# BruceCanovas/supersurfel_fusion

Hardware: AMD Instinct MI355X
Metric: frames_per_sec (higher is better)
Workload: dtype f32; 1 GPU; 640x480 synthetic RGB-D orbit (seed 1234), map seeded with 1000000 supersurfels (~993223 live, ~86081 visible), reference rgbd_benchmark parameters, extract+ICP+fuse per frame; width=640, height=480, n_model=993223, n_visible=86081, superpixels=1200, icp_iter_max=10, icp_forced=False, seed_order=seeded, exchange=none, pipeline_depth=2, extract_batch=8

## Files before the change

supersurfel_fusion_amd/binding.py:

```python
import ctypes as C
import os
import numpy as np

ICP_RECORD = 29
MIGRANT_WORDS = 28
_HERE = os.path.dirname(os.path.abspath(__file__))
PRODUCT_LIB = os.path.join(_HERE, "csrc", "libssf_hip.so")


class SsfConfig(C.Structure):
    _fields_ = [
        ("width", C.c_int), ("height", C.c_int),
        ("fx", C.c_float), ("fy", C.c_float), ("cx", C.c_float), ("cy", C.c_float),
        ("cell_size", C.c_int), ("lambda_pos", C.c_float), ("lambda_bound", C.c_float),
        ("lambda_size", C.c_float), ("lambda_disp", C.c_float), ("thresh_disp", C.c_float),
        ("seg_iter", C.c_int), ("seg_use_ransac", C.c_int), ("nb_samples", C.c_int),
        ("filter_iter", C.c_int), ("filter_alpha", C.c_float), ("filter_beta", C.c_float),
        ("filter_threshold", C.c_float), ("range_min", C.c_float), ("range_max", C.c_float),
        ("delta_t", C.c_int), ("conf_thresh", C.c_float), ("nb_supersurfels_max", C.c_int),
        ("icp_iter", C.c_int), ("icp_cov_thresh", C.c_double),
        ("rng_seed", C.c_uint64), ("icp_force_iters", C.c_int), ("device_id", C.c_int),
        ("stream", C.c_void_p), ("rank", C.c_int), ("nranks", C.c_int),
        ("shard_tile", C.c_float), ("depth_prefilter", C.c_int), ("prefilter_sigma_color", C.c_float),
        ("prefilter_sigma_space", C.c_float), ("profile", C.c_int), ("pipeline_depth", C.c_int), ("extract_batch", C.c_int),
# ... 2 lines not shown

class SsfSurfels(C.Structure):
    _fields_ = [("positions", C.c_void_p), ("colors", C.c_void_p), ("stamps", C.c_void_p),
                ("orientations", C.c_void_p), ("shapes", C.c_void_p), ("dims", C.c_void_p),
                ("confidences", C.c_void_p)]


class SsfFrameResult(C.Structure):
    _fields_ = [("pose", C.c_float * 12), ("icp_valid", C.c_int), ("icp_iters", C.c_int),
                ("n_model", C.c_int), ("n_visible", C.c_int), ("n_removed", C.c_int),
                ("n_inserted", C.c_int), ("n_updated", C.c_int), ("stamp", C.c_int),
                ("stage_ms", C.c_float * 3)]

    def as_dict(self):
        return dict(pose=np.array(self.pose[:], np.float32), icp_valid=self.icp_valid,
                    icp_iters=self.icp_iters, n_model=self.n_model, n_visible=self.n_visible,
                    n_removed=self.n_removed, n_inserted=self.n_inserted, n_updated=self.n_updated,
                    stamp=self.stamp, stage_ms=list(self.stage_ms[:]))


ABI_SYMBOLS = [
    "ssf_abi_version", "ssf_backend_name", "ssf_default_config", "ssf_create", "ssf_destroy",
    "ssf_last_error", "ssf_process_frame", "ssf_process_frame_device", "ssf_stage_extract",
    "ssf_debug_set_max_passes", "ssf_debug_set_bin_min_rows", "ssf_stage_set_shard", "ssf_stage_icp_begin",
    "ssf_stage_icp_accumulate", "ssf_stage_icp_update", "ssf_stage_icp_end", "ssf_stage_match",
    "ssf_stage_fuse", "ssf_get_pose", "ssf_set_pose", "ssf_get_counts", "ssf_get_model",
    "ssf_get_frame", "ssf_set_model", "ssf_get_index_map", "ssf_get_boundary_map",
    "ssf_get_inlier_map", "ssf_get_plane_depth", "ssf_get_superpixels", "ssf_get_model_device", "ssf_get_frame_device",
    "ssf_export_model_txt", "ssf_apply_deformation", "ssf_get_kernel_times",
    "ssf_reset_kernel_times", "ssf_set_profile", "ssf_bilateral_filter", "ssf_submit_frame",
    "ssf_process_submitted", "ssf_pending_frames", "ssf_pipeline_capacity", "ssf_can_submit", "ssf_stage_begin_submitted",
    "ssf_stage_icp_accumulate_device", "ssf_stage_icp_fetch", "ssf_stage_match_device", "ssf_stage_fuse_device",
    "ssf_comm_unique_id", "ssf_comm_attach", "ssf_comm_info", "ssf_p2p_export", "ssf_p2p_attach", "ssf_p2p_region", "ssf_p2p_attach_local", "ssf_p2p_configure", "ssf_rehome_begin", "ssf_rehome_end", "ssf_get_global_counts", "ssf_align", "ssf_fern_codes", "ssf_process_sequence", "ssf_debug_recentre", "ssf_debug_recentre_count", "ssf_get_preview_image", "ssf_stage_fuse_begin", "ssf_stage_fuse_end", "ssf_stage_fuse_begin_device", "ssf_stage_fuse_end_device",
    "ssf_sequence_times", "ssf_sequence_marks", "ssf_stream_copy_rate", "ssf_upload_stats", "ssf_pooled_streams", "ssf_waiter_matches", "ssf_waiter_match_repairs", "ssf_tuner_state", "ssf_submit_frame_tables", "ssf_comm_deal_extract",
]

INPUT_FORMAT_SYMBOLS = ["ssf_set_input_format", "ssf_get_input_format"]
COLOR_FORMATS = {"rgb8": (0, 3), "bgr8": (1, 3), "rgba8": (2, 4), "bgra8": (3, 4)}
DEPTH_FORMATS = {"f32": (0, 4), "u16": (1, 2)}
DYNAMIC_MASK_SYMBOLS = ["ssf_process_frame_pixmask", "ssf_submit_frame_pixmask", "ssf_process_sequence_pixmask",
                        "ssf_stage_extract_pixmask", "ssf_get_dynamic_superpixels"]
RENDER_SYMBOLS = ["ssf_render_default_params", "ssf_render_model"]
GRAPH_SYMBOLS = ["ssf_graph_default_params", "ssf_graph_build", "ssf_graph_get_nodes", "ssf_graph_get_binding",
                 "ssf_graph_bind_points", "ssf_graph_apply", "ssf_graph_info"]
GRAPH_SOLVE_SYMBOLS = ["ssf_graph_solve_default_params", "ssf_graph_get_edges", "ssf_graph_solve", "ssf_graph_get_transforms",
                       "ssf_graph_apply_solved"]
KEYFRAME_SYMBOLS = ["ssf_keyframes_default_params", "ssf_keyframes_configure", "ssf_keyframes_set_ferns", "ssf_keyframes_get_ferns",
                    "ssf_keyframes_encode", "ssf_keyframes_query", "ssf_keyframes_add", "ssf_keyframes_consider", "ssf_keyframes_put",
                    "ssf_keyframes_get", "ssf_keyframes_set_pose", "ssf_keyframes_align", "ssf_keyframes_info", "ssf_keyframes_clear"]
KEYFRAMES_MAX_FERNS = 4096
KEYFRAMES_MAX_CANDIDATES = 8
FERN_DTYPE = np.dtype([("x", np.uint16), ("y", np.uint16), ("r", np.uint8), ("g", np.uint8), ("b", np.uint8), ("pad", np.uint8),
                       ("depth_mm", np.uint32)])
QUERY_SYMBOLS = ["ssf_query_default_params", "ssf_query_count", "ssf_query_rows"]
QUERY_REGIONS = {"all": 0, "sphere": 1, "box": 2, "frustum": 3}
NAVGRID_SYMBOLS = ["ssf_navgrid_default_params", "ssf_navgrid_default_pose", "ssf_navgrid_build"]
NAVGRID_OUTPUTS = (("zmin", np.float32, ()), ("zmax", np.float32, ()), ("hits", np.uint32, (2,)), ("state", np.int8, ()),
                   ("dist2", np.int32, ()))
NAVGRID_OUTPUT_NAMES = tuple(nm for nm, _, _ in NAVGRID_OUTPUTS)
MOTION_SYMBOLS = ["ssf_motion_default_params", "ssf_motion_segment", "ssf_motion_mask", "ssf_process_frame_motion", "ssf_get_motion_mask"]
ODOMETRY_SYMBOLS = ["ssf_odometry_default_params", "ssf_odometry_set_reference", "ssf_odometry_linearise", "ssf_odometry_estimate",
                    "ssf_odometry_track", "ssf_process_frame_odometry", "ssf_get_odometry"]
ODOMETRY_REASONS = ("converged", "max_iterations", "too_few_pixels", "degenerate", "motion_gate")
ODO_MAX_LEVELS, ODO_RECORD = 6, 29
MOTION_CLASSES = {"invalid": 0, "static": 1, "seed": 2, "unknown": 3}
MOTION_OUTPUTS = (("mask", np.uint8), ("label", np.int32), ("cls", np.uint8))
MOTION_OUTPUT_NAMES = tuple(nm for nm, _ in MOTION_OUTPUTS)
RENDER_OUTPUTS = (("depth", np.float32, ()), ("index", np.int32, ()), ("rgb8", np.uint8, (3,)), ("color", np.float32, (3,)),
                  ("normal", np.float32, (3,)))
RENDER_OUTPUT_NAMES = tuple(nm for nm, _, _ in RENDER_OUTPUTS)

SURFEL_FIELDS = (("positions", 3, np.float32), ("colors", 3, np.float32), ("stamps", 2, np.int32),
                 ("orientations", 9, np.float32), ("shapes", 6, np.float32),
                 ("dims", 2, np.float32), ("confidences", 1, np.float32))


class SsfError(RuntimeError):
    pass


class SsfRenderParams(C.Structure):
    _fields_ = [("pose", C.c_void_p), ("width", C.c_int), ("height", C.c_int)] + \
               [(nm, C.c_float) for nm in ("fx", "fy", "cx", "cy", "z_min", "z_max", "min_conf", "splat_scale")] + \
               [("visible_only", C.c_int), ("on_device", C.c_int)]


class SsfRenderStats(C.Structure):
    _fields_ = [(nm, C.c_int64) for nm in ("fragments", "pixels_filled", "rows_shown", "list_entries")]

    def as_dict(self):
        return {nm: int(getattr(self, nm)) for nm, _ in self._fields_}


class SsfMotionParams(C.Structure):
    _fields_ = [("pose", C.c_void_p)] + \
               [(nm, C.c_float) for nm in ("min_conf", "splat_scale", "front_abs", "front_quad", "link_abs", "link_rel")] + \
               [("min_seeds", C.c_int), ("unknown_per_seed", C.c_int), ("on_device", C.c_int)]


class SsfMotionStats(C.Structure):
    _fields_ = [(nm, C.c_int64) for nm in ("n_seed", "n_unknown", "n_components", "n_dynamic_components", "pixels_masked")]

    def as_dict(self):
        return {nm: int(getattr(self, nm)) for nm, _ in self._fields_}


# ... 136 lines not shown
        L.ssf_set_model.argtypes = [vp, C.POINTER(SsfSurfels), C.c_int, C.c_int, C.c_int]
        for nm in ("ssf_get_index_map", "ssf_get_boundary_map", "ssf_get_inlier_map",
                   "ssf_get_plane_depth", "ssf_get_superpixels", "ssf_get_preview_image"):
            getattr(L, nm).argtypes = [vp, vp]
        L.ssf_get_model_device.argtypes = [vp, C.POINTER(SsfSurfels), C.POINTER(C.c_int)]
        L.ssf_export_model_txt.argtypes = [vp, C.c_char_p]
        L.ssf_apply_deformation.argtypes = [vp, vp, vp, vp, C.c_int, vp, vp]
        L.ssf_get_kernel_times.argtypes = [vp, vp, vp, vp, C.c_int]
        L.ssf_reset_kernel_times.argtypes = [vp]
        L.ssf_set_profile.argtypes = [vp, C.c_int]
        L.ssf_bilateral_filter.argtypes = [vp, vp, vp, C.c_int]
        L.ssf_submit_frame.argtypes = [vp, vp, vp, C.c_int, vp]
        L.ssf_process_sequence.argtypes = [vp, vp, vp, C.c_int, C.c_int, vp]
        L.ssf_process_submitted.argtypes = [vp, vp, C.POINTER(SsfFrameResult)]
        L.ssf_pending_frames.argtypes = [vp]
        L.ssf_pipeline_capacity.argtypes = [vp]
        L.ssf_can_submit.argtypes = [vp]
        L.ssf_align.argtypes = [vp, C.POINTER(SsfSurfels), C.c_int, vp, vp, C.POINTER(C.c_int), C.POINTER(C.c_int), C.POINTER(C.c_int)]
        L.ssf_fern_codes.argtypes = [vp, vp, vp, C.c_int, C.c_int, vp, vp, vp, C.c_int, vp]
        L.ssf_comm_unique_id.argtypes = [vp]
        L.ssf_comm_attach.argtypes = [vp, vp]
        L.ssf_p2p_export.argtypes = [vp, vp]
        L.ssf_p2p_attach.argtypes = [vp, vp]
        L.ssf_p2p_region.argtypes = [vp, C.POINTER(C.c_void_p), C.POINTER(C.c_size_t)]
        L.ssf_p2p_attach_local.argtypes = [vp, C.POINTER(C.c_void_p)]
        L.ssf_p2p_configure.argtypes = [vp, C.c_int, C.c_double]
        L.ssf_rehome_begin.argtypes = [vp, vp, C.c_int, C.POINTER(C.c_int)]
        L.ssf_rehome_end.argtypes = [vp, vp, C.c_int]
        L.ssf_get_global_counts.argtypes = [vp, vp]
        L.ssf_stage_begin_submitted.argtypes = [vp]
        L.ssf_stage_icp_accumulate_device.argtypes = [vp, vp]
        L.ssf_stage_icp_fetch.argtypes = [vp, vp, vp]
        L.ssf_stage_match_device.argtypes = [vp, vp, vp]
        L.ssf_stage_fuse_device.argtypes = [vp, vp, vp, C.POINTER(SsfFrameResult)]
        L.ssf_stage_fuse_begin.argtypes = [vp, vp, vp, vp]
        L.ssf_stage_fuse_end.argtypes = [vp, vp, C.POINTER(SsfFrameResult)]
        L.ssf_stage_fuse_begin_device.argtypes = [vp, vp, vp, vp]
        L.ssf_stage_fuse_end_device.argtypes = [vp, vp, C.POINTER(SsfFrameResult)]
        self.has_input_format = all(hasattr(L, nm) for nm in INPUT_FORMAT_SYMBOLS)
        if self.has_input_format:
            L.ssf_set_input_format.argtypes = [vp, C.c_int, C.c_int, C.c_double]
            L.ssf_get_input_format.argtypes = [vp, C.POINTER(C.c_int), C.POINTER(C.c_int), C.POINTER(C.c_double)]
        self.has_dynamic_mask = all(hasattr(L, nm) for nm in DYNAMIC_MASK_SYMBOLS)
        if self.has_dynamic_mask:
            L.ssf_process_frame_pixmask.argtypes = [vp, vp, vp, C.c_int, vp, vp, C.POINTER(SsfFrameResult)]
            L.ssf_submit_frame_pixmask.argtypes = [vp, vp, vp, C.c_int, vp]
            L.ssf_process_sequence_pixmask.argtypes = [vp, vp, vp, vp, C.c_int, C.c_int, vp]
            L.ssf_stage_extract_pixmask.argtypes = [vp, vp, vp, C.c_int, vp]
            L.ssf_get_dynamic_superpixels.argtypes = [vp, vp, C.POINTER(C.c_int)]
        self.has_render = all(hasattr(L, nm) for nm in RENDER_SYMBOLS)
        if self.has_render:
            L.ssf_render_default_params.argtypes = [vp, C.POINTER(SsfRenderParams)]
            L.ssf_render_model.argtypes = [vp, C.POINTER(SsfRenderParams), vp, vp, vp, vp, vp, C.POINTER(SsfRenderStats)]
        self.has_query = all(hasattr(L, nm) for nm in QUERY_SYMBOLS)
        if self.has_query:
            L.ssf_query_default_params.argtypes = [vp, C.POINTER(SsfQueryParams)]
            L.ssf_query_count.argtypes = [vp, C.POINTER(SsfQueryParams), C.POINTER(SsfQueryStats)]
            L.ssf_query_rows.argtypes = [vp, C.POINTER(SsfQueryParams), C.POINTER(SsfSurfels), vp, C.c_int, C.POINTER(SsfQueryStats)]
        self.has_navgrid = all(hasattr(L, nm) for nm in NAVGRID_SYMBOLS)
        if self.has_navgrid:
            L.ssf_navgrid_default_params.argtypes = [vp, C.POINTER(SsfNavGridParams)]
            L.ssf_navgrid_default_pose.argtypes = [vp, C.POINTER(SsfNavGridParams), vp]
            L.ssf_navgrid_build.argtypes = [vp, C.POINTER(SsfNavGridParams), C.POINTER(SsfNavGridOut), C.POINTER(SsfNavGridStats)]
        self.has_motion = all(hasattr(L, nm) for nm in MOTION_SYMBOLS)
        if self.has_motion:
            mp, ms = C.POINTER(SsfMotionParams), C.POINTER(SsfMotionStats)
            L.ssf_motion_default_params.argtypes = [vp, mp]
            L.ssf_motion_segment.argtypes = [vp, mp, vp, vp, vp, vp, vp, ms]
            L.ssf_motion_mask.argtypes = [vp, mp, vp, vp, vp, vp, vp, ms]
            L.ssf_process_frame_motion.argtypes = [vp, vp, vp, C.c_int, vp, mp, C.POINTER(SsfFrameResult)]
            L.ssf_get_motion_mask.argtypes = [vp, vp, ms]
        self.has_odometry = all(hasattr(L, nm) for nm in ODOMETRY_SYMBOLS)
        if self.has_odometry:
            op, orr = C.POINTER(SsfOdometryParams), C.POINTER(SsfOdometryResult)
            L.ssf_odometry_default_params.argtypes = [vp, op]
            L.ssf_odometry_set_reference.argtypes = [vp, vp, vp, C.c_int, vp]
            L.ssf_odometry_linearise.argtypes = [vp, op, C.c_int, vp, vp]
            L.ssf_odometry_estimate.argtypes = [vp, op, vp, vp, C.c_int, vp, vp, orr]
            L.ssf_odometry_track.argtypes = [vp, op, vp, vp, C.c_int, vp, orr]
            L.ssf_process_frame_odometry.argtypes = [vp, vp, vp, C.c_int, op, C.POINTER(SsfMotionParams), C.POINTER(SsfFrameResult)]
            L.ssf_get_odometry.argtypes = [vp, vp, vp, orr]
            L.ssf_odometry_get_pyramid.argtypes = [vp, C.c_int, C.c_int, vp, vp, vp, vp, C.POINTER(C.c_int), C.POINTER(C.c_int), vp]
        self.has_graph = all(hasattr(L, nm) for nm in GRAPH_SYMBOLS)
        if self.has_graph:
            ip = C.POINTER(C.c_int)
            L.ssf_graph_default_params.argtypes = [C.POINTER(SsfGraphParams)]
            L.ssf_graph_build.argtypes = [vp, C.POINTER(SsfGraphParams), ip]
            L.ssf_graph_get_nodes.argtypes = [vp, vp, vp, vp, C.c_int]
            L.ssf_graph_get_binding.argtypes = [vp, vp, vp, C.c_int]
            L.ssf_graph_bind_points.argtypes = [vp, vp, vp, C.c_int, vp, vp]
            L.ssf_graph_apply.argtypes = [vp, vp, vp]
            L.ssf_graph_info.argtypes = [vp, ip, ip, ip]
        self.has_graph_solve = all(hasattr(L, nm) for nm in GRAPH_SOLVE_SYMBOLS)
        if self.has_graph_solve:
            L.ssf_graph_solve_default_params.argtypes = [C.POINTER(SsfGraphSolveParams)]
            L.ssf_graph_get_edges.argtypes = [vp, vp, C.c_int]
            L.ssf_graph_solve.argtypes = [vp, C.POINTER(SsfGraphSolveParams), vp, vp, vp, C.c_int, C.POINTER(SsfGraphSolveResult)]
            L.ssf_graph_get_transforms.argtypes = [vp, vp, vp, C.c_int]
            L.ssf_graph_apply_solved.argtypes = [vp]
        self.has_keyframes = all(hasattr(L, nm) for nm in KEYFRAME_SYMBOLS)
        if self.has_keyframes:
            ip, kp, kr = C.POINTER(C.c_int), C.POINTER(SsfKeyframesParams), C.POINTER(SsfKeyframeResult)
            L.ssf_keyframes_default_params.argtypes = [kp]
            L.ssf_keyframes_configure.argtypes = [vp, kp]
            L.ssf_keyframes_set_ferns.argtypes = [vp, vp, C.c_int]
            L.ssf_keyframes_get_ferns.argtypes = [vp, vp, C.c_int]
# ... 375 lines not shown
        self._need_odometry("ssf_odometry_estimate")
        return self._odometry_estimate(self._dev_addr(d_rgb), self._dev_addr(d_depth), 1, init12, params)

    def _odometry_track(self, rgb_ptr, depth_ptr, on_device, params):
        p = self._odometry_params(params)
        prior, res = np.zeros(12, np.float32), SsfOdometryResult()
        self._ck(self.L.lib.ssf_odometry_track(self.h, C.byref(p), rgb_ptr, depth_ptr, int(on_device), _ptr(prior), C.byref(res)),
                 "ssf_odometry_track")
        return (prior if res.valid else None), res.as_dict()

    def odometry_track(self, rgb, depth, params=None):
        self._need_odometry("ssf_odometry_track")
        rgb, depth = self._frame(rgb, depth)
        return self._odometry_track(_ptr(rgb), _ptr(depth), 0, params)

    def odometry_track_device(self, d_rgb, d_depth, params=None):
        self._need_odometry("ssf_odometry_track")
        return self._odometry_track(self._dev_addr(d_rgb), self._dev_addr(d_depth), 1, params)

    def odometry_last(self):
        self._need_odometry("ssf_get_odometry")
        rel, prior, res = np.zeros(12, np.float32), np.zeros(12, np.float32), SsfOdometryResult()
        self._ck(self.L.lib.ssf_get_odometry(self.h, _ptr(rel), _ptr(prior), C.byref(res)), "ssf_get_odometry")
        return dict(rel=rel, prior=prior if res.valid else None, result=res.as_dict())

    def odometry_pyramid(self, which, level):
        self._need_odometry("ssf_odometry_get_pyramid")
        w, h, k = C.c_int(), C.c_int(), np.zeros(4, np.float32)
        self._ck(self.L.lib.ssf_odometry_get_pyramid(self.h, int(which), int(level), None, None, None, None, C.byref(w), C.byref(h), _ptr(k)),
                 "ssf_odometry_get_pyramid")
        out = {nm: np.empty((h.value, w.value), np.float32) for nm in ("I", "D", "gx", "gy")}
        self._ck(self.L.lib.ssf_odometry_get_pyramid(self.h, int(which), int(level), *[_ptr(out[nm]) for nm in ("I", "D", "gx", "gy")],
                                                     None, None, None), "ssf_odometry_get_pyramid")
        out["intrinsics"] = k
        return out

    def _process_frame_odometry(self, rgb_ptr, depth_ptr, on_device, odometry, motion):
        self._need_odometry("ssf_process_frame_odometry")
        if not (odometry is True or isinstance(odometry, dict)):
            raise SsfError("odometry is None, True or a dict of ssf_odometry_params fields, got %r" % (odometry,))
        p = self._odometry_params(None if odometry is True else odometry)
        mp, keep = None, None
        if motion is not None:
            self._need_motion("ssf_process_frame_motion")
            if not (motion is True or isinstance(motion, dict)):
                raise SsfError("motion is None, True or a dict of ssf_motion_params fields, got %r" % (motion,))
            m, keep = self._motion_params(None if motion is True else motion, on_device)
            mp = C.byref(m)
        res = SsfFrameResult()
        self._ck(self.L.lib.ssf_process_frame_odometry(self.h, rgb_ptr, depth_ptr, int(bool(on_device)), C.byref(p), mp, C.byref(res)),
                 "ssf_process_frame_odometry")
        return res

    def _need_query(self, symbol):
        if not self.L.has_query:
            raise SsfError("%s does not export %s: it does not query the model (include/ssf_query.h, HIP product only)"
                           % (self.L.path, symbol))

    def _query_params(self, on_device, min_conf=0.0, t_init=None, t_last=None, visible_only=False, region="all", pose=None,
                      radius=0.0, half=(0.0, 0.0, 0.0), camera=None, z_range=None):
        p = SsfQueryParams()
        self._ck(self.L.lib.ssf_query_default_params(self.h, C.byref(p)), "ssf_query_default_params")
        keep = None
        if pose is not None:
            pose = np.asarray(pose, np.float32)
            if pose.shape == (3, 4):
                pose = np.concatenate([pose[:, :3].ravel(), pose[:, 3]])
            if pose.size != 12:
                raise SsfError("a query pose is 12 floats (R row-major, then t) or 3 x 4 [R | t], got shape %s" % (pose.shape,))
            keep = np.ascontiguousarray(pose.ravel(), np.float32)
            p.pose = keep.ctypes.data
        p.min_conf = float(min_conf)
        if t_init is not None:
            p.t_init_min, p.t_init_max = int(t_init[0]), int(t_init[1])
        if t_last is not None:
            p.t_last_min, p.t_last_max = int(t_last[0]), int(t_last[1])
        if isinstance(region, str) and region not in QUERY_REGIONS:
            raise SsfError("unknown query region %r (known: %s)" % (region, ", ".join(QUERY_REGIONS)))
        p.region = QUERY_REGIONS[region] if isinstance(region, str) else int(region)
        p.radius = float(radius)
        p.half[0], p.half[1], p.half[2] = (float(v) for v in half)
        if camera is not None:
            p.width, p.height = int(camera["width"]), int(camera["height"])
            p.fx, p.fy, p.cx, p.cy = (float(camera[k]) for k in ("fx", "fy", "cx", "cy"))
        if z_range is not None:
            p.z_min, p.z_max = float(z_range[0]), float(z_range[1])
        p.visible_only, p.on_device = int(bool(visible_only)), int(bool(on_device))
        return p, keep

    def _query_rows(self, p, ptrs, index_ptr, capacity):
        st = SsfQueryStats()
        surf = SsfSurfels(*[ptrs.get(name) for name, _, _ in SURFEL_FIELDS])
        rc = self.L.lib.ssf_query_rows(self.h, C.byref(p), C.byref(surf) if any(ptrs.get(name) for name, _, _ in SURFEL_FIELDS) else None,
                                       index_ptr, int(capacity), C.byref(st))
        if rc != 0:
            e = SsfError("ssf_query_rows failed (%d): %s" % (rc, self.L.lib.ssf_last_error(self.h).decode()))
            e.rc, e.stats = rc, st.as_dict()
            raise e
        return st.as_dict()

    def query_default_params(self):
        self._need_query("ssf_query_default_params")
        p = SsfQueryParams()
        self._ck(self.L.lib.ssf_query_default_params(self.h, C.byref(p)), "ssf_query_default_params")
        return {nm: (list(getattr(p, nm)) if nm == "half" else getattr(p, nm)) for nm, _ in p._fields_ if nm != "pose"}

# ... 773 lines not shown
```

supersurfel_fusion_amd/csrc/ssf_device.hpp:

```cpp
#pragma once
#include <hip/hip_runtime.h>
#include <stdint.h>
#include <cstddef>
#include "ssf_math.hpp"
#include "../../include/ssf.h"
#include "../../include/ssf_input.h"
#include "../../include/ssf_dynamic.h"

#ifdef SSF_EXPERIMENTS
#include <stdlib.h>
static inline int ssf_env_int_(const char* name, int dflt) { const char* e = getenv(name); return e ? atoi(e) : dflt; }
#define SSF_ENV_INT(name, dflt) ssf_env_int_("SSF_" name, dflt)
#define SSF_ENV_SET(name) (getenv("SSF_" name) != nullptr)
#define SSF_ENV_STR(name) getenv("SSF_" name)
#define SSF_PROBE(dbg, bits) ((((dbg)) & (bits)) != 0)
#else
#define SSF_PROBE(dbg, bits) (false)
#define SSF_ENV_INT(name, dflt) (dflt)
#define SSF_ENV_SET(name) (false)
#define SSF_ENV_STR(name) ((const char*)nullptr)
#endif

namespace ssf {

// ... 126 lines not shown
void pass_args_table(const SegParams& p, const FrameMaps& m, int kmax, void* host_out);
void launch_update_passes_team(hipStream_t st, const SegParams& p, FrameMaps& m, int nb, int k0, int k1, bool rgbd, const void* d_pas, void* d_ws,
                               unsigned int* abort_flag);
void launch_init_samples(hipStream_t st, const SegParams& p, FrameMaps& m, int nb, int true_buf);
void launch_eval_samples(hipStream_t st, const SegParams& p, FrameMaps& m, int nb);
void launch_init_disp(hipStream_t st, const SegParams& p, FrameMaps& m, int nb, bool ransac);
void launch_plane_filter(hipStream_t st, const SegParams& p, FrameMaps& m, int nb, int true_buf);
void launch_import_frame(hipStream_t st, const SegParams& p, FrameMaps& m, int nb, SurfelSoA frame, const float* wire, unsigned long long* best, uint8_t* matched);
void launch_export_rows(hipStream_t st, const SegParams& p, const FrameMaps& m, int nb, SurfelSoA frame, float* wire);
void launch_render_moments(hipStream_t st, const SegParams& p, const Cam& cam, FrameMaps& m, int nb);
void launch_render_moments_pixmask(hipStream_t st, const SegParams& p, const Cam& cam, FrameMaps& m, int nb, const uint8_t* pixmask,
                                   uint32_t* pixcnt);
void launch_finalize_surfels(hipStream_t st, const SegParams& p, FrameMaps& m, int nb, SurfelSoA frame, float zmin,
                             float zmax, int stamp0, const uint8_t* dynamic_mask, unsigned mask_bits,
                             unsigned long long* best, uint8_t* matched);
void launch_finalize_surfels_pixmask(hipStream_t st, const SegParams& p, FrameMaps& m, int nb, SurfelSoA frame, float zmin, float zmax,
                                     int stamp0, const uint8_t* dynamic_mask, unsigned mask_bits, unsigned long long* best, uint8_t* matched,
                                     const uint32_t* pixcnt, unsigned pixmask_bits);
void launch_bilateral(hipStream_t st, const void* in, int depth_format, double depth_scale, float* out, int W, int H, float sigma_color,
                      float sigma_space);
void launch_bilateral_batch(hipStream_t st, const BatchIn& in, float* out0, size_t slab, int nb, int W, int H, float sigma_color, float sigma_space);
void launch_boundary_map(hipStream_t st, const SegParams& p, const int32_t* label, int32_t* out);
void launch_preview(hipStream_t st, int W, int H, const int32_t* label, const uint32_t* rgba, uint8_t* out );

struct alignas(64) IcpGo { float T[12]; unsigned long long flag; unsigned long long x; };
static_assert(sizeof(IcpGo) == 64, "one line");
#define SSF_ICP_GO_ABORT (1ull << 63)
#define SSF_ICP_GO_MATCH (1ull << 62)
#define SSF_ICP_GO_CHECK_MASK 0x3FFFFFFFu
SSF_HD unsigned int icp_go_word_weight(unsigned int dword) {
    return dword < 12u ? (2u * dword + 1u) * 0x9E3779B1u : (dword == 14u ? 0x85EBCA6Bu : (dword == 15u ? 0xC2B2AE35u : 0u));
}
SSF_HD unsigned int icp_go_abort_check(unsigned int want) { return ((want * 0x9E3779B1u) >> 2) & SSF_ICP_GO_CHECK_MASK; }
#define SSF_ICP_GO_SLOTS 4
struct MatchArgs { float zmin, zmax; long long id_offset; unsigned long long* best; uint8_t* matched; int32_t* cand; };
struct ClassifyArgs { Cam cam; const float* plane_depth; int delta_t; float conf_thresh, zmin, zmax; };
struct ShardArgs { int rank, nranks, migrate; float tile; };
struct AssocTables { const unsigned long long* best; const uint8_t* matched; const int32_t* cand; int S; };
int icp_variant_mode();
void launch_icp(hipStream_t st, const Cam& cam, SurfelSoA model, int n_visible, const uint2* pix2, const float4* fpack,
                Rt T, long long* replicas, unsigned int* ticket,
                long long* sums29, Mailbox* mb, unsigned long long seq, int dbg = -1, IcpGo* go = nullptr,
                unsigned long long go_seq = 0, const struct P2PView* pv = nullptr, int by_tile = 0, const MatchArgs* match = nullptr);
void launch_bin_rows(hipStream_t st, const Cam& cam, SurfelSoA model, int n, Rt T, uint32_t* count, uint32_t* cursor, SurfelSoA out);
size_t bin_buffer_words(const Cam& cam, size_t capacity);
void launch_match(hipStream_t st, const Cam& cam, SurfelSoA model, int n_visible, const uint2* pix2, const float4* fpack,
                  Rt pose, float zmin, float zmax, long long id_offset,
                  unsigned long long* best, uint8_t* matched, int32_t* cand , int S,
                  const int32_t* orig = nullptr );
struct OovStore { SurfelSoA rows; uint8_t* live; int cap; };
#define PART_GROUP 16
#define PART_REPLICAS 8
struct PartitionWs { uint32_t* sup_vis; uint32_t* sup_oov; uint32_t* tot; uint32_t* ticket; uint32_t* other; int words; };
void launch_fuse(hipStream_t st, SurfelSoA model , SurfelSoA frame, Rt pose, int stamp, long long id_offset,
                 int n_visible, const AssocTables& at, int do_update, int capacity, const ShardArgs& sh, Counters* cnt, OovStore oov,
                 int span_upper, const ClassifyArgs& ca, uint8_t* state_vis, uint8_t* state_oov, uint32_t* bc_oov, const PartitionWs& ws,
                 int tail_in_move = 0 );
#ifdef SSF_EXPERIMENTS
void set_pass_stats(int on);
void set_pass_trace(unsigned long long* device_words );
void set_fuse_trace(unsigned long long* device_words );
#endif
struct MoveTotals { int from_tot, nv , head_old, tail_old ; };
void launch_pack_emigrants(hipStream_t st, SurfelSoA model, const AssocTables& at, long long id_offset, int n_visible,
                           const uint8_t* state_vis, int do_update, const ShardArgs& sh, int32_t* table);
void launch_migrate_in(hipStream_t st, SurfelSoA model, const int32_t* table, int S, int capacity, Counters* cnt, const ShardArgs& sh,
                       const ClassifyArgs& ca, Rt pose, int stamp, uint8_t* state_vis, const PartitionWs& ws);
void launch_rehome_split(hipStream_t st, SurfelSoA dense, int n, int n_visible, int rank, int nranks, float tile, uint32_t* bc, int* tot3,
                         SurfelSoA stay, int32_t* table, int table_rows);
void launch_rehome_unpack(hipStream_t st, const int32_t* table, int n, SurfelSoA dst, int base);
void launch_first_frame(hipStream_t st, SurfelSoA model, SurfelSoA frame, Rt pose, int S, int capacity, const ShardArgs& sh, Counters* cnt);
struct NextIcp {
    Cam cam; const uint2* pix2; const float4* fpack;
    Rt T;
    long long* replicas; unsigned int* ticket; long long* sums; Mailbox* mb; unsigned long long seq;
};
void launch_move_rows(hipStream_t st, SurfelSoA vis_src, SurfelSoA vis_dst, OovStore oov, int nv_upper, int span_upper,
                      const uint8_t* state_vis, const uint8_t* state_oov, const uint32_t* bc_oov, const PartitionWs& ws,
                      Counters* cnt , Mailbox* mb, unsigned long long cnt_seq, const NextIcp* next,
                      const struct P2PView* next_pv = nullptr, const MoveTotals* totals = nullptr);
void launch_oov_compact(hipStream_t st, OovStore src, OovStore dst, int span_upper, int new_head, uint32_t* bc_oov, Counters* cnt,
                        int set_span);
struct ModelView { SurfelSoA vis; OovStore oov; int n_visible, nbv, nvs, oov_head, oov_tail, nbo, nslots; };
void launch_align(hipStream_t st, const Cam& cam, const float* spos, const float* slab, const float* snrm, const float* sconf,
                  int n, SurfelSoA frame, const int32_t* label, const float* plane_depth, Rt T, long long* out40);
void launch_fern_codes(hipStream_t st, const uint8_t* rgb, const float* depth, int W, int H, const uint32_t* fpos,
                       const uint8_t* frgb, const float* fdepth, int n, uint8_t* codes);
#define SSF_P2P_MAX_RANKS 8
struct P2PView { unsigned char* peer[SSF_P2P_MAX_RANKS]; int me, nranks, S; unsigned long long seq, timeout_ticks; };
enum { P2P_FLAG_ASSOC = 0, P2P_FLAG_MIGR = 1 };
#define SSF_P2P_HEADER 8192
SSF_HD size_t p2p_slot(int par, int src) { return (size_t)(par * SSF_P2P_MAX_RANKS + src); }
SSF_HD size_t p2p_spad(int S) { return ((size_t)S + 63) & ~(size_t)63; }
SSF_HD size_t p2p_off_icp(int par, int src) { return p2p_slot(par, src) * 320; }
SSF_HD size_t p2p_off_cnt(int par, int src) { return 16 * 320 + p2p_slot(par, src) * 64; }
SSF_HD size_t p2p_off_flag(int kind, int par, int src) { return 16 * 384 + ((size_t)kind * 16 + p2p_slot(par, src)) * 64; }
SSF_HD size_t p2p_off_best(int S, int par, int src) { return SSF_P2P_HEADER + p2p_slot(par, src) * (size_t)S * 8; }
SSF_HD size_t p2p_off_matched(int S, int par, int src) { return SSF_P2P_HEADER + 16 * (size_t)S * 8 + p2p_slot(par, src) * p2p_spad(S); }
SSF_HD size_t p2p_off_migr(int S, int par, int src) {
    return SSF_P2P_HEADER + 16 * (size_t)S * 8 + 16 * p2p_spad(S) + p2p_slot(par, src) * (size_t)S * SSF_MIGRANT_WORDS * 4;
}
SSF_HD size_t p2p_region_bytes(int S) { return p2p_off_migr(S, 1, SSF_P2P_MAX_RANKS - 1) + (size_t)S * SSF_MIGRANT_WORDS * 4; }
void launch_p2p_counts(hipStream_t st, const P2PView& pv, const Counters* cnt, Mailbox* mb, unsigned long long all_seq);
void launch_p2p_assoc(hipStream_t st, const P2PView& pv, unsigned long long* best, uint8_t* matched, Mailbox* mb);
void launch_p2p_migrants(hipStream_t st, const P2PView& pv, int32_t* table, unsigned int* ticket , Mailbox* mb);
void launch_publish_icp(hipStream_t st, const long long* rec29, Mailbox* mb, unsigned long long seq);
void launch_publish_all_counts(hipStream_t st, const int* all5, int nranks, Mailbox* mb, unsigned long long seq);
void launch_publish_counts(hipStream_t st, Counters* cnt, int shrink_by_removed, Mailbox* mb, unsigned long long seq);
void launch_lab_refresh(hipStream_t st, SurfelSoA s, int n);
void launch_pack_orient(hipStream_t st, SurfelSoA s, int n, float* out9);
void launch_deformation(hipStream_t st, SurfelSoA model, int n, int m, const float* npos, const float* nrot,
                        const float* ntrans, float* nodes16, const float* w4, const int32_t* idx4);

struct KernelTimer;
KernelTimer* current_timer();
void set_current_timer(KernelTimer* t);
void timer_begin(KernelTimer* t, const char* name, hipStream_t st);
void timer_end(KernelTimer* t, hipStream_t st);
struct ScopedKernel {
    KernelTimer* t; hipStream_t st;
    ScopedKernel(const char* name, hipStream_t s) : t(current_timer()), st(s) { if (t) timer_begin(t, name, st); }
    ~ScopedKernel() { if (t) timer_end(t, st); }
};

}
```

supersurfel_fusion_amd/csrc/ssf_graph.hip:

```cpp
#include <climits>
#include "ssf_slots.hpp"
#include "ssf_handle.hpp"

namespace ssf {

#define GRAPH_SORT_ITEMS 2048

__global__ __launch_bounds__(256) void k_graph_keys(ModelView mv, float min_conf, int32_t* __restrict__ stamp, uint8_t* __restrict__ elig,
                                                    uint32_t* __restrict__ bc, int* __restrict__ mm) {
    __shared__ int mmw[4][2], ce[4], cl[4];
    const uint32_t s = blockIdx.x * 256u + threadIdx.x;
    SurfelSoA src; size_t row;
    const bool lv = slot_row(mv, s, src, row);
    int t = 0; bool el = false;
    if (lv) {
        t = src.stamps[2 * row];
        el = src.conf[row] > min_conf && finite3(src.pos[3 * row], src.pos[3 * row + 1], src.pos[3 * row + 2]);
    }
    stamp[s] = t; elig[s] = el ? 1 : 0;
    int lo = el ? t : INT_MAX, hi = el ? t : INT_MIN;
#pragma unroll
    for (int o = 32; o > 0; o >>= 1) { lo = min(lo, __shfl_xor(lo, o, 64)); hi = max(hi, __shfl_xor(hi, o, 64)); }
    if (lane() == 0) { mmw[threadIdx.x >> 6][0] = lo; mmw[threadIdx.x >> 6][1] = hi; }
    const int e = block_count256(el, ce), l = block_count256(lv, cl);
// ... 294 lines not shown
    if (!h) return SSF_ERR_INVALID_ARG;
    if (n_nodes) *n_nodes = h->graph.built ? h->graph.m : 0;
    if (n_rows) *n_rows = h->graph.built ? h->graph.rows : 0;
    if (valid) *valid = graph_valid(h) ? 1 : 0;
    return SSF_OK;
}
int ssf_graph_get_nodes(ssf_handle* h, float* positions, int32_t* t_init, int32_t* rows, int capacity) {
    if (!h || (!positions && !t_init && !rows)) return SSF_ERR_INVALID_ARG;
    const GraphWs& g = h->graph;
    if (!g.built) { h->err = "ssf_graph_get_nodes: no graph has been built (ssf_graph_build)"; return SSF_ERR_STATE; }
    if (capacity < g.m) { h->err = "ssf_graph_get_nodes: " + std::to_string(g.m) + " nodes, room for " + std::to_string(capacity); return SSF_ERR_CAPACITY; }
    hipStream_t st = h->stream;
    const size_t m = g.m;
    std::vector<float> rec;
    if (positions) HCK(hipMemcpyAsync(positions, g.npos3, 12 * m, hipMemcpyDeviceToHost, st));
    if (rows) HCK(hipMemcpyAsync(rows, g.nrow, 4 * m, hipMemcpyDeviceToHost, st));
    if (t_init) { rec.resize(4 * m); HCK(hipMemcpyAsync(rec.data(), g.nodes, 16 * m, hipMemcpyDeviceToHost, st)); }
    HCK(hipStreamSynchronize(st));
    if (t_init) for (size_t k = 0; k < m; k++) std::memcpy(&t_init[k], &rec[4 * k + 3], 4);
    return SSF_OK;
}
int ssf_graph_get_binding(ssf_handle* h, float* weights4, int32_t* idx4, int on_device) {
    if (!h || (!weights4 && !idx4)) return SSF_ERR_INVALID_ARG;
    { int rc = graph_usable(h, "ssf_graph_get_binding"); if (rc) return rc; }
    const GraphWs& g = h->graph;
    const hipMemcpyKind kind = on_device ? hipMemcpyDeviceToDevice : hipMemcpyDeviceToHost;
    if (weights4) HCK(hipMemcpyAsync(weights4, g.w4, 16 * (size_t)g.rows, kind, h->stream));
    if (idx4) HCK(hipMemcpyAsync(idx4, g.idx4, 16 * (size_t)g.rows, kind, h->stream));
    HCK(hipStreamSynchronize(h->stream));
    return SSF_OK;
}
int ssf_graph_bind_points(ssf_handle* h, const float* points, const int32_t* t_init, int n, float* weights4, int32_t* idx4) {
    if (!h || !points || !t_init || !weights4 || !idx4 || n < 0) return SSF_ERR_INVALID_ARG;
    { int rc = graph_usable(h, "ssf_graph_bind_points"); if (rc) return rc; }
    if (n == 0) return SSF_OK;
    const GraphWs& g = h->graph;
    float *d_p, *d_w; int32_t *d_t, *d_i;
    DevTemps tmp;
    HCK(tmp.take(&d_p, 12 * (size_t)n)); HCK(tmp.take(&d_t, 4 * (size_t)n)); HCK(tmp.take(&d_w, 16 * (size_t)n)); HCK(tmp.take(&d_i, 16 * (size_t)n));
    hipStream_t st = h->stream;
    HCK(hipMemcpyAsync(d_p, points, 12 * (size_t)n, hipMemcpyHostToDevice, st));
    HCK(hipMemcpyAsync(d_t, t_init, 4 * (size_t)n, hipMemcpyHostToDevice, st));
    { TimerScope ts(h); launch_graph_bind_points(st, d_p, d_t, n, g.nodes, g.m, g.look, d_w, d_i, "graph_bind"); }
    HCK(hipGetLastError());
    HCK(hipMemcpyAsync(weights4, d_w, 16 * (size_t)n, hipMemcpyDeviceToHost, st));
    HCK(hipMemcpyAsync(idx4, d_i, 16 * (size_t)n, hipMemcpyDeviceToHost, st));
    { int rc = sync_collect(h); if (rc) return rc; }
    return SSF_OK;
}
int ssf_graph_apply(ssf_handle* h, const float* nr, const float* nt) {
    if (!h || !nr || !nt) return SSF_ERR_INVALID_ARG;
    { int rc = graph_usable(h, "ssf_graph_apply"); if (rc) return rc; }
    drop_shard_sizes(h);
    h->ahead.valid = false;
    const GraphWs& g = h->graph;
    const size_t m = g.m;
    float *d_nr, *d_nt, *d_nodes;
    DevTemps tmp;
    HCK(tmp.take(&d_nr, 36 * m)); HCK(tmp.take(&d_nt, 12 * m)); HCK(tmp.take(&d_nodes, 64 * m));
    HCK(hipMemcpyAsync(d_nr, nr, 36 * m, hipMemcpyHostToDevice, h->stream));
    HCK(hipMemcpyAsync(d_nt, nt, 12 * m, hipMemcpyHostToDevice, h->stream));
    return deform_dense(h, g.m, g.npos3, d_nr, d_nt, d_nodes, g.w4, g.idx4);
}
}
```

supersurfel_fusion_amd/csrc/ssf_graph_solve.hip:

```cpp
#include "ssf_handle.hpp"

namespace ssf {

struct SolveArgs {
    const float4* nodes; const int4* edges; int m, nc, nbn, nbc;
    const uint32_t *in_off, *in_list, *con_off, *con_list;
    const float *src, *dst; const float4* w4; const int4* idx4;
    double *x, *b, *D, *delta, *r, *z, *q, *y_rot, *y_reg, *y_con;
    double *e_rot, *e_reg, *e_con, *pq, *hist;
    float *rot, *trans;
    double sr, sg, sc, damping;
};

__device__ __forceinline__ double block_tree256(double v, double* s) {
    s[threadIdx.x] = v;
    __syncthreads();
#pragma unroll
    for (int h = 128; h >= 1; h >>= 1) {
        if ((int)threadIdx.x < h) s[threadIdx.x] = s[threadIdx.x] + s[threadIdx.x + h];
        __syncthreads();
    }
    const double out = s[0];
    __syncthreads();
    return out;
// ... 424 lines not shown
                ScopedKernel sk("graph_solve", st);
                for (int k = 0; k < chunk; k++, it++) {
                    const int cur = it & 1;
                    hipLaunchKernelGGL(k_solve_jp, dim3(nbmax), dim3(256), 0, st, a, it == 0 ? 1 : 0, rho[cur], rho[cur ^ 1], pbuf[cur ^ 1], pbuf[cur]);
                    hipLaunchKernelGGL(k_solve_jt<false>, dim3(nbn), dim3(256), 0, st, a, (const double*)pbuf[cur], a.pq);
                    hipLaunchKernelGGL(k_solve_update, dim3(nbn), dim3(256), 0, st, a, (const double*)pbuf[cur], (const double*)rho[cur], rho[cur ^ 1], k);
                }
            }
            HCK(hipGetLastError());
            HCK(hipMemcpyAsync(hp.data(), rho[it & 1], 8 * (size_t)nbn, hipMemcpyDeviceToHost, st));
            HCK(hipMemcpyAsync(hp.data() + nbn, a.hist, 8 * (size_t)chunk, hipMemcpyDeviceToHost, st));
            HCK(hipStreamSynchronize(st));
            for (int k = 0; k < chunk; k++) {
                const double pq = hp[nbn + k];
                if (!(pq > 0.0 && std::isfinite(pq))) { it = it - chunk + k; end = SSF_GRAPH_SOLVE_END_BREAKDOWN; running = false; break; }
            }
            if (!running) break;
            const double rho_now = host_ordered_sum(hp.data(), nbn);
            if (it % p->inner_check == 0 && rho_now <= tol2 * rho0) { end = SSF_GRAPH_SOLVE_END_TOLERANCE; break; }
            if (it >= p->max_inner) { end = SSF_GRAPH_SOLVE_END_MAX_INNER; break; }
        }
        { ScopedKernel sk("graph_solve", st); hipLaunchKernelGGL(k_solve_step, dim3(nbn), dim3(256), 0, st, a); }
        { int rc = energy(En); if (rc) return rc; }
        res.inner[outer] = it; res.inner_end = end; res.outer = outer + 1;
        const bool done = std::fabs(E[0] - En[0]) <= p->outer_tol * E[0];
        std::memcpy(E, En, sizeof(E));
        if (done) break;
    }
    res.e_after = E[0]; res.e_rot = E[1]; res.e_reg = E[2]; res.e_con = E[3];
    { int rc = sync_collect(h); if (rc) return rc; }
    s.solved = true; s.gen = g.gen;
    if (result) *result = res;
    return SSF_OK;
}
static int solved_usable(ssf_handle* h, const char* who) {
    { int rc = graph_usable(h, who); if (rc) return rc; }
    if (!h->solve.solved || h->solve.gen != h->graph.gen) { h->err = std::string(who) + ": no transforms have been solved on this graph (ssf_graph_solve)"; return SSF_ERR_STATE; }
    return SSF_OK;
}
int ssf_graph_get_transforms(ssf_handle* h, float* rotations, float* translations, int capacity) {
    if (!h || (!rotations && !translations)) return SSF_ERR_INVALID_ARG;
    { int rc = solved_usable(h, "ssf_graph_get_transforms"); if (rc) return rc; }
    const size_t m = h->graph.m;
    if (capacity < h->graph.m) { h->err = "ssf_graph_get_transforms: " + std::to_string(m) + " nodes, room for " + std::to_string(capacity); return SSF_ERR_CAPACITY; }
    if (rotations) HCK(hipMemcpyAsync(rotations, h->solve.rot, 36 * m, hipMemcpyDeviceToHost, h->stream));
    if (translations) HCK(hipMemcpyAsync(translations, h->solve.trans, 12 * m, hipMemcpyDeviceToHost, h->stream));
    HCK(hipStreamSynchronize(h->stream));
    return SSF_OK;
}
int ssf_graph_apply_solved(ssf_handle* h) {
    if (!h) return SSF_ERR_INVALID_ARG;
    { int rc = solved_usable(h, "ssf_graph_apply_solved"); if (rc) return rc; }
    drop_shard_sizes(h);
    h->ahead.valid = false;
    const GraphWs& g = h->graph;
    float* d_nodes;
    DevTemps tmp;
    HCK(tmp.take(&d_nodes, 64 * (size_t)g.m));
    return deform_dense(h, g.m, g.npos3, h->solve.rot, h->solve.trans, d_nodes, g.w4, g.idx4);
}
}
```

supersurfel_fusion_amd/csrc/ssf_handle.hpp:

```cpp
#pragma once
#include <algorithm>
#include <climits>
#include <cmath>
#include <cstring>
#include <deque>
#include <initializer_list>
#include <map>
#include <string>
#include <utility>
#include <vector>
#include "ssf_device.hpp"
#include "../../include/ssf_render.h"
#include "../../include/ssf_graph.h"
#include "../../include/ssf_graph_solve.h"
#include "../../include/ssf_keyframes.h"
#include "../../include/ssf_motion.h"
#include "../../include/ssf_odometry.h"
#include "../../include/ssf_navgrid.h"

struct ncclComm; typedef struct ncclComm* ncclComm_t;
struct Uploader;
namespace ssf {
struct KernelTimer {
    struct Rec { const char* name; hipEvent_t e0, e1; };
    std::vector<Rec> open, pool_free;
    std::vector<Rec> pending;
    std::map<std::string, std::pair<double, long long>> acc;
    const char* cur_name = nullptr; hipEvent_t cur_e0 = nullptr, cur_e1 = nullptr;
    double bracket_bias_ms = -1.0;
};
}
using namespace ssf;

struct AheadTuner {
    static const int START = 48, PROBE = 16, ROUNDS = 3, HOLD = 1024, SKIP = 2;
    int forced = -1;
    int mode = 0, frames = 0, left = START, round = 0, since_switch = 0;
    bool probing = false;
    double sum[2] = {0, 0}; int n[2] = {0, 0};
    double last_done_us = -1.0; int last_mode = 0;
    int current() const { return forced >= 0 ? (forced ? 1 : 0) : mode; }
    void sequence_break() { last_done_us = -1.0; }
    void frame_done(double t_us, int iters) {
        if (forced >= 0) return;
        if (last_done_us >= 0.0 && since_switch >= SKIP && probing && iters > 0) { sum[last_mode] += (t_us - last_done_us) / (double)(iters + 4); n[last_mode]++; }
        last_done_us = t_us; last_mode = mode; frames++; since_switch++;
        if (--left > 0) return;
        if (!probing) { probing = true; round = 0; sum[0] = sum[1] = 0; n[0] = n[1] = 0; mode ^= 1; left = PROBE; since_switch = 0; return; }
        if (++round < 2 * ROUNDS) { mode ^= 1; left = PROBE; since_switch = 0; return; }
        probing = false;
        if (n[0] > 0 && n[1] > 0) mode = (sum[1] / n[1] < sum[0] / n[0]) ? 1 : 0;
        left = HOLD; since_switch = 0;
    }
};

struct IcpLoop {
    bool active = false, valid = true, done = true;
    int iter = 0;
    unsigned long long ahead_seq = 0;
    double tf_inc[16], prev_error, JtJ[36];
    M3 R_init; V3 t_init, t_inc_stale;
};

struct ExtractCtx {
    FrameMaps maps;
    SurfelSoA frame;
    unsigned long long* d_best = nullptr; uint8_t* d_matched = nullptr;
    uint8_t* d_rgb_in = nullptr; float* d_depth_in = nullptr; float* d_depth_filt = nullptr; uint8_t* d_mask = nullptr;
    float* d_wire = nullptr;
    char* d_pas = nullptr; char* d_team_ws = nullptr;
    ncclComm_t deal_comm = nullptr;
    bool mine = true; long long deal_batch = 0;
    hipStream_t stream = nullptr; bool own_stream = false; int stream_prio = 0;
    hipEvent_t ev_done = nullptr, ev_consumed = nullptr, ev_t0 = nullptr, ev_t1 = nullptr;
    bool consumed_valid = false, timed = false;
    hipGraph_t graph[SSF_MAX_BATCH + 1] = {}; hipGraphExec_t exec[SSF_MAX_BATCH + 1] = {};
    int count = 0, inflight = 0, stamp0 = 0, nb_launched = 1; bool launched = false, waited = false;
    uint32_t epoch0 = 0;
    BatchIn in = {}; unsigned mask_bits = 0;
    uint8_t* d_pixmask = nullptr; uint32_t* d_pixcnt = nullptr; unsigned pixmask_bits = 0;
    bool from_tables = false;
    hipGraph_t graph_pm[SSF_MAX_BATCH + 1] = {}; hipGraphExec_t exec_pm[SSF_MAX_BATCH + 1] = {};
};
struct ActiveFrame {
    FrameMaps maps; SurfelSoA frame;
    unsigned long long* d_best = nullptr; uint8_t* d_matched = nullptr;
    ExtractCtx* ctx = nullptr; int slot = 0;
    bool pixmask = false;
    bool has_rgba = false;
    bool activated = false;
};

#ifndef SSF_BIN_MIN_ROWS_DEFAULT
#define SSF_BIN_MIN_ROWS_DEFAULT 400000
#endif
struct TileCopy {
    SurfelSoA rows{};
    int32_t* d_idx = nullptr; uint32_t* d_count = nullptr; uint32_t* d_cursor = nullptr;
    bool valid = false; int min_rows = SSF_BIN_MIN_ROWS_DEFAULT;
    int make_if_large(ssf_handle* h);
    void drop() { valid = false; }
};
struct DevBufs {
    std::vector<void**> owned;
    bool grow(std::initializer_list<std::pair<void**, size_t>> want) {
        std::vector<void*> got;
        for (const auto& w : want) {
// ... 85 lines not shown
struct NavGridWs {
    DevBufs bufs;
    float4* rec = nullptr; uint2* rbox = nullptr; size_t slots = 0;
    uint32_t* tcnt = nullptr; uint32_t* cursor = nullptr; size_t tiles = 0;
    uint32_t* list = nullptr; size_t list_cap = 0;
    uint32_t* acc = nullptr; uint16_t* colg = nullptr; int8_t* state = nullptr; size_t cells = 0;
    unsigned long long* stats = nullptr;
    unsigned char* img = nullptr; size_t img_bytes = 0;
};
struct ssf_handle {
    ssf_config cfg;
    int S = 0, gx = 0, gy = 0;
    std::string err;
    hipStream_t stream = nullptr; bool own_stream = false; int stream_prio = 0;
    SegParams seg; Cam cam;
    std::vector<ExtractCtx> ctx; int open_ctx = 0, batch = 1;
    std::deque<std::pair<int, int>> pending;
    ActiveFrame active; ActiveFrame* cc = &active;
    uint32_t extract_ordinal = 0;
    const void* const* seq_rgb = nullptr; const void* const* seq_depth = nullptr; const uint8_t* const* seq_pixmask = nullptr; int seq_next = 0, seq_n = 0, seq_on_device = 0, stamp_bias = 0;
    long long n_waiter_matches = 0;
    int seq_k = 0;
    int seq_batches = 0;
    double us_wait_upload = 0.0;
    Uploader* up = nullptr; bool seq_upload = false;
    int in_color = SSF_COLOR_RGB8, in_depth = SSF_DEPTH_F32_METRES; double in_scale = 1.0;
    ncclComm_t comm = nullptr; int* d_all5 = nullptr;
    int deal = 0; long long deal_batches = 0;
    struct P2P {
        unsigned char* region = nullptr; size_t bytes = 0; bool fine = false;
        bool same_device = false; double timeout_s = 30.0;
        P2PView view{}; bool on = false; std::vector<void*> opened;
        unsigned long long seq_icp = 0, seq_cnt = 0, seq_assoc = 0, seq_migr = 0;
    } p2p;
    unsigned long long all_seq = 0; bool all_pending = false, all_valid = false;
    long long all_cnt[5 * SSF_MAX_RANKS];
    SurfelSoA model[2]; int mcur = 0;
    std::vector<void*> allocs;
    struct Guarded { void* base; size_t bytes, guard; };
    std::vector<Guarded> guarded;
    float* d_bf_in = nullptr; float* d_bf_out = nullptr; float* d_orient9 = nullptr; float* d_frame_orient9 = nullptr;
    long long* d_icp = nullptr;
    uint8_t* d_state = nullptr; int32_t* d_cand = nullptr; Counters* d_cnt = nullptr;
    int32_t* d_migrants = nullptr; PartitionWs fuse_ws{}; bool fuse_first = false, fuse_migrate = false, fusing = false;
    MoveTotals fuse_totals{0, 0, 0, 0}; bool move_totals_on = true;
    OovStore oov[2]; int ocur = 0; int oov_head = 0, oov_tail = 0, oov_live = 0; long long n_recentres = 0;
    uint8_t* d_state_oov = nullptr; uint32_t* d_bc_oov = nullptr;
    uint32_t* d_part = nullptr; uint32_t* d_part_ticket = nullptr; int part_words = 0, part_sup_vis = 0, part_sup_oov = 0, part_set = 0;
    SurfelSoA dense; uint8_t* d_live_scratch = nullptr;
    int32_t* d_scratch_map = nullptr;
    long long* d_icp_replicas = nullptr; unsigned int* d_tickets = nullptr; float* d_srgb_lut = nullptr;
    Mailbox* mb_host = nullptr; Mailbox* mb_dev = nullptr;
    unsigned long long icp_seq = 0, cnt_seq = 0;
    struct { bool valid = false; unsigned long long seq = 0; ExtractCtx* ctx = nullptr; int slot = 0; int stamp = 0; Rt pose; } ahead;
    double wait_launched_us = 0.0; long long n_waiter_match_repairs = 0; long long dbg_stall_before_match_us = 0;
    bool icp_ahead = true; int icp_ahead_mode = 1;
    AheadTuner ahead_tuner;
    IcpGo* go = nullptr; bool icp_chain = true; unsigned long long go_count = 0;
    bool graph_failed = false; hipStream_t capture_stream = nullptr;
    TileCopy bins;
    ClassifyArgs classify{}; ShardArgs shard{};
    bool pass_team = false; ExtractCtx* team_prev = nullptr;
    long long h_icp_local[SSF_ICP_RECORD];
    long long* h_icp = nullptr; Counters* h_cnt = nullptr;
    int n_model = 0, n_visible = 0, stamp = 0, max_passes = 0;
    Rt pose;
    IcpLoop icp;
    long long id_offset = 0, global_n_model = -1, global_n_visible = -1;
    bool have_frame = false;
    int last_icp_valid = 0, last_icp_iters = 0;
    hipEvent_t ev[4] = {nullptr, nullptr, nullptr, nullptr};
    KernelTimer timer;
    std::vector<std::string> timer_names;
    double seq_mark_us[4][64] = {{0}}, seq_launch_us[32] = {0}, seq_launch_host_us[32] = {0}; int seq_launch_n[32] = {0}, seq_launches = 0;
    double seq_t0_us = 0, seq_done_us[64] = {0};
    double host_us[8] = {0, 0, 0, 0, 0, 0, 0, 0};
    RenderWs render;
    GraphWs graph;
    KeyframeWs kf;
    SolveWs solve;
    QueryWs query;
    MotionWs motion;
    OdoWs odo;
    NavGridWs navgrid;
    unsigned long long model_gen = 0;
};

#define HCK(call)                                                                                    \
    do {                                                                                             \
        hipError_t e_ = (call);                                                                      \
        if (e_ != hipSuccess) {                                                                      \
            h->err = std::string(#call) + ": " + hipGetErrorString(e_);                              \
            return SSF_ERR_DEVICE;                                                                   \
        }                                                                                            \
    } while (0)

#pragma GCC visibility push(hidden)
namespace ssf {
struct DevTemps {
    std::vector<void*> p;
    template <typename T> hipError_t take(T** out, size_t bytes) {
        void* q = nullptr;
        const hipError_t e = hipMalloc(&q, bytes ? bytes : 1);
        if (e == hipSuccess) { p.push_back(q); *out = (T*)q; }
        return e;
    }
    ~DevTemps() { for (void* q : p) (void)hipFree(q); }
};
struct TimerScope { ssf_handle* h; explicit TimerScope(ssf_handle* hh); ~TimerScope(); };
void timer_collect(KernelTimer* t);
// ... 38 lines not shown
```

supersurfel_fusion_amd/csrc/ssf_host.hip:

```cpp
#include <atomic>
#include <chrono>
#include <cstdio>
#include <cstdlib>
#include <new>
#include <condition_variable>
#include <mutex>
#include <thread>
#include <type_traits>
#include <unistd.h>
#include "ssf_exchange.hpp"
#include "ssf_solvers.hpp"

using namespace ssf;

namespace ssf {
static thread_local KernelTimer* g_timer = nullptr;
KernelTimer* current_timer() { return g_timer; }
void set_current_timer(KernelTimer* t) { g_timer = t; }
void timer_begin(KernelTimer* t, const char* name, hipStream_t st) {
    KernelTimer::Rec r;
    if (!t->pool_free.empty()) { r = t->pool_free.back(); t->pool_free.pop_back(); }
    else { (void)hipEventCreate(&r.e0); (void)hipEventCreate(&r.e1); }
    r.name = name;
    (void)hipEventRecord(r.e0, st);
// ... 465 lines not shown
    if (h->seq_next < h->seq_n) return SSF_OK;
    ExtractCtx& c = h->ctx[h->open_ctx];
    return (c.count > 0 && !c.launched) ? launch_batch(h, c) : SSF_OK;
}
static int seq_submit(ssf_handle* h) {
    const int i = h->seq_next;
    const uint8_t* pixmask = h->seq_pixmask ? h->seq_pixmask[i] : nullptr;
    if (h->seq_on_device || !h->seq_upload) {
        int rc = submit_extract(h, h->seq_rgb[i], h->seq_depth[i], h->seq_on_device, nullptr, pixmask, h->seq_on_device);
        if (!rc) { h->seq_next++; rc = seq_flush_tail(h); }
        return rc;
    }
    Uploader& u = *h->up;
    const auto t0 = std::chrono::steady_clock::now();
    const double w0 = now_us();
    for (unsigned long long spins = 0; !u.ready(i); spins++) {
        if (u.failed.load()) { h->err = "upload of a host frame failed"; return SSF_ERR_DEVICE; }
        if ((spins & 0xFFFF) == 0xFFFF && std::chrono::duration<double>(std::chrono::steady_clock::now() - t0).count() > 10.0) {
            h->err = "upload of a host frame never finished"; return SSF_ERR_DEVICE;
        }
        std::this_thread::yield();
    }
    h->us_wait_upload += now_us() - w0;
    const int sl = i % u.ring;
    int rc = submit_extract(h, u.d_rgb[sl], u.d_depth[sl], 1, nullptr, pixmask ? u.d_mask[sl] : nullptr, 1);
    if (!rc) { h->seq_next++; rc = seq_flush_tail(h); }
    return rc;
}
static int do_extract(ssf_handle* h, const void* rgb, const void* depth, int on_device, const uint8_t* mask, const uint8_t* pixmask = nullptr) {
    if (!frame_args_ok(h, rgb, depth, on_device)) return SSF_ERR_INVALID_ARG;
    TimerScope ts(h);
    if (!h->pending.empty()) { h->err = "frames are pending in the extract pipeline"; return SSF_ERR_STATE; }
    int rc = retire_active(h);
    if (!rc) rc = submit_extract(h, rgb, depth, on_device, mask, pixmask, on_device);
    return rc ? rc : activate_oldest(h);
}

static inline bool single_shard_alone(const ssf_handle* h) { return h->cfg.nranks == 1 && !h->comm && !h->p2p.on; }
static inline bool exchanges_natively(const ssf_handle* h) { return h->comm || h->p2p.on; }
static inline bool icp_is_one_launch(const ssf_handle* h) { return single_shard_alone(h) || (h->p2p.on && !h->comm); }
static inline long long total_model(const ssf_handle* h) { return (h->cfg.nranks > 1 && h->global_n_model >= 0) ? h->global_n_model : h->n_model; }
static inline long long total_visible(const ssf_handle* h) { return (h->cfg.nranks > 1 && h->global_n_visible >= 0) ? h->global_n_visible : h->n_visible; }
static void icp_start_from(IcpLoop& I, const Rt& pose) {
    I.R_init = m3_transpose(pose.R);
    I.t_init = negate(m3_mulv(I.R_init, pose.t));
    for (int i = 0; i < 16; i++) I.tf_inc[i] = (i % 5 == 0) ? 1.0 : 0.0;
}
static void icp_begin(ssf_handle* h, const float* prior) {
    h->bins.drop();
    if (prior) h->pose = pose_from12(prior);
    IcpLoop& I = h->icp;
    I.ahead_seq = 0;
    if (h->ahead.valid && !prior && h->have_frame && h->active.ctx == h->ahead.ctx && h->active.slot == h->ahead.slot &&
        h->stamp == h->ahead.stamp && std::memcmp(&h->pose, &h->ahead.pose, sizeof(Rt)) == 0) I.ahead_seq = h->ahead.seq;
    h->ahead.valid = false;
    I.active = total_visible(h) > 0 && h->cfg.icp_iter > 0;
    I.valid = true; I.done = !I.active; I.iter = 0;
    icp_start_from(I, h->pose);
    for (int i = 0; i < 36; i++) I.JtJ[i] = 0.0;
    I.prev_error = DBL_MAX;
    I.t_inc_stale = v3(0, 0, 0);
    h->last_icp_valid = 0; h->last_icp_iters = 0;
}
static void inc_to_float(const double* tf, M3& R, V3& t) {
    R = m3(v3((float)tf[0], (float)tf[1], (float)tf[2]), v3((float)tf[4], (float)tf[5], (float)tf[6]),
           v3((float)tf[8], (float)tf[9], (float)tf[10]));
    t = v3((float)tf[3], (float)tf[7], (float)tf[11]);
}
static Rt icp_transform(IcpLoop& I) {
    M3 R_inc; V3 t_inc;
    inc_to_float(I.tf_inc, R_inc, t_inc);
    I.t_inc_stale = t_inc;
    Rt T; T.R = m3_mul(R_inc, I.R_init); T.t = add(m3_mulv(R_inc, I.t_init), t_inc);
    return T;
}
static inline void store_fence() {
#if defined(__x86_64__)
    __builtin_ia32_sfence();
#else
    __atomic_thread_fence(__ATOMIC_SEQ_CST);
#endif
}
static void icp_release_waiting(IcpGo* slot, unsigned long long go_seq, const Rt* T, unsigned long long p2p_seq = 0, bool match = false) {
    volatile IcpGo* s = slot;
    const unsigned long long want = go_seq & 0xFFFFFFFFull;
    if (T) {
        const float v[12] = {T->R.r0.x, T->R.r0.y, T->R.r0.z, T->R.r1.x, T->R.r1.y, T->R.r1.z, T->R.r2.x, T->R.r2.y, T->R.r2.z,
                             T->t.x, T->t.y, T->t.z};
        uint32_t w[12]; memcpy(w, v, sizeof w);
        uint32_t sum = (uint32_t)p2p_seq * icp_go_word_weight(14) + (uint32_t)(p2p_seq >> 32) * icp_go_word_weight(15);
        for (unsigned int i = 0; i < 12; i++) sum += w[i] * icp_go_word_weight(i);
        for (int i = 0; i < 12; i++) s->T[i] = v[i];
        s->x = p2p_seq;
        s->flag = want | ((unsigned long long)((sum >> 2) & SSF_ICP_GO_CHECK_MASK) << 32) | (match ? SSF_ICP_GO_MATCH : 0ull);
    } else s->flag = want | ((unsigned long long)icp_go_abort_check((unsigned int)want) << 32) | SSF_ICP_GO_ABORT;
    store_fence();
}

struct IcpWaiter { bool waiting = false; IcpGo* slot = nullptr; unsigned long long go_seq = 0, seq_rec = 0; };
static int icp_fetch(ssf_handle* h, unsigned long long seq, IcpWaiter* waiter = nullptr) {
    const volatile unsigned long long* rec = h->mb_host->icp_rec;
    auto t0 = std::chrono::steady_clock::now();
    bool drained = false;
    for (unsigned long long spins = 0;; spins++) {
        bool ok = true;
        for (int j = 0; j < 5 && ok; j++) ok = __atomic_load_n(&rec[8 * j + 7], __ATOMIC_ACQUIRE) == seq;
        if (ok) {
            unsigned long long check = seq, w29 = 0;
            for (int p = 0; p < 30; p++) {
// ... 75 lines not shown
        else {
            M3 R_inc; V3 t_inc;
            inc_to_float(I.tf_inc, R_inc, t_inc);
            const M3 R_rel = m3_transpose(R_inc);
            const V3 t_rel = negate(m3_mulv(R_rel, t_inc));
            h->pose.t = add(m3_mulv(h->pose.R, t_rel), h->pose.t);
            h->pose.R = m3_mul(h->pose.R, R_rel);
            float R9[9] = {h->pose.R.r0.x, h->pose.R.r0.y, h->pose.R.r0.z, h->pose.R.r1.x, h->pose.R.r1.y, h->pose.R.r1.z,
                           h->pose.R.r2.x, h->pose.R.r2.y, h->pose.R.r2.z};
            renormalise_rotation<float>(R9);
            h->pose.R = m3(v3(R9[0], R9[1], R9[2]), v3(R9[3], R9[4], R9[5]), v3(R9[6], R9[7], R9[8]));
        }
    }
    *valid = ok ? 1 : 0;
    h->last_icp_valid = *valid;
    I.active = false;
}

namespace ssf {
SurfelSoA soa_rows(const SurfelSoA& s, size_t r) {
    SurfelSoA v = s;
    each_stream([&](auto m, size_t w) { v.*m += w * r; });
    return v;
}
int copy_soa(ssf_handle* h, const SurfelSoA& d, const SurfelSoA& s, size_t n) {
    if (n == 0) return SSF_OK;
    hipError_t copy_of_a_stream = hipSuccess;
    each_stream([&](auto m, size_t w) { if (!copy_of_a_stream) copy_of_a_stream = hipMemcpyAsync(d.*m, s.*m, 4 * w * n, hipMemcpyDeviceToDevice, h->stream); });
    HCK(copy_of_a_stream);
    return SSF_OK;
}
static int oov_home(const ssf_handle* h) { return h->cfg.nb_supersurfels_max + h->S + 256; }
static int oov_recentre(ssf_handle* h) {
    OovStore& src = h->oov[h->ocur]; OovStore& dst = h->oov[h->ocur ^ 1];
    HCK(hipMemsetAsync(dst.live, 0, (size_t)dst.cap, h->stream));
    launch_oov_compact(h->stream, src, dst, h->oov_tail - h->oov_head, oov_home(h), h->d_bc_oov, h->d_cnt, 1);
    HCK(hipGetLastError());
    h->ocur ^= 1;
    h->oov_head = oov_home(h); h->oov_tail = h->oov_head + h->oov_live;
    h->n_recentres++;
    return SSF_OK;
}
int materialise(ssf_handle* h) {
    int rc = copy_soa(h, h->dense, h->model[h->mcur], (size_t)h->n_visible);
    if (rc) return rc;
    if (h->oov_live > 0) {
        OovStore dst; dst.rows = h->dense; dst.live = h->d_live_scratch; dst.cap = h->cfg.nb_supersurfels_max;
        launch_oov_compact(h->stream, h->oov[h->ocur], dst, h->oov_tail - h->oov_head, h->n_visible, h->d_bc_oov, h->d_cnt, 0);
        HCK(hipGetLastError());
    }
    return SSF_OK;
}
int store_from_dense(ssf_handle* h, int n, int n_visible) {
    h->ahead.valid = false;
    h->bins.drop();
    h->model_gen++;
    int rc = copy_soa(h, h->model[h->mcur], h->dense, (size_t)n_visible);
    if (rc) return rc;
    OovStore& o = h->oov[h->ocur];
    const int head = oov_home(h), n_oov = n - n_visible;
    rc = copy_soa(h, soa_rows(o.rows, (size_t)head), soa_rows(h->dense, (size_t)n_visible), (size_t)n_oov);
    if (rc) return rc;
    HCK(hipMemsetAsync(o.live, 0, (size_t)o.cap, h->stream));
    if (n_oov > 0) HCK(hipMemsetAsync(o.live + head, 1, (size_t)n_oov, h->stream));
    Counters c; std::memset(&c, 0, sizeof(c));
    c.n_model = n; c.n_visible = n_visible; c.oov_head = head; c.oov_tail = head + n_oov; c.oov_live = n_oov;
    c.last[0] = n; c.last[1] = n_visible;
    HCK(hipStreamSynchronize(h->stream));
    HCK(hipMemcpy(h->d_cnt, &c, sizeof(c), hipMemcpyHostToDevice));
    h->n_model = n; h->n_visible = n_visible; h->oov_head = c.oov_head; h->oov_tail = c.oov_tail; h->oov_live = n_oov;
    return SSF_OK;
}
void drop_shard_sizes(ssf_handle* h) { h->all_valid = false; h->all_pending = false; }
}

static int do_match(ssf_handle* h, int exchange = 0) {
    const bool any = total_model(h) > 0 && total_visible(h) > 0;
    const int n = any ? h->n_visible : 0;
    launch_match(h->stream, h->cam, icp_rows(h), n, h->cc->maps.pix2, h->cc->maps.fpack, h->pose, h->cfg.range_min,
                 h->cfg.range_max, h->id_offset, h->cc->d_best, h->cc->d_matched, h->d_cand, h->S, h->bins.valid ? h->bins.d_idx : nullptr);
    if (exchange && h->p2p.on) launch_p2p_assoc(h->stream, p2p_view(h, ++h->p2p.seq_assoc), h->cc->d_best, h->cc->d_matched, h->mb_dev);
    HCK(hipGetLastError());
    return SSF_OK;
}

static int fuse_begin(ssf_handle* h, int migrate) {
    const long long nmodel_g = total_model(h), nvis_g = total_visible(h);
    SurfelSoA& M = h->model[h->mcur];
    h->bins.drop();
    h->fuse_first = !(nmodel_g > 0);
    h->fuse_migrate = migrate && h->cfg.nranks > 1 && !h->fuse_first;
    h->classify.plane_depth = h->cc->maps.plane_depth; h->shard.migrate = h->fuse_migrate ? 1 : 0;
    if (nmodel_g > 0) {
        {
            const int span = h->oov_tail - h->oov_head;
            if (h->oov_head < h->n_visible + h->S + 256 || h->oov[h->ocur].cap - h->oov_tail < 2 * h->S + 256 ||
                span > h->oov_live + h->oov_live / 4 + 65536) { int rc2 = oov_recentre(h); if (rc2) return rc2; }
        }
        h->fuse_totals.from_tot = (single_shard_alone(h) && !h->fuse_migrate && h->move_totals_on) ? 1 : 0;
        h->fuse_totals.nv = h->n_visible; h->fuse_totals.head_old = h->oov_head; h->fuse_totals.tail_old = h->oov_tail;
        PartitionWs& ws = h->fuse_ws;
        {
            uint32_t* set = h->d_part + (size_t)h->part_set * h->part_words;
            ws.sup_vis = set; ws.sup_oov = set + h->part_sup_vis; ws.tot = ws.sup_oov + h->part_sup_oov;
            ws.ticket = h->d_part_ticket; ws.other = h->d_part + (size_t)(h->part_set ^ 1) * h->part_words; ws.words = h->part_words;
            h->part_set ^= 1;
        }
        const AssocTables at{h->cc->d_best, h->cc->d_matched, h->d_cand, h->S};
        launch_fuse(h->stream, M, h->cc->frame, h->pose, h->stamp, h->id_offset, h->n_visible, at, nvis_g > 0 ? 1 : 0,
                    h->cfg.nb_supersurfels_max, h->shard, h->d_cnt, h->oov[h->ocur], h->oov_tail - h->oov_head, h->classify,
                    h->d_state, h->d_state_oov, h->d_bc_oov, ws, h->fuse_totals.from_tot);
        if (h->fuse_migrate)
            launch_pack_emigrants(h->stream, M, at, h->id_offset, h->n_visible, h->d_state, nvis_g > 0 ? 1 : 0, h->shard, h->d_migrants);
    }
    HCK(hipGetLastError());
    h->fusing = true;
    h->model_gen++;
    return SSF_OK;
}
static int fuse_end(ssf_handle* h, const int32_t* d_table, ssf_frame_result* out) {
    SurfelSoA& M = h->model[h->mcur];
    const unsigned long long seq = ++h->cnt_seq;
    h->fusing = false;
    if (!h->fuse_first) {
        const PartitionWs& ws = h->fuse_ws;
        if (h->fuse_migrate && d_table)
            launch_migrate_in(h->stream, M, d_table, h->S, h->cfg.nb_supersurfels_max, h->d_cnt, h->shard, h->classify, h->pose, h->stamp,
                              h->d_state, ws);
        NextIcp next{};
        P2PView next_pv{};
        bool have_next = false;
        if (h->icp_ahead && (h->p2p.on || h->ahead_tuner.current() == 1) && icp_is_one_launch(h) && h->cfg.icp_iter > 0 && !h->pending.empty()) {
            ExtractCtx& nc = h->ctx[h->pending.front().first];
            const int nslot = h->pending.front().second;
            const bool multi = h->ctx.size() > 1;
            bool ready = nc.launched && (!multi || nc.waited);
            if (nc.launched && !ready && (h->icp_ahead_mode == 2 || h->p2p.on || hipEventQuery(nc.ev_done) == hipSuccess)) {
                HCK(hipStreamWaitEvent(h->stream, nc.ev_done, 0)); nc.waited = true; ready = true;
            }
            (void)hipGetLastError();
            if (ready) {
                const FrameMaps nm = batch_slot(nc.maps, nslot);
                IcpLoop first;
                icp_start_from(first, h->pose);
                next = NextIcp{h->cam, nm.pix2, nm.fpack, icp_transform(first), h->d_icp_replicas, h->d_tickets + 8, h->d_icp, h->mb_dev, ++h->icp_seq};
                if (h->p2p.on) next_pv = p2p_view(h, ++h->p2p.seq_icp);
                h->ahead.valid = true; h->ahead.seq = next.seq; h->ahead.ctx = &nc; h->ahead.slot = nslot;
                h->ahead.stamp = h->stamp + 1; h->ahead.pose = h->pose;
                have_next = true;
            }
        }
        if (exchanges_natively(h)) { int rg = comm_gather_counts(h); if (rg) return rg; }
        launch_move_rows(h->stream, M, h->model[h->mcur ^ 1], h->oov[h->ocur], h->n_visible + (h->fuse_migrate ? 2 : 1) * h->S, h->oov_tail - h->oov_head,
                         h->d_state, h->d_state_oov, h->d_bc_oov, ws, h->d_cnt, h->mb_dev, seq, have_next ? &next : nullptr,
                         have_next && h->p2p.on ? &next_pv : nullptr, h->fuse_totals.from_tot ? &h->fuse_totals : nullptr);
        h->mcur ^= 1;
    } else {
        launch_first_frame(h->stream, M, h->cc->frame, h->pose, h->S, h->cfg.nb_supersurfels_max, h->shard, h->d_cnt);
        launch_publish_counts(h->stream, h->d_cnt, 0, h->mb_dev, seq);
        if (exchanges_natively(h)) { int rg = comm_gather_counts(h); if (rg) return rg; }
    }
    HCK(hipGetLastError());
    { int rr = retire_active(h); if (rr) return rr; }
    h->stamp_bias = 1;
    while (h->seq_next < h->seq_n && !h->ctx[h->open_ctx].launched) {
        int rs = seq_submit(h);
        if (rs) { h->stamp_bias = 0; return rs; }
    }
    h->stamp_bias = 0;
    int rc = wait_seq(h, &h->mb_host->cnt_seq, seq);
    if (rc) return rc;
    Counters c;
    for (int attempt = 0;; attempt++) {
        unsigned long long check = seq;
        const int* srcw = reinterpret_cast<const int*>(&h->mb_host->cnt);
        int* dstw = reinterpret_cast<int*>(&c);
        for (int i = 0; i < (int)(sizeof(Counters) / sizeof(int)); i++) {
            dstw[i] = __atomic_load_n(&srcw[i], __ATOMIC_RELAXED);
            check += (unsigned long long)(unsigned int)dstw[i];
        }
        if (check == __atomic_load_n(&h->mb_host->cnt_check, __ATOMIC_ACQUIRE)) break;
        if (attempt > 100000) { h->err = "counter mailbox record failed its checksum"; return SSF_ERR_DEVICE; }
    }
    h->n_model = c.n_model; h->n_visible = c.n_visible;
    h->oov_head = c.oov_head; h->oov_tail = c.oov_tail; h->oov_live = c.oov_live;
    if (__atomic_load_n(&h->mb_host->extract_abort, __ATOMIC_ACQUIRE) != 0u) {
        __atomic_store_n(&h->mb_host->extract_abort, 0u, __ATOMIC_RELEASE);
        h->err = "a team launch of the relabelling passes could not get all its workgroups onto the GPU and gave up (the GPU is oversubscribed: "
                 "several processes?); the frames of that batch are invalid";
        return SSF_ERR_DEVICE;
    }
    if (h->p2p.on && __atomic_load_n(&h->mb_host->p2p_timeout, __ATOMIC_ACQUIRE) != 0u) {
        __atomic_store_n(&h->mb_host->p2p_timeout, 0u, __ATOMIC_RELEASE);
        h->err = "a peer's association / migrant tables never arrived (peer-to-peer exchange)"; return SSF_ERR_DEVICE;
    }
    if (out) {
        std::memset(out, 0, sizeof(*out));
        pose_to12(h->pose, out->pose);
        out->icp_valid = h->last_icp_valid; out->icp_iters = h->last_icp_iters;
        out->n_model = h->n_model; out->n_visible = h->n_visible; out->n_removed = c.n_removed;
        out->n_inserted = c.n_inserted; out->n_updated = c.n_updated; out->stamp = h->stamp;
        ExtractCtx* ec = h->active.ctx;
        float ms;
        if (h->cfg.profile != 0 && ec && ec->timed && hipEventElapsedTime(&ms, ec->ev_t0, ec->ev_t1) == hipSuccess)
            out->stage_ms[0] = ms / (float)ec->nb_launched;
    }
    h->stamp++;
    h->global_n_model = -1; h->global_n_visible = -1;
    if (h->cfg.profile == 1) { HCK(hipStreamSynchronize(h->stream)); timer_collect(&h->timer); }
    return SSF_OK;
}

static int do_fuse(ssf_handle* h, ssf_frame_result* out) {
    int rc = fuse_begin(h, 0);
    return rc ? rc : fuse_end(h, nullptr, out);
}

static bool icp_waiter_can_match(const ssf_handle* h) {
    static const bool off = SSF_ENV_SET("NO_MATCH_IN_WAITER");
    return !off && single_shard_alone(h) && h->cfg.profile == 0 && icp_variant_mode() == 0;
}
static int icp_launch_waiting(ssf_handle* h, IcpWaiter& w) {
    w.seq_rec = ++h->icp_seq;
    w.go_seq = ++h->go_count;
    w.slot = h->go + (w.go_seq % SSF_ICP_GO_SLOTS);
    h->wait_launched_us = now_us();
    Rt none; none.R = m3_identity(); none.t = v3(0, 0, 0);
    const P2PView pv = h->p2p.view;
    const MatchArgs ma{h->cfg.range_min, h->cfg.range_max, h->id_offset, h->cc->d_best, h->cc->d_matched, h->d_cand};
    const int rc = icp_issue(h, none, w.seq_rec, nullptr, w.slot, w.go_seq, h->p2p.on ? &pv : nullptr, icp_waiter_can_match(h) ? &ma : nullptr);
    w.waiting = rc == SSF_OK;
    return rc;
}
static void icp_chain_reset(ssf_handle* h) {
    (void)hipStreamSynchronize(h->stream);
    (void)hipMemsetAsync(h->d_icp_replicas, 0, 2 * SSF_ICP_REPLICAS * 32 * sizeof(long long), h->stream);
    (void)hipMemsetAsync(h->d_tickets, 0, 512 * sizeof(unsigned int), h->stream);
    (void)hipStreamSynchronize(h->stream);
    h->icp_chain = false; h->ahead.valid = false;
}
struct TrackFrame { double t_a = 0.0, t_b = 0.0; int kf = -1; bool timing = false, first_it = true; IcpWaiter w; };
int TileCopy::make_if_large(ssf_handle* h) {
    if (!(h->icp.active && min_rows >= 0 && h->n_visible >= min_rows && h->n_visible > 0 && single_shard_alone(h) && bin_buffer_words(h->cam, 1) != 0)) return SSF_OK;
    if (!d_idx) {
        const size_t N = (size_t)h->cfg.nb_supersurfels_max, bw = bin_buffer_words(h->cam, N);
        const bool ok = bw && dalloc(h, &rows.pos, 12 * N) && dalloc(h, &d_idx, 1) && dalloc(h, &d_count, bw) && dalloc(h, &d_cursor, bw);
        if (!ok) { h->err = "allocation of the tile-sorted copy failed"; return SSF_ERR_DEVICE; }
    }
    Rt T0; T0.R = h->icp.R_init; T0.t = h->icp.t_init;
    launch_bin_rows(h->stream, h->cam, h->model[h->mcur], h->n_visible, T0, d_count, d_cursor, rows);
    HCK(hipGetLastError());
    valid = true;
    return SSF_OK;
}
static inline bool icp_chains(const ssf_handle* h) { return h->icp_chain && h->go && icp_is_one_launch(h) && h->cfg.profile != 1; }
static int icp_loop_chained(ssf_handle* h, TrackFrame& f) {
    IcpWaiter& w = f.w;
    int again = h->icp.active ? 1 : 0, rc;
    while (again) {
        unsigned long long seq_rec;
        if (h->icp.ahead_seq) { seq_rec = h->icp.ahead_seq; h->icp.ahead_seq = 0; }
        else {
            const Rt T = icp_transform(h->icp);
            const unsigned long long xseq = h->p2p.on ? ++h->p2p.seq_icp : 0;
            if (w.waiting) { icp_release_waiting(w.slot, w.go_seq, &T, xseq); seq_rec = w.seq_rec; w.waiting = false; }
            else {
                const P2PView pv = p2p_view(h, xseq);
                seq_rec = ++h->icp_seq;
                rc = icp_issue(h, T, seq_rec, nullptr, nullptr, 0, h->p2p.on ? &pv : nullptr);
                if (rc) return rc;
            }
        }
        if (h->icp.iter + 1 < h->cfg.icp_iter || (!f.timing && icp_waiter_can_match(h))) {
            rc = icp_launch_waiting(h, w);
            if (rc) return rc;
        }
        rc = icp_fetch(h, seq_rec, w.waiting ? &w : nullptr);
        if (rc) { if (w.waiting) icp_release_waiting(w.slot, w.go_seq, nullptr); icp_chain_reset(h); return rc; }
        if (f.first_it) { h->host_us[5] += now_us() - f.t_a; f.first_it = false; if (f.kf >= 0 && f.kf < 64) h->seq_mark_us[1][f.kf] = now_us() - h->seq_t0_us; }
        icp_update(h, (const int64_t*)h->h_icp, &again);
    }
    return SSF_OK;
}
static int icp_loop_plain(ssf_handle* h, TrackFrame& f) {
    int again = h->icp.active ? 1 : 0, rc;
    while (again) {
        if (h->p2p.on) {
            const P2PView pv = p2p_view(h, ++h->p2p.seq_icp);
            rc = icp_accumulate(h, true, nullptr, &pv);
        } else if (h->comm) {
            rc = icp_accumulate(h, false);
            if (rc) return rc;
// ... 40 lines not shown
        NCK(api->AllReduce(h->cc->d_best, h->cc->d_best, h->S, ncclInt64, ncclMin, h->comm, h->stream));
        NCK(api->AllReduce(h->cc->d_matched, h->cc->d_matched, h->S, ncclUint8, ncclMax, h->comm, h->stream));
    }
    return SSF_OK;
}
static int exchange_and_fuse(ssf_handle* h, ssf_frame_result* r) {
    if (!exchanges_natively(h)) return do_fuse(h, r);
    static const int migrate = SSF_ENV_SET("NO_MIGRATE") ? 0 : 1;
    const int rc = fuse_begin(h, migrate);
    if (rc) { h->fusing = false; return rc; }
    if (h->fuse_migrate && h->p2p.on) launch_p2p_migrants(h->stream, p2p_view(h, ++h->p2p.seq_migr), h->d_migrants, h->d_tickets + 320, h->mb_dev);
    else if (h->fuse_migrate) {
        RcclApi* api = rccl_api();
        ScopedKernel sk("exchange_migrants", h->stream);
        const ncclResult_t nr = api->AllReduce(h->d_migrants, h->d_migrants, (size_t)SSF_MIGRANT_WORDS * h->S, ncclInt32, ncclSum, h->comm, h->stream);
        if (nr != ncclSuccess) {
            h->fusing = false;
            h->err = std::string("ncclAllReduce (migrant table): ") + (api->GetErrorString ? api->GetErrorString(nr) : "RCCL error");
            return SSF_ERR_DEVICE;
        }
    }
    return fuse_end(h, h->d_migrants, r);
}
static int stage_times(ssf_handle* h, ssf_frame_result* r) {
    HCK(hipEventRecord(h->ev[3], h->stream));
    HCK(hipEventSynchronize(h->ev[3]));
    float ms;
    ExtractCtx* ec = h->cc->ctx;
    if (hipEventElapsedTime(&ms, ec->ev_t0, ec->ev_t1) == hipSuccess) r->stage_ms[0] = ms / (float)ec->nb_launched;
    if (hipEventElapsedTime(&ms, h->ev[1], h->ev[2]) == hipSuccess) r->stage_ms[1] = ms;
    if (hipEventElapsedTime(&ms, h->ev[2], h->ev[3]) == hipSuccess) r->stage_ms[2] = ms;
    return SSF_OK;
}

static int process_oldest(ssf_handle* h, const float* prior, ssf_frame_result* out) {
    TimerScope ts(h);
    int rc = activate_oldest(h);
    if (rc) return rc;
    TrackFrame f;
    f.t_a = now_us();
    f.kf = h->seq_n > 0 ? h->seq_k : -1;
    if (f.kf >= 0 && f.kf < 64) { h->seq_mark_us[0][f.kf] = f.t_a - h->seq_t0_us; h->seq_mark_us[1][f.kf] = 0; }
    if (h->ctx.size() > 1 && hipEventQuery(h->cc->ctx->ev_done) == hipSuccess) h->host_us[4] += 1;
    f.timing = h->cfg.profile != 0 && h->cc->ctx->timed;
    if (f.timing) HCK(hipEventRecord(h->ev[1], h->stream));
    if (exchanges_natively(h)) { rc = comm_counts(h); if (rc) return rc; }
    icp_begin(h, prior);
    rc = h->bins.make_if_large(h);
    if (!rc) rc = icp_chains(h) ? icp_loop_chained(h, f) : icp_loop_plain(h, f);
    if (!rc) rc = icp_loop_end(h, f);
    ssf_frame_result r;
    if (!rc) rc = exchange_and_fuse(h, &r);
    if (rc) return rc;
    if (h->pending.empty()) h->ahead_tuner.sequence_break(); else h->ahead_tuner.frame_done(now_us(), r.icp_iters);
    h->host_us[1] += f.t_b - f.t_a; h->host_us[2] += now_us() - f.t_b; h->host_us[3] += 1;
    if (f.timing) { rc = stage_times(h, &r); if (rc) return rc; }
    if (out) *out = r;
    return SSF_OK;
}
static int process_frame_impl(ssf_handle* h, const void* rgb, const void* depth, int on_device, const float* prior,
                              const uint8_t* mask, ssf_frame_result* out, const uint8_t* pixmask = nullptr, int pixmask_on_device = -1) {
    if (!frame_args_ok(h, rgb, depth, on_device)) return SSF_ERR_INVALID_ARG;
    if (!h->pending.empty()) { h->err = "frames are pending in the extract pipeline: use ssf_process_submitted"; return SSF_ERR_STATE; }
    int rc;
    { TimerScope ts(h); rc = submit_extract(h, rgb, depth, on_device, mask, pixmask, pixmask_on_device < 0 ? on_device : pixmask_on_device); }
    return rc ? rc : process_oldest(h, prior, out);
}

namespace ssf {
bool frame_inputs_ok(ssf_handle* h, const void* rgb, const void* depth, int on_device) { return frame_args_ok(h, rgb, depth, on_device); }
int process_frame_devmask(ssf_handle* h, const void* rgb, const void* depth, int on_device, const float* prior, const uint8_t* d_pixmask,
                          ssf_frame_result* out) {
    return process_frame_impl(h, rgb, depth, on_device ? 1 : 0, prior, nullptr, out, d_pixmask, 1);
}
int copy_rows(ssf_handle* h, const ssf_surfels& dst, size_t d0, const ssf_surfels& src, size_t s0, size_t n, hipMemcpyKind kind) {
    if (n == 0) return SSF_OK;
    auto one = [&](auto* d, const auto* s, size_t w) { return d ? hipMemcpyAsync(d + w * d0, s + w * s0, 4 * w * n, kind, h->stream) : hipSuccess; };
    HCK(one(dst.positions, src.positions, 3)); HCK(one(dst.colors, src.colors, 3)); HCK(one(dst.stamps, src.stamps, 2));
    HCK(one(dst.orientations, src.orientations, 9)); HCK(one(dst.shapes, src.shapes, 6)); HCK(one(dst.dims, src.dims, 2));
    HCK(one(dst.confidences, src.confidences, 1));
    return SSF_OK;
}
static ssf_surfels soa_surfels(const SurfelSoA& s) { return ssf_surfels{s.pos, s.col, s.stamps, nullptr, s.shape, s.dims, s.conf}; }
ModelView model_view(const ssf_handle* h, bool visible_only) {
    ModelView mv;
    mv.vis = h->model[h->mcur]; mv.oov = h->oov[h->ocur];
    mv.n_visible = h->n_visible; mv.nbv = (h->n_visible + 255) / 256; mv.nvs = 256 * mv.nbv;
    mv.oov_head = h->oov_head; mv.oov_tail = h->oov_tail;
    mv.nbo = visible_only ? 0 : (h->oov_tail - h->oov_head + 255) / 256;
    mv.nslots = 256 * (mv.nbv + mv.nbo);
    return mv;
}
int model_at_rest(ssf_handle* h, const char* who, const char* lacks) {
    if (!h->pending.empty() || h->fusing) { h->err = "frames are pending in the extract pipeline"; return SSF_ERR_STATE; }
    if (who && h->cfg.nranks > 1) { h->err = std::string(who) + ": a sharded handle (cfg.nranks > 1) " + lacks; return SSF_ERR_STATE; }
    return SSF_OK;
}
int align_loop(ssf_handle* h, const float* d_pos, const float* d_lab, const float* d_nrm, const float* d_conf, int n, long long* d_out,
               const float* init_pose, float* rel_pose, int* valid, int* iters, int* pairs_last) {
    hipStream_t st = h->stream;
    int rc = SSF_OK;
    M3 R_init = m3_identity(); V3 t_init = v3(0, 0, 0);
    if (init_pose) { const Rt p0 = pose_from12(init_pose); R_init = p0.R; t_init = p0.t; }
    double tf_inc[16], JtJ[36];
    for (int i = 0; i < 16; i++) tf_inc[i] = (i % 5 == 0) ? 1.0 : 0.0;
    for (int i = 0; i < 36; i++) JtJ[i] = 0.0;
    M3 R_inc = m3_identity(); V3 t_inc = v3(0, 0, 0);
// ... 95 lines not shown
        for (auto q : h->up->p_rgb) if (q) (void)hipHostFree(q);
        for (auto q : h->up->p_depth) if (q) (void)hipHostFree(q);
        for (auto q : h->up->p_mask) if (q) (void)hipHostFree(q);
        delete h->up; h->up = nullptr;
    }
    for (auto& c : h->ctx) if (c.stream) (void)hipStreamSynchronize(c.stream);
    if (h->stream) (void)hipStreamSynchronize(h->stream);
    for (auto& c : h->ctx) if (c.deal_comm) { RcclApi* api = rccl_api(); if (api) (void)api->CommDestroy(c.deal_comm); c.deal_comm = nullptr; }
    if (h->comm) { RcclApi* api = rccl_api(); if (api) (void)api->CommDestroy(h->comm); h->comm = nullptr; }
    for (void* q : h->p2p.opened) (void)hipIpcCloseMemHandle(q);
    if (h->p2p.region) (void)hipFree(h->p2p.region);
    for (auto& c : h->ctx) {
        for (int n = 0; n <= SSF_MAX_BATCH; n++) { if (c.exec[n]) (void)hipGraphExecDestroy(c.exec[n]); if (c.graph[n]) (void)hipGraphDestroy(c.graph[n]); }
        for (int n = 0; n <= SSF_MAX_BATCH; n++) { if (c.exec_pm[n]) (void)hipGraphExecDestroy(c.exec_pm[n]); if (c.graph_pm[n]) (void)hipGraphDestroy(c.graph_pm[n]); }
        hipEvent_t evs[4] = {c.ev_done, c.ev_consumed, c.ev_t0, c.ev_t1};
        for (hipEvent_t e : evs) if (e) (void)hipEventDestroy(e);
        if (c.own_stream && c.stream) stream_pool().give(c.stream, h->cfg.device_id, c.stream_prio);
    }
    if (h->capture_stream) stream_pool().give(h->capture_stream, h->cfg.device_id, StreamPool::CAPTURE);
    if (!h->guarded.empty() && !SSF_ENV_SET("GUARD_ONLY")) check_guards(h);
    for (void* p : h->allocs) (void)hipFree(p);
    if (h->mb_host) (void)hipHostFree(h->mb_host);
    for (int i = 0; i < 4; i++) if (h->ev[i]) (void)hipEventDestroy(h->ev[i]);
    for (auto& r : h->timer.pool_free) { (void)hipEventDestroy(r.e0); (void)hipEventDestroy(r.e1); }
    if (h->own_stream && h->stream) { (void)hipStreamSynchronize(h->stream); stream_pool().give(h->stream, h->cfg.device_id, h->stream_prio); }
    delete h;
}

int ssf_create(const ssf_config* cfg, ssf_handle** out) {
    if (!cfg || !out) { g_create_err = "null argument"; return SSF_ERR_INVALID_ARG; }
    if (cfg->width <= 0 || cfg->height <= 0 || cfg->cell_size <= 0 || cfg->nb_samples <= 0 || cfg->nb_samples > 64 ||
        cfg->nb_supersurfels_max <= 0 || cfg->nranks < 1 || cfg->rank < 0 || cfg->rank >= cfg->nranks) {
        g_create_err = "invalid configuration"; return SSF_ERR_INVALID_ARG;
    }
    int ndev = 0;
    if (hipGetDeviceCount(&ndev) != hipSuccess || ndev <= 0) {
        g_create_err = "no HIP device: libssf_hip.so needs a gfx950 GPU (there is no CPU fallback)";
        return SSF_ERR_NO_DEVICE;
    }
    if (cfg->device_id < 0 || cfg->device_id >= ndev) { g_create_err = "device_id out of range"; return SSF_ERR_INVALID_ARG; }
    if (hipSetDevice(cfg->device_id) != hipSuccess) { g_create_err = "hipSetDevice failed"; return SSF_ERR_DEVICE; }
    ssf_handle* h = new (std::nothrow) ssf_handle();
    if (!h) return SSF_ERR_DEVICE;
    h->cfg = *cfg;
    const int W = cfg->width, H = cfg->height, c = cfg->cell_size;
    h->gx = (W + c - 1) / c; h->gy = (H + c - 1) / c; h->S = h->gx * h->gy;
    if (cfg->nb_supersurfels_max < h->S) { delete h; g_create_err = "nb_supersurfels_max < nbSuperpixels"; return SSF_ERR_INVALID_ARG; }
#ifndef SSF_MOVE_TOTALS_DEFAULT
#define SSF_MOVE_TOTALS_DEFAULT 1
#endif
    h->move_totals_on = SSF_ENV_INT("MOVE_TOTALS", SSF_MOVE_TOTALS_DEFAULT) != 0;
    h->icp_ahead_mode = SSF_ENV_INT("ICP_AHEAD", 1);
    h->icp_ahead = h->icp_ahead_mode != 0;
    h->ahead_tuner.forced = SSF_ENV_INT("ICP_AHEAD", -1);
    h->icp_chain = SSF_ENV_INT("ICP_CHAIN", 1) != 0;
    if (SSF_ENV_SET("NO_GRAPH")) h->graph_failed = true;
    if (cfg->stream) h->stream = (hipStream_t)cfg->stream;
    else {
        int least = 0, greatest = 0;
        (void)hipDeviceGetStreamPriorityRange(&least, &greatest);
        const int prio = SSF_ENV_INT("TRACK_PRIORITY", greatest);
        h->stream = stream_pool().take(cfg->device_id, prio);
        if (!h->stream) { delete h; g_create_err = "hipStreamCreate failed"; return SSF_ERR_DEVICE; }
        h->own_stream = true; h->stream_prio = prio;
    }
    SegParams& p = h->seg;
    p.W = W; p.H = H; p.cell = c; p.gx = h->gx; p.gy = h->gy; p.S = h->S; p.nb_samples = cfg->nb_samples;
    p.min_size = (int)((float)(c * c) / 4.f);
    p.lambda_pos = cfg->lambda_pos; p.lambda_bound = cfg->lambda_bound; p.lambda_size = cfg->lambda_size;
    p.lambda_disp = cfg->lambda_disp; p.thresh_disp = cfg->thresh_disp;
    p.filter_alpha = cfg->filter_alpha; p.filter_beta = cfg->filter_beta; p.filter_threshold = cfg->filter_threshold;
    p.filter_iter = cfg->filter_iter; p.seed = cfg->rng_seed;
    p.inv_gx = 1.0f / (float)h->gx;
    p.cell_magic = c > 1 ? (uint32_t)((0x100000000ull + (uint64_t)c - 1) / (uint64_t)c) : 0u;
    p.win_cells_max = tile_window_cells_max(p);
    h->cam.fx = cfg->fx; h->cam.fy = cfg->fy; h->cam.cx = cfg->cx; h->cam.cy = cfg->cy; h->cam.W = W; h->cam.H = H;
    h->classify = ClassifyArgs{h->cam, nullptr, cfg->delta_t, cfg->conf_thresh, cfg->range_min, cfg->range_max};
    h->shard = ShardArgs{cfg->rank, cfg->nranks, 0, cfg->shard_tile};
    const size_t P = (size_t)W * H, S = h->S, N = cfg->nb_supersurfels_max, NS = S * cfg->nb_samples;
    const size_t NT32 = (size_t)((W + 30 + 31) / 32) * ((H + 31) / 32), NT64 = (size_t)((W + 62 + 63) / 64) * ((H + 31) / 32);
    const size_t NT = std::max(NT32, 2 * NT64);
    const int nctx = std::max(0, std::min(cfg->pipeline_depth, SSF_MAX_PIPELINE_DEPTH)) + 1;
    h->batch = std::max(1, std::min(cfg->extract_batch, SSF_MAX_BATCH));
    h->ctx.resize(nctx);
    h->pass_team = SSF_ENV_INT("PASS_TEAM", 0) != 0;
    bool ok = dalloc(h, &h->d_srgb_lut, 256) && dalloc(h, &h->d_tickets, 512);
    {
        const int ne = pass_geometry_entries(W, H);
        std::vector<uint2> tab((size_t)ne);
        p.pass_geom = nullptr; p.pass_ntile = ne / 2;
        pass_geometry_table(p, tab.data());
        uint2* d_geom = nullptr;
        ok = ok && dalloc(h, &d_geom, (size_t)ne) && hipMemcpy(d_geom, tab.data(), (size_t)ne * sizeof(uint2), hipMemcpyHostToDevice) == hipSuccess;
        if (ok) p.pass_geom = d_geom;
    }
    auto carve = [&](ExtractCtx& c, char* base) -> size_t {
        size_t off = 0;
        auto take = [&](auto*& ptr, size_t count) {
            using T = typename std::remove_reference<decltype(*ptr)>::type;
            off = (off + 255) & ~(size_t)255;
            ptr = reinterpret_cast<T*>(base + off);
            off += std::max<size_t>(count, 1) * sizeof(T);
        };
        FrameMaps& m = c.maps;
        take(m.rgba, P); take(m.disp, P); take(m.label, P); take(m.inlier, P); take(m.plane_depth, P);
        take(m.sp, S); take(m.samples, NS); take(m.sample_score, NS); take(m.moments, 13 * S); take(m.filt, 11 * S); take(m.epoch, 64); take(m.pix2, P); take(m.fpack, 4 * S);
        for (int b = 0; b < 2; b++) take(m.sums[b].r, S);
        for (int b = 0; b < 3; b++) { take(m.log.ent[b], NT * 256); take(m.log.disp[b], NT * 256); take(m.log.count[b], NT); }
        SurfelSoA& f = c.frame;
        take(f.pos, 3 * S); take(f.col, 3 * S); take(f.lab, 3 * S); take(f.stamps, 2 * S); take(f.r0, 3 * S); take(f.r1, 3 * S);
        take(f.r2, 3 * S); take(f.shape, 6 * S); take(f.dims, 2 * S); take(f.conf, S);
        take(c.d_best, S); take(c.d_matched, S); take(c.d_rgb_in, 4 * P); take(c.d_depth_in, P); take(c.d_depth_filt, P); take(c.d_mask, S);
        take(c.d_wire, 26 * S);
        take(c.d_pixmask, P); take(c.d_pixcnt, 2 * S);
        return (off + 255) & ~(size_t)255;
    };
    size_t slab_bytes = 0;
    for (int ci = 0; ci < nctx && ok; ci++) {
        ExtractCtx& c = h->ctx[ci];
        slab_bytes = carve(c, nullptr);
        char* base = nullptr;
        ok = dalloc(h, &base, slab_bytes * h->batch);
        if (!ok) break;
        (void)carve(c, base);
        FrameMaps& m = c.maps;
        m.slab = slab_bytes;
        m.srgb_lut = h->d_srgb_lut;
        (void)hipMemsetAsync(base, 0, slab_bytes * h->batch, h->stream);
        if (nctx == 1) c.stream = h->stream;
        else {
            int least = 0, greatest = 0;
            (void)hipDeviceGetStreamPriorityRange(&least, &greatest);
            static const bool ctx0_up = SSF_ENV_INT("CTX0_PRIORITY", 1) != 0;
            const int prio = (ci == 0 && ctx0_up && least - greatest >= 2) ? least - 1 : least;
            c.stream = stream_pool().take(h->cfg.device_id, prio); ok = c.stream != nullptr; c.own_stream = ok; c.stream_prio = prio;
        }
        if (ok && h->pass_team) {
            const int kmax = 4 * std::max(cfg->seg_iter, 0);
            std::vector<char> tab(pass_args_bytes(std::max(kmax, 1)));
// ... 487 lines not shown
    return SSF_OK;
}

int ssf_get_frame_device(ssf_handle* h, ssf_surfels* o, int* n) {
    if (!h || !o) return SSF_ERR_INVALID_ARG;
    if (!h->cc || !h->cc->frame.pos) { h->err = "no frame has been processed yet"; return SSF_ERR_STATE; }
    if (!h->d_frame_orient9 && !dalloc(h, &h->d_frame_orient9, 9 * (size_t)h->S)) { h->err = "allocation failed"; return SSF_ERR_DEVICE; }
    const SurfelSoA& s = h->cc->frame;
    launch_pack_orient(h->stream, s, h->S, h->d_frame_orient9);
    HCK(hipGetLastError());
    HCK(hipStreamSynchronize(h->stream));
    *o = soa_surfels(s); o->orientations = h->d_frame_orient9;
    if (n) *n = h->S;
    return SSF_OK;
}
int ssf_get_preview_image(ssf_handle* h, uint8_t* o) {
    if (!h || !o) return SSF_ERR_INVALID_ARG;
    const size_t P = (size_t)h->cfg.width * h->cfg.height;
    uint8_t* d = reinterpret_cast<uint8_t*>(h->d_scratch_map);
    launch_preview(h->stream, h->cfg.width, h->cfg.height, h->cc->maps.label, h->cc->maps.rgba, d);
    HCK(hipGetLastError());
    return copy_map(h, o, d, 3 * P);
}

int ssf_export_model_txt(ssf_handle* h, const char* path) {
    if (!h || !path) return SSF_ERR_INVALID_ARG;
    const int n = h->n_model;
    std::vector<float> pos(3 * (size_t)n), col(3 * (size_t)n), ori(9 * (size_t)n), shp(6 * (size_t)n), dims(2 * (size_t)n), conf(n);
    std::vector<int32_t> stamps(2 * (size_t)n);
    ssf_surfels o = {pos.data(), col.data(), stamps.data(), ori.data(), shp.data(), dims.data(), conf.data()};
    int rc = materialise(h);
    if (!rc) rc = copy_out(h, h->dense, 0, n, &o);
    if (rc) return rc;
    FILE* f = std::fopen(path, "w");
    if (!f) { h->err = "cannot open file"; return SSF_ERR_IO; }
    for (int i = 0; i < n; i++) {
        if (!(conf[i] > h->cfg.conf_thresh)) continue;
        std::fprintf(f, "%d %d %f\n", stamps[2 * i], stamps[2 * i + 1], conf[i]);
        std::fprintf(f, "%f %f %f\n", pos[3 * i], pos[3 * i + 1], pos[3 * i + 2]);
        std::fprintf(f, "%f %f %f\n", col[3 * i], col[3 * i + 1], col[3 * i + 2]);
        std::fprintf(f, "%f %f\n", dims[2 * i], dims[2 * i + 1]);
        const float* q = &ori[9 * (size_t)i];
        std::fprintf(f, "%f %f %f %f %f %f %f %f %f\n", q[0], q[1], q[2], q[3], q[4], q[5], q[6], q[7], q[8]);
        const float* c = &shp[6 * (size_t)i];
        std::fprintf(f, "%f %f %f %f %f %f\n\n", c[0], c[1], c[2], c[3], c[4], c[5]);
    }
    std::fclose(f);
    return SSF_OK;
}

int ssf_apply_deformation(ssf_handle* h, const float* np, const float* nr, const float* nt, int m, const float* w4, const int32_t* idx4) {
    if (!h || !np || !nr || !nt || !w4 || !idx4 || m <= 0) return SSF_ERR_INVALID_ARG;
    drop_shard_sizes(h);
    h->ahead.valid = false;
    const size_t n = h->n_model;
    if (n == 0) return SSF_OK;
    float *d_np, *d_nr, *d_nt, *d_w, *d_nodes; int32_t* d_i;
    DevTemps tmp;
    HCK(tmp.take(&d_np, 12 * (size_t)m)); HCK(tmp.take(&d_nr, 36 * (size_t)m)); HCK(tmp.take(&d_nt, 12 * (size_t)m));
    HCK(tmp.take(&d_nodes, 64 * (size_t)m));
    HCK(tmp.take(&d_w, 16 * n)); HCK(tmp.take(&d_i, 16 * n));
    hipStream_t st = h->stream;
    HCK(hipMemcpyAsync(d_np, np, 12 * (size_t)m, hipMemcpyHostToDevice, st));
    HCK(hipMemcpyAsync(d_nr, nr, 36 * (size_t)m, hipMemcpyHostToDevice, st));
    HCK(hipMemcpyAsync(d_nt, nt, 12 * (size_t)m, hipMemcpyHostToDevice, st));
    HCK(hipMemcpyAsync(d_w, w4, 16 * n, hipMemcpyHostToDevice, st));
    HCK(hipMemcpyAsync(d_i, idx4, 16 * n, hipMemcpyHostToDevice, st));
    return deform_dense(h, m, d_np, d_nr, d_nt, d_nodes, d_w, d_i);
}

int ssf_bilateral_filter(ssf_handle* h, const void* in, void* out, int on_device) {
    if (!h || !in || !out) return SSF_ERR_INVALID_ARG;
    const size_t P = (size_t)h->cfg.width * h->cfg.height;
    const void* d_in = in; float* d_out = (float*)out;
    if (on_device && (!device_input_aligned(h, nullptr, in) || (uintptr_t)out % 4)) return SSF_ERR_INVALID_ARG;
    if (!on_device) { HCK(hipMemcpyAsync(h->d_bf_in, in, depth_bpp(h) * P, hipMemcpyHostToDevice, h->stream)); d_in = h->d_bf_in; d_out = h->d_bf_out; }
    { TimerScope ts(h); launch_bilateral(h->stream, d_in, h->in_depth, h->in_scale, d_out, h->cfg.width, h->cfg.height, h->cfg.prefilter_sigma_color, h->cfg.prefilter_sigma_space); }
    if (!on_device) HCK(hipMemcpyAsync(out, d_out, 4 * P, hipMemcpyDeviceToHost, h->stream));
    HCK(hipStreamSynchronize(h->stream));
    if (h->cfg.profile == 1) timer_collect(&h->timer);
    return SSF_OK;
}
int ssf_get_kernel_times(ssf_handle* h, const char** names, double* ms, int64_t* calls, int max_k) {
    if (!h || !names || !ms || !calls) return 0;
    h->timer_names.clear();
    for (auto& kv : h->timer.acc) h->timer_names.push_back(kv.first);
    int k = 0;
    for (auto& nm : h->timer_names) {
        if (k >= max_k) break;
        names[k] = nm.c_str(); ms[k] = h->timer.acc[nm].first; calls[k] = h->timer.acc[nm].second; k++;
    }
    return k;
}
int ssf_reset_kernel_times(ssf_handle* h) { if (!h) return SSF_ERR_INVALID_ARG; h->timer.acc.clear(); return SSF_OK; }
int ssf_set_profile(ssf_handle* h, int enable) {
    if (!h) return SSF_ERR_INVALID_ARG;
    h->cfg.profile = enable;
    if (enable == 1) timer_calibrate(&h->timer, h->stream);
    return SSF_OK;
}

int ssf_sequence_marks(ssf_handle* h, double* out320) {
    if (!h || !out320) return SSF_ERR_INVALID_ARG;
    for (int m = 0; m < 4; m++) for (int i = 0; i < 64; i++) out320[m * 64 + i] = h->seq_mark_us[m][i];
    for (int i = 0; i < 32; i++) { out320[256 + 2 * i] = i < h->seq_launches ? h->seq_launch_us[i] : -1.0; out320[257 + 2 * i] = i < h->seq_launches ? h->seq_launch_n[i] + h->seq_launch_host_us[i] / 1e4 : 0; }
    return SSF_OK;
}
long long ssf_waiter_matches(ssf_handle* h) { return h ? h->n_waiter_matches : -1; }
int ssf_tuner_state(ssf_handle* h, double* out4) {
    if (!h || !out4) return SSF_ERR_INVALID_ARG;
    const AheadTuner& t = h->ahead_tuner;
    out4[0] = t.current(); out4[1] = t.frames; out4[2] = t.n[0] ? t.sum[0] / t.n[0] : 0.0; out4[3] = t.n[1] ? t.sum[1] / t.n[1] : 0.0;
    return SSF_OK;
}
long long ssf_waiter_match_repairs(ssf_handle* h) { return h ? h->n_waiter_match_repairs : -1; }
int ssf_sequence_times(ssf_handle* h, double* out64) {
    if (!h || !out64) return SSF_ERR_INVALID_ARG;
    for (int i = 0; i < 64; i++) out64[i] = h->seq_done_us[i];
    return SSF_OK;
}

double ssf_stream_copy_rate(int mib, int reps) {
    if (mib < 256 || reps < 1) return -1.0;
    const size_t bytes = ((size_t)mib << 20) & ~(size_t)((1u << 28) - 1u), n = bytes / sizeof(f4v);
    if (bytes == 0) return -1.0;
    f4v *a = nullptr, *b = nullptr;
    if (hipMalloc(&a, bytes) != hipSuccess || hipMalloc(&b, bytes) != hipSuccess) { (void)hipGetLastError(); (void)hipFree(a); return -1.0; }
    (void)hipMemset(a, 1, bytes); (void)hipMemset(b, 0, bytes);
    hipEvent_t e0, e1; (void)hipEventCreate(&e0); (void)hipEventCreate(&e1);
    double best = 0.0;
    for (int form = 0; form < 6; form++) {
        for (int r = 0; r < reps + 2; r++) {
            (void)hipEventRecord(e0, 0);
            const dim3 grid_stride(256 * 32), blk(256);
            switch (form) {
                case 0: hipLaunchKernelGGL((k_stream_copy<4, false, false>), grid_stride, blk, 0, 0, a, b, n); break;
                case 1: hipLaunchKernelGGL((k_stream_copy<4, true, false>), grid_stride, blk, 0, 0, a, b, n); break;
                case 2: hipLaunchKernelGGL((k_stream_copy<8, true, false>), grid_stride, blk, 0, 0, a, b, n); break;
                case 3: hipLaunchKernelGGL((k_stream_copy<4, true, true>), dim3((unsigned int)(n / (256 * 4))), blk, 0, 0, a, b, n); break;
                case 4: hipLaunchKernelGGL((k_stream_copy<8, true, true>), dim3((unsigned int)(n / (256 * 8))), blk, 0, 0, a, b, n); break;
                default: hipLaunchKernelGGL((k_stream_copy<8, false, true>), dim3((unsigned int)(n / (256 * 8))), blk, 0, 0, a, b, n); break;
            }
            (void)hipEventRecord(e1, 0);
            (void)hipEventSynchronize(e1);
            float ms = 0.f; (void)hipEventElapsedTime(&ms, e0, e1);
            if (r >= 2 && ms > 0.f) best = std::max(best, 2.0 * (double)bytes / (ms * 1e-3) / 1e9);
        }
    }
    (void)hipGetLastError();
    (void)hipEventDestroy(e0); (void)hipEventDestroy(e1); (void)hipFree(a); (void)hipFree(b);
    return best;
}

int ssf_pooled_streams(void) {
    StreamPool& sp = stream_pool();
    std::lock_guard<std::mutex> lk(sp.mu);
    int n = 0;
    for (auto& kv : sp.idle) n += (int)kv.second.size();
    return n;
}
int ssf_upload_stats(ssf_handle* h, double* out6) {
    if (!h || !out6) return SSF_ERR_INVALID_ARG;
    for (int i = 0; i < 6; i++) out6[i] = 0.0;
    if (h->up) {
        out6[0] = Uploader::NTH; out6[1] = (double)h->up->frames_done.load(); out6[2] = (double)h->up->us_ring.load();
// ... 10 lines not shown
```

supersurfel_fusion_amd/csrc/ssf_track_fuse.hip:

```cpp
#include <stdlib.h>
#include <algorithm>
#include "ssf_slots.hpp"

namespace ssf {

__device__ __forceinline__ long long wsum64(long long v) {
#pragma unroll
    for (int o = 32; o > 0; o >>= 1) v += __shfl_xor(v, o, 64);
    return v;
}
__device__ __forceinline__ V3 ld3(const float* __restrict__ p, size_t i) { return v3(p[3 * i], p[3 * i + 1], p[3 * i + 2]); }
__device__ __forceinline__ void st3(float* __restrict__ p, size_t i, V3 v) { p[3 * i] = v.x; p[3 * i + 1] = v.y; p[3 * i + 2] = v.z; }
__device__ __forceinline__ Sym3 ld6(const float* __restrict__ p, size_t i) {
    return sym3(p[6 * i], p[6 * i + 1], p[6 * i + 2], p[6 * i + 3], p[6 * i + 4], p[6 * i + 5]);
}
__device__ __forceinline__ void st6(float* __restrict__ p, size_t i, Sym3 c) {
    p[6 * i] = c.xx; p[6 * i + 1] = c.xy; p[6 * i + 2] = c.xz; p[6 * i + 3] = c.yy; p[6 * i + 4] = c.yz; p[6 * i + 5] = c.zz;
}

#ifndef ICP_SLOTS
#define ICP_SLOTS 16
#endif
template <bool UNIFORM, typename Emit>
__device__ __forceinline__ void icp_row_terms_(const Cam& cam, const uint2* __restrict__ pix2, const float4* __restrict__ fpack,
// ... 624 lines not shown
__device__ __forceinline__ int classify_values(const Cam& cam, float conf, int last_seen, const V3& pos, const Rt& pose,
                                               const float* __restrict__ plane_depth, int stamp, int delta_t, float conf_thresh,
                                               float zmin, float zmax) {
    const ClsPre r = classify_pre(cam, conf, last_seen, pos, pose, stamp, delta_t, conf_thresh, zmin, zmax);
    return r.st >= 0 ? r.st : classify_post(r, plane_depth[r.pix]);
}
__device__ __forceinline__ int classify_row(const Cam& cam, const SurfelSoA& M, size_t idx, const Rt& pose,
                                            const float* __restrict__ plane_depth, int stamp, int delta_t, float conf_thresh,
                                            float zmin, float zmax) {
    const int st = classify_values(cam, M.conf[idx], M.stamps[2 * idx + 1], ld3(M.pos, idx), pose, plane_depth, stamp, delta_t,
                                   conf_thresh, zmin, zmax);
    if (st == 2) M.conf[idx] = -1.0f;
    return st;
}
#ifndef OOV_PER_WG
#define OOV_PER_WG 4
#endif
__device__ __forceinline__ void classify_oov_block(const Cam& cam, const OovStore& O, const Rt& pose, const float* __restrict__ plane_depth,
                                                   int stamp, int delta_t, float conf_thresh, float zmin, float zmax,
                                                   uint8_t* __restrict__ state_oov, uint32_t* __restrict__ bc_oov, PartitionWs ws,
                                                   const Counters* __restrict__ cnt, int wg, int nb_oov) {
    __shared__ int h2[OOV_PER_WG][4][2];
    const int wv = threadIdx.x >> 6;
    const long long head = cnt->oov_head, tail = cnt->oov_tail;
    int cls[OOV_PER_WG];
    uint8_t lv[OOV_PER_WG]; float conf[OOV_PER_WG]; int seen[OOV_PER_WG]; V3 pos[OOV_PER_WG]; ClsPre pre[OOV_PER_WG]; float z[OOV_PER_WG];
    bool in[OOV_PER_WG];
#pragma unroll
    for (int j = 0; j < OOV_PER_WG; j++) {
        const long long phys = head + ((long long)wg * OOV_PER_WG + j) * 256  + threadIdx.x;
        in[j] = phys < tail;
        const size_t q = (size_t)(in[j] ? phys : tail - 1);
        lv[j] = O.live[q]; conf[j] = O.rows.conf[q]; seen[j] = O.rows.stamps[2 * q + 1]; pos[j] = ld3(O.rows.pos, q);
    }
#pragma unroll
    for (int j = 0; j < OOV_PER_WG; j++) {
        int lvj = lv[j];
        asm volatile("" : "+v"(lvj), "+v"(conf[j]), "+v"(seen[j]), "+v"(pos[j].x), "+v"(pos[j].y), "+v"(pos[j].z));
        lv[j] = in[j] ? (uint8_t)lvj : (uint8_t)0;
    }
#pragma unroll
    for (int j = 0; j < OOV_PER_WG; j++) {
        pre[j] = classify_pre(cam, conf[j], seen[j], pos[j], pose, stamp, delta_t, conf_thresh, zmin, zmax);
        if (!lv[j]) { pre[j].st = 7; pre[j].pix = 0; }
        if (pre[j].st >= 0) pre[j].pix = 0;
    }
#pragma unroll
    for (int j = 0; j < OOV_PER_WG; j++) z[j] = plane_depth[pre[j].pix];
#pragma unroll
    for (int j = 0; j < OOV_PER_WG; j++) asm volatile("" : "+v"(z[j]));
#pragma unroll
    for (int j = 0; j < OOV_PER_WG; j++) {
        cls[j] = classify_post(pre[j], z[j]);
        if (lv[j]) {
            const long long phys = head + ((long long)wg * OOV_PER_WG + j) * 256  + threadIdx.x;
            if (cls[j] == 2) O.rows.conf[phys] = -1.0f;
            state_oov[phys] = (uint8_t)cls[j];
        }
    }
#pragma unroll
    for (int j = 0; j < OOV_PER_WG; j++) {
        const int k0 = __popcll(__ballot(cls[j] == 0)), k2 = __popcll(__ballot(cls[j] == 2));
        if (lane() == 0) { h2[j][wv][0] = k0; h2[j][wv][1] = k2; }
    }
    __syncthreads();
    if (threadIdx.x < 2 * OOV_PER_WG) {
        const int j = threadIdx.x >> 1, which = threadIdx.x & 1, ob = wg * OOV_PER_WG + j;
        const uint32_t k = h2[j][0][which] + h2[j][1][which] + h2[j][2][which] + h2[j][3][which];
        if (ob < nb_oov) {
            const uint32_t other = __shfl_xor(k, 1, 64);
            if (which == 0) bc_oov[ob] = k | (other << 16);
            if (k) {
                atomic_add_done(&ws.tot[(ob & (PART_REPLICAS - 1)) * 8 + 6 + which], k);
                if (which == 0) atomicAdd(&ws.sup_oov[ob / PART_GROUP], k);
            }
        }
    }
}
#define UPD_PER_WG 32
__device__ __forceinline__ int tile_owner(const V3& pw, int nranks, float tile);
__device__ __forceinline__ float pick3(const V3& v, int k) { return k == 0 ? v.x : (k == 1 ? v.y : v.z); }
__device__ __forceinline__ void update_group(SurfelSoA M, SurfelSoA F, Rt pose, int stamp, long long id_offset, int n_visible,
                                             const unsigned long long* __restrict__ best, const uint8_t* __restrict__ matched,
                                             int S, Counters* cnt, int f0, const ClassifyArgs& ca, uint8_t* __restrict__ state_vis,
                                             PartitionWs ws, const ShardArgs& sh) {
    const int wv = threadIdx.x >> 6, l = lane();
    if (wv == 3) return;
    const int f = wv == 0 ? f0 + (l >> 1) : f0 + (wv - 1) * 16 + (l >> 2);
    if (f >= S) return;
    unsigned int mt = matched[f];
    unsigned long long bk = best[f];
    float f_conf = F.conf[f];
    V3 f_pos = v3(0.f, 0.f, 0.f), f_lab = v3(0.f, 0.f, 0.f);
    Sym3 f_shape = sym3(0.f, 0.f, 0.f, 0.f, 0.f, 0.f);
    if (wv == 0) { f_pos = ld3(F.pos, f); f_shape = ld6(F.shape, f); } else f_lab = ld3(F.lab, f);
    asm volatile("" : "+v"(mt), "+v"(bk), "+v"(f_conf), "+v"(f_pos.x), "+v"(f_shape.xx), "+v"(f_lab.x));
    if (!mt || bk == SSF_NO_MATCH) return;
    const long long local = (long long)(uint32_t)(bk & 0xFFFFFFFFull) - id_offset;
    if (local < 0 || local >= n_visible) return;
    const size_t m = (size_t)local;
    float m_conf = M.conf[m];
    V3 model_position = v3(0.f, 0.f, 0.f), model_lab = v3(0.f, 0.f, 0.f);
    Sym3 model_shape = sym3(0.f, 0.f, 0.f, 0.f, 0.f, 0.f);
    if (wv == 0) { model_position = ld3(M.pos, m); model_shape = ld6(M.shape, m); } else model_lab = ld3(M.lab, m);
    asm volatile("" : "+v"(m_conf), "+v"(model_position.x), "+v"(model_shape.xx), "+v"(model_lab.x));
    const float ratio = 1.0f / (m_conf + f_conf);
    if (wv == 0) {
// ... 111 lines not shown
    if (flag && base_total + before + r < capacity) {
        const V3 f_pos = ld3(F.pos, f), f_col = ld3(F.col, f), f_lab = ld3(F.lab, f);
        const V3 f_r0 = ld3(F.r0, f), f_r1 = ld3(F.r1, f), f_r2 = ld3(F.r2, f);
        const Sym3 f_shape = ld6(F.shape, f);
        const float f_d0 = F.dims[2 * f], f_d1 = F.dims[2 * f + 1];
        const float new_conf = F.conf[f];
        const V3 new_pos = add(m3_mulv(R, f_pos), t);
        const int st = classify_values(ca.cam, new_conf, stamp, new_pos, pose, ca.plane_depth, stamp, ca.delta_t, ca.conf_thresh,
                                       ca.zmin, ca.zmax);
        st3(M.pos, k, new_pos);
        M.conf[k] = st == 2 ? -1.0f : new_conf;
        st3(M.col, k, f_col);
        st3(M.lab, k, f_lab);
        M.stamps[2 * k] = stamp; M.stamps[2 * k + 1] = stamp;
        M.dims[2 * k] = f_d0; M.dims[2 * k + 1] = f_d1;
        st3(M.r0, k, row_mul(f_r0, Rt_));
        st3(M.r1, k, row_mul(f_r1, Rt_));
        st3(M.r2, k, row_mul(f_r2, Rt_));
        st6(M.shape, k, rot_sym(R, f_shape));
        state_vis[k] = (uint8_t)st;
        atomicAdd(&s_cls[(k >> 8) / PART_GROUP - g_first][st], 1u);
    }
    __syncthreads();
    if (threadIdx.x < 6) {
        const int seg = threadIdx.x / 3, st = threadIdx.x % 3;
        const uint32_t n = s_cls[seg][st];
        if (n) {
            atomicAdd(&ws.sup_vis[(g_first + seg) * 6 + 3 + st], n);
            atomic_add_done(&ws.tot[(chunk & (PART_REPLICAS - 1)) * 8 + 3 + st], n);
        }
    }
    if (chunk == nchunks - 1 && threadIdx.x == 0)
        atomic_store_done(&cnt->n_inserted, min(base_total + before + total, capacity) - base_total);
}
__device__ __forceinline__ Counters finalise_counters(Counters* cnt, Counters c, int shrink_by_removed, int keep_inserted = 0);
__device__ __forceinline__ void mailbox_counters(const Counters& c, Mailbox* mb, unsigned long long seq);
__device__ __forceinline__ Counters frame_counters(const Counters& c_in, const uint32_t* tot) {
    const int a0 = (int)tot[0], a1 = (int)tot[1], a2 = (int)tot[2], c0 = (int)tot[3], c1 = (int)tot[4], c2 = (int)tot[5];
    const int b0 = (int)tot[6], b2 = (int)tot[7], b1 = c_in.oov_live - b0 - b2;
    Counters c = c_in;
    c.n_model = c_in.n_model + c_in.n_inserted;
    c.n_state0 = a0 + b0 + c0; c.n_state1 = a1 + b1 + c1; c.n_state2 = a2 + b2 + c2;
    c.n_visible = a0 + b0 + c0; c.n_removed = (a2 + b2 + c2) - c_in.n_emigrated;
    c.mv_nv = c_in.n_visible; c.mv_a0 = a0; c.mv_b0 = b0; c.mv_nc = c_in.n_inserted;
    c.mv_head_old = c_in.oov_head; c.mv_tail_old = c_in.oov_tail; c.mv_head_new = c_in.oov_head - a1;
    c.oov_head = c_in.oov_head - a1; c.oov_tail = c_in.oov_tail + c1;
    c.oov_live = (c_in.oov_live - b0 - b2) + a1 + c1;
    return c;
}
#ifdef SSF_EXPERIMENTS
__device__ unsigned long long* g_fuse_trace = nullptr;
void set_fuse_trace(unsigned long long* p) { (void)hipMemcpyToSymbol(HIP_SYMBOL(g_fuse_trace), &p, sizeof(p)); }
#endif
__global__ __launch_bounds__(256) void k_update_insert(SurfelSoA M, SurfelSoA F, Rt pose, int stamp, long long id_offset,
                                                       int n_visible, const unsigned long long* __restrict__ best,
                                                       const uint8_t* __restrict__ matched, const int32_t* __restrict__ cand, int S,
                                                       int do_update, int capacity, int rank, int nranks, float tile, Counters* cnt,
                                                       int nupd, int nchunks, int nb_vis, int nb_oov, OovStore O, ClassifyArgs ca,
                                                       uint8_t* __restrict__ state_vis, uint8_t* __restrict__ state_oov,
                                                       uint32_t* __restrict__ bc_oov, PartitionWs ws, int migrate, int tail_in_move) {
    __builtin_amdgcn_s_setprio(3);
    __shared__ int wave_tot[16];
    __shared__ int hist[4][6];
    __shared__ int s_last;
    __shared__ uint32_t tot[8];
    const int b = blockIdx.x;
#ifdef SSF_EXPERIMENTS
    unsigned long long* const trace = g_fuse_trace;
    if (trace && threadIdx.x == 0) trace[3 * (size_t)b] = wall_clock64();
#endif
    if (b >= nupd + nchunks + nb_vis)
        classify_oov_block(ca.cam, O, pose, ca.plane_depth, stamp, ca.delta_t, ca.conf_thresh, ca.zmin, ca.zmax, state_oov, bc_oov,
                           ws, cnt, b - nupd - nchunks - nb_vis, nb_oov);
    else if (b >= nupd + nchunks) {
        const int vb = b - nupd - nchunks, i = vb * blockDim.x + threadIdx.x, wv = threadIdx.x >> 6;
        int cls = 7;
        if (i < n_visible) {
            int f = cand[i];
            float conf = M.conf[i]; int seen = M.stamps[2 * (size_t)i + 1]; V3 pos = ld3(M.pos, (size_t)i);
            asm volatile("" : "+v"(f), "+v"(conf), "+v"(seen), "+v"(pos.x));
            const bool rewritten = do_update && f >= 0 && (uint32_t)(best[f] & 0xFFFFFFFFull) == (uint32_t)(id_offset + i);
            if (!rewritten) {
                cls = classify_values(ca.cam, conf, seen, pos, pose, ca.plane_depth, stamp, ca.delta_t, ca.conf_thresh, ca.zmin, ca.zmax);
                if (cls == 2) M.conf[i] = -1.0f;
                state_vis[i] = (uint8_t)cls;
            }
        }
#pragma unroll
        for (int c = 0; c < 3; c++) { const int k = __popcll(__ballot(cls == c)); if (lane() == 0) hist[wv][c] = k; }
        __syncthreads();
        if (threadIdx.x < 3) {
            const uint32_t k = hist[0][threadIdx.x] + hist[1][threadIdx.x] + hist[2][threadIdx.x] + hist[3][threadIdx.x];
            if (k) {
                atomicAdd(&ws.sup_vis[(vb / PART_GROUP) * 6 + threadIdx.x], k);
                atomic_add_done(&ws.tot[(vb & (PART_REPLICAS - 1)) * 8 + threadIdx.x], k);
            }
        }
    } else if (b >= nupd)
        insert_chunk(M, F, pose, stamp, matched, S, capacity, rank, nranks, tile, cnt, wave_tot, b - nupd, nchunks, ca, state_vis, ws);
    else if (do_update) {
        ShardArgs sh; sh.rank = rank; sh.nranks = nranks; sh.migrate = (migrate && nranks > 1) ? 1 : 0; sh.tile = tile;
        update_group(M, F, pose, stamp, id_offset, n_visible, best, matched, S, cnt, b * UPD_PER_WG, ca, state_vis, ws, sh);
    }
#ifdef SSF_EXPERIMENTS
    if (trace) {
        __syncthreads();
        if (threadIdx.x == 0) trace[3 * (size_t)b + 1] = wall_clock64();
        asm volatile("s_waitcnt vmcnt(0) lgkmcnt(0)" ::: "memory");
        __syncthreads();
        if (threadIdx.x == 0) trace[3 * (size_t)b + 2] = wall_clock64();
    }
#endif
    if (tail_in_move) return;
    asm volatile("s_waitcnt vmcnt(0)" ::: "memory");
    __syncthreads();
    if (threadIdx.x == 0) s_last = grid_arrive(ws.ticket);
    __syncthreads();
    if (!s_last) return;
    if (threadIdx.x < 8) {
        uint32_t v = 0;
#pragma unroll
        for (int r = 0; r < PART_REPLICAS; r++) v += __hip_atomic_load(&ws.tot[r * 8 + threadIdx.x], __ATOMIC_RELAXED, __HIP_MEMORY_SCOPE_AGENT);
        tot[threadIdx.x] = v;
    }
    __syncthreads();
    if (threadIdx.x >= 64) {
        for (int i = threadIdx.x - 64; i < ws.words; i += blockDim.x - 64) ws.other[i] = 0u;
    } else if (threadIdx.x == 0) {
        Counters c_in = *cnt;
        c_in.n_inserted = __hip_atomic_load(&cnt->n_inserted, __ATOMIC_RELAXED, __HIP_MEMORY_SCOPE_AGENT);
        c_in.n_updated = __hip_atomic_load(&cnt->n_updated, __ATOMIC_RELAXED, __HIP_MEMORY_SCOPE_AGENT);
        c_in.n_emigrated = __hip_atomic_load(&cnt->n_emigrated, __ATOMIC_RELAXED, __HIP_MEMORY_SCOPE_AGENT);
        cnt[1] = finalise_counters(cnt, frame_counters(c_in, tot), 1);
    }
}

__global__ __launch_bounds__(1024) void k_first_frame(SurfelSoA M, SurfelSoA F, Rt pose, int S, int capacity, int rank,
                                                      int nranks, float tile, Counters* cnt) {
    __shared__ int wave_tot[16];
    int running = 0;
    for (int c0 = 0; c0 < S; c0 += 1024) {
        const int f = c0 + threadIdx.x;
        const bool flag = (f < S) && shard_owner(F, f, pose, nranks, tile) == rank;
        int total;
        const int r = block_rank_1024(flag, wave_tot, total);
        const int k = running + r;
        if (flag && k < capacity) {
            st3(M.pos, k, ld3(F.pos, f)); st3(M.col, k, ld3(F.col, f)); st3(M.lab, k, ld3(F.lab, f));
            M.stamps[2 * k] = F.stamps[2 * f]; M.stamps[2 * k + 1] = F.stamps[2 * f + 1];
            st3(M.r0, k, ld3(F.r0, f)); st3(M.r1, k, ld3(F.r1, f)); st3(M.r2, k, ld3(F.r2, f));
            st6(M.shape, k, ld6(F.shape, f));
            M.dims[2 * k] = F.dims[2 * f]; M.dims[2 * k + 1] = F.dims[2 * f + 1];
            M.conf[k] = F.conf[f];
        }
        running += total;
    }
    if (threadIdx.x == 0) {
        const int n = min(running, capacity);
        cnt->n_model = n; cnt->n_visible = n; cnt->n_inserted = 0; cnt->n_removed = 0;
    }
}

struct RowRegs { V3 pos, col, lab, r0, r1, r2; Sym3 shape; int s0, s1; float d0, d1, conf; };
__device__ __forceinline__ RowRegs load_row(const SurfelSoA& A, size_t i) {
    RowRegs r;
    r.pos = ld3(A.pos, i); r.col = ld3(A.col, i); r.lab = ld3(A.lab, i);
    r.s0 = A.stamps[2 * i]; r.s1 = A.stamps[2 * i + 1];
    r.r0 = ld3(A.r0, i); r.r1 = ld3(A.r1, i); r.r2 = ld3(A.r2, i);
    r.shape = ld6(A.shape, i);
    r.d0 = A.dims[2 * i]; r.d1 = A.dims[2 * i + 1];
    r.conf = A.conf[i];
    return r;
}
__device__ __forceinline__ void store_row(const SurfelSoA& B, size_t j, const RowRegs& r) {
    st3(B.pos, j, r.pos); st3(B.col, j, r.col); st3(B.lab, j, r.lab);
    B.stamps[2 * j] = r.s0; B.stamps[2 * j + 1] = r.s1;
    st3(B.r0, j, r.r0); st3(B.r1, j, r.r1); st3(B.r2, j, r.r2);
    st6(B.shape, j, r.shape);
    B.dims[2 * j] = r.d0; B.dims[2 * j + 1] = r.d1;
    B.conf[j] = r.conf;
}
__device__ __forceinline__ void copy_row(const SurfelSoA& A, size_t i, const SurfelSoA& B, size_t j) { store_row(B, j, load_row(A, i)); }
__device__ __forceinline__ void copy_row_keep(const SurfelSoA& A, size_t i, const SurfelSoA& B, size_t j, V3& pos, V3& lab, V3& nrm) {
    const RowRegs r = load_row(A, i);
    pos = r.pos; lab = r.lab; nrm = r.r2;
    store_row(B, j, r);
}
template <bool ICP, bool P2P>
__global__ __launch_bounds__(256) void k_move_rows(SurfelSoA V, SurfelSoA Vn, OovStore O, const uint8_t* __restrict__ state_vis,
                                                   const uint8_t* __restrict__ state_oov,
                                                   const uint32_t* __restrict__ bc_oov, PartitionWs ws,
                                                   Counters* cnt, int nb_vis, NextIcp nx, Mailbox* mb,
                                                   unsigned long long cnt_seq, P2PView pv, MoveTotals mt) {
    __builtin_amdgcn_s_setprio(3);
    if (blockIdx.x == 0 && threadIdx.x == 255) {
        Counters c;
        if (mt.from_tot) {
            uint32_t tot[8];
#pragma unroll
            for (int k = 0; k < 8; k++) {
                uint32_t v = 0;
#pragma unroll
                for (int r = 0; r < PART_REPLICAS; r++) v += __builtin_nontemporal_load(&ws.tot[r * 8 + k]);
                tot[k] = v;
            }
            const Counters c_in = *cnt;
            c = finalise_counters(cnt, frame_counters(c_in, tot), 1, 1);
            cnt[1] = c;
        } else {
            int w[sizeof(Counters) / sizeof(int)];
            const int* src = reinterpret_cast<const int*>(&cnt[1]);
#pragma unroll
            for (int i = 0; i < (int)(sizeof(Counters) / sizeof(int)); i++) w[i] = __builtin_nontemporal_load(&src[i]);
            __builtin_memcpy(&c, w, sizeof(c));
        }
        mailbox_counters(c, mb, cnt_seq);
    }
    if (mt.from_tot && blockIdx.x == 0 && threadIdx.x >= 64 && threadIdx.x < 255)
        for (int i = threadIdx.x - 64; i < ws.words; i += 191) ws.other[i] = 0u;
    if ((int)blockIdx.x >= nb_vis && bc_oov[blockIdx.x - nb_vis] == 0u) return;
    __shared__ uint32_t s_tot[8];
    if (mt.from_tot && threadIdx.x < 8) {
        uint32_t v = 0;
#pragma unroll
        for (int r = 0; r < PART_REPLICAS; r++) v += ws.tot[r * 8 + threadIdx.x];
        s_tot[threadIdx.x] = v;
    }
    const int mv_nv = mt.from_tot ? mt.nv : cnt->mv_nv, mv_nc = mt.from_tot ? cnt->n_inserted : cnt->mv_nc;
    const int mv_head_old = mt.from_tot ? mt.head_old : cnt->mv_head_old, mv_tail_old = mt.from_tot ? mt.tail_old : cnt->mv_tail_old;
    auto mv_a0 = [&]() -> int { return mt.from_tot ? (int)s_tot[0] : cnt->mv_a0; };
    auto mv_b0 = [&]() -> int { return mt.from_tot ? (int)s_tot[6] : cnt->mv_b0; };
    auto mv_head_new = [&]() -> int { return mt.from_tot ? mt.head_old - (int)s_tot[1] : cnt->mv_head_new; };
    auto new_n_visible = [&]() -> int { return mt.from_tot ? (int)(s_tot[0] + s_tot[6] + s_tot[3]) : cnt->n_visible; };
    __shared__ int hist[4][6];
    __shared__ uint32_t base[6];
    __shared__ unsigned long long red[ICP ? 29 * ICP_SLOTS : 1];
    if (ICP) for (int i = threadIdx.x; i < 29 * ICP_SLOTS; i += blockDim.x) red[i] = 0ull;
    if (threadIdx.x < 6) base[threadIdx.x] = 0u;
    const int wv = threadIdx.x >> 6;
    int cls = 7, in_wave = 0;
    bool keep = false;
    V3 pos, lab, nrm;
    if ((int)blockIdx.x < nb_vis) {
        const int nv = mv_nv, n_rows = nv + mv_nc;
        const int i = blockIdx.x * blockDim.x + threadIdx.x;
        RowRegs row;
        if (i < n_rows) {
            int st = (int)state_vis[i];
            row = load_row(V, i);
            asm volatile("" : "+v"(st), "+v"(row.pos.x));
            cls = (i < nv ? 0 : 3) + st;
        }
        const int g0 = (int)(blockIdx.x / PART_GROUP), ng = 6 * g0;
        const int row0 = g0 * PART_GROUP * 256, n16 = 16 * ((int)blockIdx.x - g0 * PART_GROUP);
        __syncthreads();
        for (int w = threadIdx.x; w < ng; w += blockDim.x) {
            const uint32_t v = ws.sup_vis[w];
            if (v) atomicAdd(&base[w % 6], v);
        }
        uint32_t pa0 = 0, pa1 = 0, pc0 = 0, pc1 = 0;
        for (int q = threadIdx.x; q < n16; q += blockDim.x) {
            const int r0 = row0 + 16 * q;
            if (r0 < n_rows) {
                const uint4 sv = *reinterpret_cast<const uint4*>(state_vis + r0);
                const uint32_t wd[4] = {sv.x, sv.y, sv.z, sv.w};
                uint32_t a0 = 0, a1 = 0, c0 = 0, c1 = 0;
#pragma unroll
                for (int j = 0; j < 16; j++) {
                    const int rr = r0 + j;
                    const uint32_t stt = (wd[j >> 2] >> (8 * (j & 3))) & 0xFFu;
                    const bool in = rr < n_rows, old = rr < nv;
                    a0 += (in && old && stt == 0u) ? 1u : 0u; a1 += (in && old && stt == 1u) ? 1u : 0u;
                    c0 += (in && !old && stt == 0u) ? 1u : 0u; c1 += (in && !old && stt == 1u) ? 1u : 0u;
                }
                pa0 += a0; pa1 += a1; pc0 += c0; pc1 += c1;
            }
        }
#pragma unroll
        for (int o = 32; o > 0; o >>= 1) {
            pa0 += __shfl_xor(pa0, o, 64); pa1 += __shfl_xor(pa1, o, 64); pc0 += __shfl_xor(pc0, o, 64); pc1 += __shfl_xor(pc1, o, 64);
        }
        if (lane() == 0) {
            if (pa0) atomicAdd(&base[0], pa0);
            if (pa1) atomicAdd(&base[1], pa1);
            if (pc0) atomicAdd(&base[3], pc0);
            if (pc1) atomicAdd(&base[4], pc1);
        }
#pragma unroll
        for (int c = 0; c < 6; c++) {
            const unsigned long long mask = __ballot(cls == c);
            if (cls == c) in_wave = __popcll(mask & ((1ull << lane()) - 1ull));
            if (lane() == 0) hist[wv][c] = __popcll(mask);
        }
        __syncthreads();
        if (cls == 0 || cls == 1 || cls == 3 || cls == 4) {
            int before = 0;
            for (int w = 0; w < wv; w++) before += hist[w][cls];
            const size_t r = (size_t)base[cls] + before + in_wave;
            if (cls == 0 || cls == 3) {
                const size_t j = cls == 0 ? r : (size_t)mv_a0() + mv_b0() + r;
                store_row(Vn, j, row);
                if (ICP) { pos = row.pos; lab = row.lab; nrm = row.r2; keep = true; }
            } else {
                const size_t j = (cls == 1 ? (size_t)mv_head_new() : (size_t)mv_tail_old) + r;
                store_row(O.rows, j, row);
                O.live[j] = 1;
            }
        }
    } else {
        const int ob = blockIdx.x - nb_vis;
        const long long phys = (long long)mv_head_old + (long long)ob * blockDim.x + threadIdx.x;
        if (phys < mv_tail_old) {
            int lv = (int)O.live[phys], st = (int)state_oov[phys];
            asm volatile("" : "+v"(lv), "+v"(st));
            if (lv) cls = st;
        }
        const unsigned long long mask = __ballot(cls == 0);
        if (cls == 0) in_wave = __popcll(mask & ((1ull << lane()) - 1ull));
        if (lane() == 0) hist[wv][0] = __popcll(mask);
        if (__syncthreads_count(cls == 0)) {
            const int g0 = ob / PART_GROUP, nw = g0 + (ob - g0 * PART_GROUP);
            for (int w = threadIdx.x; w < nw; w += blockDim.x) {
                const uint32_t v = w < g0 ? ws.sup_oov[w] : (bc_oov[g0 * PART_GROUP + (w - g0)] & 0xFFFFu);
                if (v) atomicAdd(&base[0], v);
            }
            __syncthreads();
        }
        if (cls == 0) {
            int before = 0;
            for (int w = 0; w < wv; w++) before += hist[w][0];
            const size_t j = (size_t)mv_a0() + base[0] + before + in_wave;
            if (ICP) { copy_row_keep(O.rows, (size_t)phys, Vn, j, pos, lab, nrm); keep = true; }
            else copy_row(O.rows, (size_t)phys, Vn, j);
        }
        if (cls == 0 || cls == 2) O.live[phys] = 0;
    }
    if (ICP) {
        if (keep) icp_row(nx.cam, nx.pix2, nx.fpack, nx.T.R, nx.T.t, pos, lab, nrm, red, lane() & (ICP_SLOTS - 1), 0);
        const int nkeep = __syncthreads_count(keep);
        if (P2P && new_n_visible() == 0) {
            if (blockIdx.x == 0) icp_publish<true>(nx.replicas, nx.sums, nx.mb, nx.seq, pv, pv.seq);
            return;
        }
        const bool vis = (int)blockIdx.x < nb_vis;
        const int nbr = (mv_nv + mv_nc + 255) / 256;
        if (vis ? (int)blockIdx.x >= nbr : nkeep == 0) return;
        __shared__ int s_last;
        icp_fold(red, nx.replicas);
        if (threadIdx.x == 0) {
            SSF_ARRIVE_RELEASE();
            unsigned int rows = (unsigned int)nkeep;
            bool report = true;
            if (vis) {
                const unsigned int g = blockIdx.x & 63u, in_group = ((unsigned int)nbr - g + 63u) / 64u;
                unsigned long long* gw = reinterpret_cast<unsigned long long*>(nx.ticket + 128) + g;
                const unsigned long long before = __hip_atomic_fetch_add(gw, ((unsigned long long)rows << 32) | 1ull, __ATOMIC_RELAXED,
                                                                         __HIP_MEMORY_SCOPE_AGENT);
                report = (unsigned int)(before & 0xFFFFFFFFull) == in_group - 1;
                if (report) {
                    rows += (unsigned int)(before >> 32);
                    __hip_atomic_store(gw, 0ull, __ATOMIC_RELAXED, __HIP_MEMORY_SCOPE_AGENT);
                }
            }
            int last = 0;
            if (report) {
                const unsigned int total = (unsigned int)new_n_visible();
                const unsigned int before = rows ? __hip_atomic_fetch_add(&nx.ticket[65], rows, __ATOMIC_RELAXED, __HIP_MEMORY_SCOPE_AGENT) : 0u;
                last = rows != 0u && before + rows == total;
                if (last) __hip_atomic_store(&nx.ticket[65], 0u, __ATOMIC_RELAXED, __HIP_MEMORY_SCOPE_AGENT);
            }
            if (last) SSF_ARRIVE_ACQUIRE();
            s_last = last;
        }
        __syncthreads();
        if (s_last) icp_publish<P2P>(nx.replicas, nx.sums, nx.mb, nx.seq, pv, pv.seq);
    }
}

__global__ __launch_bounds__(256) void k_pack_emigrants(SurfelSoA M, const unsigned long long* __restrict__ best,
                                                        const uint8_t* __restrict__ matched, long long id_offset, int n_visible,
                                                        const uint8_t* __restrict__ state_vis, int S, int do_update, int nranks,
                                                        float tile, int32_t* __restrict__ table) {
    const int f = blockIdx.x * blockDim.x + threadIdx.x;
    if (f >= S) return;
    int32_t w[SSF_MIGRANT_WORDS];
#pragma unroll
    for (int i = 0; i < SSF_MIGRANT_WORDS; i++) w[i] = 0;
    if (do_update && matched[f] && best[f] != SSF_NO_MATCH) {
        const long long local = (long long)(uint32_t)(best[f] & 0xFFFFFFFFull) - id_offset;
        if (local >= 0 && local < n_visible) {
            const size_t m = (size_t)local;
            const float conf = M.conf[m];
            if (state_vis[m] == 2 && conf > 0.0f) {
                const RowRegs r = load_row(M, m);
                w[0] = tile_owner(r.pos, nranks, tile) + 1;
                const float v[26] = {r.pos.x, r.pos.y, r.pos.z, r.col.x, r.col.y, r.col.z, __int_as_float(r.s0), __int_as_float(r.s1),
                                     r.r0.x, r.r0.y, r.r0.z, r.r1.x, r.r1.y, r.r1.z, r.r2.x, r.r2.y, r.r2.z,
                                     r.shape.xx, r.shape.xy, r.shape.xz, r.shape.yy, r.shape.yz, r.shape.zz, r.d0, r.d1, r.conf};
#pragma unroll
                for (int i = 0; i < 26; i++) w[2 + i] = __float_as_int(v[i]);
            }
        }
    }
    int32_t* o = table + (size_t)SSF_MIGRANT_WORDS * f;
#pragma unroll
    for (int i = 0; i < SSF_MIGRANT_WORDS; i++) o[i] = w[i];
}
// ... 413 lines not shown
        const unsigned long long w0 = __hip_atomic_load(&src[0], __ATOMIC_RELAXED, __HIP_MEMORY_SCOPE_SYSTEM);
        if ((unsigned int)w0 == 0u) continue;
        own[0] += (int32_t)(unsigned int)w0; own[1] += (int32_t)(unsigned int)(w0 >> 32);
#pragma unroll
        for (int k = 1; k < SSF_MIGRANT_WORDS / 2; k++) {
            const unsigned long long w = __hip_atomic_load(&src[k], __ATOMIC_RELAXED, __HIP_MEMORY_SCOPE_SYSTEM);
            own[2 * k] += (int32_t)(unsigned int)w; own[2 * k + 1] += (int32_t)(unsigned int)(w >> 32);
        }
    }
}

int icp_variant_mode() {
    static const int mode = SSF_ENV_INT("ICP_WRED", 0) ? 2 : (SSF_ENV_INT("ICP_PER_LANE", 0) > 1 ? 1 : 0);
    return mode;
}
void launch_icp(hipStream_t st, const Cam& cam, SurfelSoA model, int n_visible, const uint2* pix2, const float4* fpack,
                Rt T, long long* replicas, unsigned int* ticket,
                long long* sums29, Mailbox* mb, unsigned long long seq, int dbg_arg, IcpGo* go, unsigned long long go_seq,
                const P2PView* pv, int by_tile, const MatchArgs* match) {
    ScopedKernel sk("icp_accumulate", st);
    const MatchArgs ma = match ? *match : MatchArgs{0.f, 0.f, 0, nullptr, nullptr, nullptr};
    const int mode = dbg_arg > 0 && dbg_arg != 4 ? 0 : icp_variant_mode();
    const int per_lane = mode == 1 ? std::max(2, SSF_ENV_INT("ICP_PER_LANE", 0)) : 1;
    const int per_block = 256 * per_lane;
    int grid = (n_visible + per_block - 1) / per_block;
    if (grid < 1) grid = 1;
    if (grid > 4096) grid = 4096;
    static const int counted = SSF_ENV_INT("ICP_COUNTED", 1);
    const int dbg = (dbg_arg < 0 ? 0 : dbg_arg) | ((counted && !pv && dbg_arg < 0) ? SSF_ICP_DBG_COUNTED : 0);
    const P2PView none{};
    const P2PView& v = pv ? *pv : none;
    if (by_tile && !pv) { hipLaunchKernelGGL((k_icp<false, 3>), dim3(grid), dim3(256), 0, st, cam, model, n_visible, pix2, fpack, T, replicas, ticket, sums29, mb, seq, dbg, go, go_seq, v, by_tile, ma); return; }
#ifdef SSF_EXPERIMENTS
    if (mode == 2 && !pv) { hipLaunchKernelGGL((k_icp<false, 2>), dim3(grid), dim3(256), 0, st, cam, model, n_visible, pix2, fpack, T, replicas, ticket, sums29, mb, seq, dbg, go, go_seq, v, by_tile, ma); return; }
    if (mode == 1 && pv) { hipLaunchKernelGGL((k_icp<true, 1>), dim3(grid), dim3(256), 0, st, cam, model, n_visible, pix2, fpack, T, replicas, ticket, sums29, mb, seq, dbg, go, go_seq, v, by_tile, ma); return; }
    if (mode == 1) { hipLaunchKernelGGL((k_icp<false, 1>), dim3(grid), dim3(256), 0, st, cam, model, n_visible, pix2, fpack, T, replicas, ticket, sums29, mb, seq, dbg, go, go_seq, v, by_tile, ma); return; }
#endif
    if (pv) hipLaunchKernelGGL((k_icp<true, 0>), dim3(grid), dim3(256), 0, st, cam, model, n_visible, pix2, fpack, T, replicas, ticket, sums29, mb, seq, dbg, go, go_seq, v, by_tile, ma);
    else hipLaunchKernelGGL((k_icp<false, 0>), dim3(grid), dim3(256), 0, st, cam, model, n_visible, pix2, fpack, T, replicas, ticket, sums29, mb, seq, dbg, go, go_seq, v, by_tile, ma);
}
void launch_match(hipStream_t st, const Cam& cam, SurfelSoA model, int n_visible, const uint2* pix2, const float4* fpack,
                  Rt pose, float zmin, float zmax, long long id_offset,
                  unsigned long long* best, uint8_t* matched, int32_t* cand, int S, const int32_t* orig) {
    (void)S;
    if (n_visible <= 0) return;
    ScopedKernel sk("match", st);
    if (orig) hipLaunchKernelGGL(k_match<true>, dim3((n_visible + 255) / 256), dim3(256), 0, st, cam, model, n_visible, pix2, fpack,
                                 pose, zmin, zmax, id_offset, best, matched, cand, orig);
    else hipLaunchKernelGGL(k_match<false>, dim3((n_visible + 255) / 256), dim3(256), 0, st, cam, model, n_visible, pix2, fpack,
                            pose, zmin, zmax, id_offset, best, matched, cand, orig);
}
void launch_fuse(hipStream_t st, SurfelSoA model, SurfelSoA frame, Rt pose, int stamp, long long id_offset, int n_visible,
                 const AssocTables& at, int do_update, int capacity, const ShardArgs& sh, Counters* cnt, OovStore oov, int span_upper,
                 const ClassifyArgs& ca, uint8_t* state_vis, uint8_t* state_oov, uint32_t* bc_oov, const PartitionWs& ws, int tail_in_move) {
    ScopedKernel sk("update_insert", st);
    const int S = at.S, nchunks = (S + 255) / 256, nb_oov = (span_upper + 255) / 256, nb_vis = (n_visible + 255) / 256;
    const int nupd = (S + UPD_PER_WG - 1) / UPD_PER_WG;
    hipLaunchKernelGGL(k_update_insert, dim3(nupd + nchunks + nb_vis + (nb_oov + OOV_PER_WG - 1) / OOV_PER_WG), dim3(256), 0, st, model,
                       frame, pose, stamp, id_offset,
                       n_visible, at.best, at.matched, at.cand, S, do_update, capacity, sh.rank, sh.nranks, sh.tile, cnt, nupd, nchunks, nb_vis,
                       nb_oov, oov, ca, state_vis, state_oov, bc_oov, ws, sh.migrate, tail_in_move);
}
void launch_pack_emigrants(hipStream_t st, SurfelSoA model, const AssocTables& at, long long id_offset, int n_visible,
                           const uint8_t* state_vis, int do_update, const ShardArgs& sh, int32_t* table) {
    ScopedKernel sk("pack_emigrants", st);
    hipLaunchKernelGGL(k_pack_emigrants, dim3((at.S + 255) / 256), dim3(256), 0, st, model, at.best, at.matched, id_offset, n_visible,
                       state_vis, at.S, do_update, sh.nranks, sh.tile, table);
}
void launch_migrate_in(hipStream_t st, SurfelSoA model, const int32_t* table, int S, int capacity, Counters* cnt, const ShardArgs& sh,
                       const ClassifyArgs& ca, Rt pose, int stamp, uint8_t* state_vis, const PartitionWs& ws) {
    ScopedKernel sk("migrate_in", st);
    hipLaunchKernelGGL(k_migrate_in, dim3(1), dim3(1024), 0, st, model, table, S, sh.rank, capacity, cnt, ca, pose, stamp, state_vis, ws);
}
void launch_first_frame(hipStream_t st, SurfelSoA model, SurfelSoA frame, Rt pose, int S, int capacity, const ShardArgs& sh, Counters* cnt) {
    ScopedKernel sk("first_frame", st);
    hipLaunchKernelGGL(k_first_frame, dim3(1), dim3(1024), 0, st, model, frame, pose, S, capacity, sh.rank, sh.nranks, sh.tile, cnt);
}
void launch_move_rows(hipStream_t st, SurfelSoA vis_src, SurfelSoA vis_dst, OovStore oov, int nv_upper, int span_upper,
                      const uint8_t* state_vis, const uint8_t* state_oov, const uint32_t* bc_oov, const PartitionWs& ws,
                      Counters* cnt, Mailbox* mb, unsigned long long cnt_seq, const NextIcp* next, const P2PView* next_pv,
                      const MoveTotals* totals) {
    const int nb_vis = std::max(1, (nv_upper + 255) / 256), nb_oov = (span_upper + 255) / 256;
    const MoveTotals mt = totals ? *totals : MoveTotals{0, 0, 0, 0};
    auto kernel = !next ? k_move_rows<false, false> : (next_pv ? k_move_rows<true, true> : k_move_rows<true, false>);
    ScopedKernel sk(next ? "reorder_move_icp" : "reorder_move", st);
    hipLaunchKernelGGL(kernel, dim3(nb_vis + nb_oov), dim3(256), 0, st, vis_src, vis_dst, oov, state_vis, state_oov, bc_oov, ws, cnt, nb_vis,
                       next ? *next : NextIcp{}, mb, cnt_seq, next_pv ? *next_pv : P2PView{}, mt);
}
void launch_oov_compact(hipStream_t st, OovStore src, OovStore dst, int span_upper, int new_head, uint32_t* bc_oov, Counters* cnt,
                        int set_span) {
    const int nb = (span_upper + 255) / 256;
    ScopedKernel sk("oov_compact", st);
    if (nb > 0) {
        hipLaunchKernelGGL(k_oov_count, dim3(nb), dim3(256), 0, st, src, bc_oov, cnt);
        hipLaunchKernelGGL(k_oov_scan, dim3(1), dim3(1024), 0, st, bc_oov, nb, cnt);
        hipLaunchKernelGGL(k_oov_compact, dim3(nb), dim3(256), 0, st, src, dst, bc_oov, new_head, cnt);
    }
    if (set_span) hipLaunchKernelGGL(k_oov_set_span, dim3(1), dim3(1), 0, st, cnt, new_head);
}
void launch_align(hipStream_t st, const Cam& cam, const float* spos, const float* slab, const float* snrm, const float* sconf,
                  int n, SurfelSoA frame, const int32_t* label, const float* plane_depth, Rt T, long long* out40) {
    ScopedKernel sk("align_iteration", st);
    hipLaunchKernelGGL(k_align, dim3(1), dim3(1024), 0, st, cam, spos, slab, snrm, sconf, n, frame, label, plane_depth, T, out40);
}
void launch_fern_codes(hipStream_t st, const uint8_t* rgb, const float* depth, int W, int H, const uint32_t* fpos,
                       const uint8_t* frgb, const float* fdepth, int n, uint8_t* codes) {
    if (n <= 0) return;
    hipLaunchKernelGGL(k_fern_codes, dim3((n + 63) / 64), dim3(64), 0, st, rgb, depth, W, H, fpos, frgb, fdepth, n, codes);
}
void launch_p2p_counts(hipStream_t st, const P2PView& pv, const Counters* cnt, Mailbox* mb, unsigned long long all_seq) {
    ScopedKernel sk("p2p_counts", st);
    hipLaunchKernelGGL(k_p2p_counts, dim3(1), dim3(64), 0, st, pv, cnt, mb, all_seq);
}
void launch_p2p_assoc(hipStream_t st, const P2PView& pv, unsigned long long* best, uint8_t* matched, Mailbox* mb) {
    ScopedKernel sk("p2p_assoc", st);
    hipLaunchKernelGGL(k_p2p_assoc, dim3(1), dim3(1024), 0, st, pv, best, matched, mb);
}
void launch_p2p_migrants(hipStream_t st, const P2PView& pv, int32_t* table, unsigned int* ticket, Mailbox* mb) {
    ScopedKernel sk("p2p_migrants", st);
    const int grid = (pv.S + 255) / 256;
    hipLaunchKernelGGL(k_p2p_migr_share, dim3(grid), dim3(256), 0, st, pv, table, ticket);
    hipLaunchKernelGGL(k_p2p_migr_gather, dim3(grid), dim3(256), 0, st, pv, table, mb);
}
void launch_publish_icp(hipStream_t st, const long long* rec, Mailbox* mb, unsigned long long seq) {
    hipLaunchKernelGGL(k_publish_icp, dim3(1), dim3(64), 0, st, rec, mb, seq);
}
void launch_publish_all_counts(hipStream_t st, const int* all5, int nranks, Mailbox* mb, unsigned long long seq) {
    hipLaunchKernelGGL(k_publish_all_counts, dim3(1), dim3(64), 0, st, all5, 5 * nranks, mb, seq);
}
void launch_publish_counts(hipStream_t st, Counters* cnt, int shrink_by_removed, Mailbox* mb, unsigned long long seq) {
    hipLaunchKernelGGL(k_publish_counts, dim3(1), dim3(1), 0, st, cnt, shrink_by_removed, mb, seq);
}
void launch_lab_refresh(hipStream_t st, SurfelSoA s, int n) {
    if (n <= 0) return;
    hipLaunchKernelGGL(k_lab_refresh, dim3((n + 255) / 256), dim3(256), 0, st, s, n);
}
void launch_deformation(hipStream_t st, SurfelSoA model, int n, int m, const float* npos, const float* nrot,
                        const float* ntrans, float* nodes16, const float* w4, const int32_t* idx4) {
    if (n <= 0) return;
    ScopedKernel sk("apply_deformation", st);
// ... 6 lines not shown
```

Measured before the change: 11630 frames/s.

## Fold next-frame ICP first iteration into fuse kernel with residual pass in move_rows

Moves the first ICP iteration for the next pending frame out of the move_rows pass and into the update_insert (fuse) kernel. A small set of extra workgroups in move_rows (a new ICP template mode) covers the residual rows. The adaptive AheadTuner, which flipped ahead-ICP on and off by measuring timings, is removed and the fused path is now the default mode. Stats counters and an ssf_ahead_stats API are added. The aim is to overlap ICP work with fusion and cut redundant row traversal, at the cost of more complex kernels and different reduction coverage.

```diff
diff --git a/include/ssf_track.h b/include/ssf_track.h
--- /dev/null
+++ b/include/ssf_track.h
@@ -0,0 +1,15 @@
+#ifndef SSF_TRACK_H
+#define SSF_TRACK_H
+
+#include "ssf.h"
+
+#ifdef __cplusplus
+extern "C" {
+#endif
+
+int ssf_ahead_stats(ssf_handle* h, long long out4[4]);
+
+#ifdef __cplusplus
+}
+#endif
+#endif
diff --git a/supersurfel_fusion_amd/binding.py b/supersurfel_fusion_amd/binding.py
--- a/supersurfel_fusion_amd/binding.py
+++ b/supersurfel_fusion_amd/binding.py
@@ -78,6 +78,7 @@
 KEYFRAMES_MAX_CANDIDATES = 8
 FERN_DTYPE = np.dtype([("x", np.uint16), ("y", np.uint16), ("r", np.uint8), ("g", np.uint8), ("b", np.uint8), ("pad", np.uint8),
                        ("depth_mm", np.uint32)])
+TRACK_SYMBOLS = ["ssf_ahead_stats"]
 QUERY_SYMBOLS = ["ssf_query_default_params", "ssf_query_count", "ssf_query_rows"]
 QUERY_REGIONS = {"all": 0, "sphere": 1, "box": 2, "frustum": 3}
 NAVGRID_SYMBOLS = ["ssf_navgrid_default_params", "ssf_navgrid_default_pose", "ssf_navgrid_build"]
@@ -320,6 +321,9 @@
         if self.has_render:
             L.ssf_render_default_params.argtypes = [vp, C.POINTER(SsfRenderParams)]
             L.ssf_render_model.argtypes = [vp, C.POINTER(SsfRenderParams), vp, vp, vp, vp, vp, C.POINTER(SsfRenderStats)]
+        self.has_track = all(hasattr(L, nm) for nm in TRACK_SYMBOLS)
+        if self.has_track:
+            L.ssf_ahead_stats.argtypes = [vp, C.POINTER(C.c_longlong)]
         self.has_query = all(hasattr(L, nm) for nm in QUERY_SYMBOLS)
         if self.has_query:
             L.ssf_query_default_params.argtypes = [vp, C.POINTER(SsfQueryParams)]
@@ -801,6 +805,13 @@
                  "ssf_process_frame_odometry")
         return res
 
+    def ahead_stats(self):
+        if not self.L.has_track:
+            raise SsfError("%s does not export ssf_ahead_stats (include/ssf_track.h, HIP product only)" % self.L.path)
+        out = (C.c_longlong * 4)()
+        self._ck(self.L.lib.ssf_ahead_stats(self.h, out), "ssf_ahead_stats")
+        return dict(fused=int(out[0]), separate=int(out[1]), dropped=int(out[2]), residual_rows=int(out[3]))
+
     def _need_query(self, symbol):
         if not self.L.has_query:
             raise SsfError("%s does not export %s: it does not query the model (include/ssf_query.h, HIP product only)"
diff --git a/supersurfel_fusion_amd/csrc/ssf_device.hpp b/supersurfel_fusion_amd/csrc/ssf_device.hpp
--- a/supersurfel_fusion_amd/csrc/ssf_device.hpp
+++ b/supersurfel_fusion_amd/csrc/ssf_device.hpp
@@ -202,10 +202,12 @@
 #define PART_GROUP 16
 #define PART_REPLICAS 8
 struct PartitionWs { uint32_t* sup_vis; uint32_t* sup_oov; uint32_t* tot; uint32_t* ticket; uint32_t* other; int words; };
+struct FuseIcp { int on; const uint2* pix2; const float4* fpack; Rt T; long long* replicas; unsigned int* ticket; };
 void launch_fuse(hipStream_t st, SurfelSoA model , SurfelSoA frame, Rt pose, int stamp, long long id_offset,
                  int n_visible, const AssocTables& at, int do_update, int capacity, const ShardArgs& sh, Counters* cnt, OovStore oov,
                  int span_upper, const ClassifyArgs& ca, uint8_t* state_vis, uint8_t* state_oov, uint32_t* bc_oov, const PartitionWs& ws,
-                 int tail_in_move = 0 );
+                 int tail_in_move = 0 ,
+                 const FuseIcp* ahead = nullptr);
 #ifdef SSF_EXPERIMENTS
 void set_pass_stats(int on);
 void set_pass_trace(unsigned long long* device_words );
@@ -225,10 +227,12 @@
     Rt T;
     long long* replicas; unsigned int* ticket; long long* sums; Mailbox* mb; unsigned long long seq;
 };
+#define SSF_MOVE_ICP_WG 16
+struct IcpResidual { const unsigned long long* best; const uint8_t* matched; int S; long long id_offset; unsigned int* rows_out; };
 void launch_move_rows(hipStream_t st, SurfelSoA vis_src, SurfelSoA vis_dst, OovStore oov, int nv_upper, int span_upper,
                       const uint8_t* state_vis, const uint8_t* state_oov, const uint32_t* bc_oov, const PartitionWs& ws,
                       Counters* cnt , Mailbox* mb, unsigned long long cnt_seq, const NextIcp* next,
-                      const struct P2PView* next_pv = nullptr, const MoveTotals* totals = nullptr);
+                      const struct P2PView* next_pv = nullptr, const MoveTotals* totals = nullptr, const IcpResidual* residual = nullptr);
 void launch_oov_compact(hipStream_t st, OovStore src, OovStore dst, int span_upper, int new_head, uint32_t* bc_oov, Counters* cnt,
                         int set_span);
 struct ModelView { SurfelSoA vis; OovStore oov; int n_visible, nbv, nvs, oov_head, oov_tail, nbo, nslots; };
diff --git a/supersurfel_fusion_amd/csrc/ssf_graph.hip b/supersurfel_fusion_amd/csrc/ssf_graph.hip
--- a/supersurfel_fusion_amd/csrc/ssf_graph.hip
+++ b/supersurfel_fusion_amd/csrc/ssf_graph.hip
@@ -370,7 +370,7 @@
     if (!h || !nr || !nt) return SSF_ERR_INVALID_ARG;
     { int rc = graph_usable(h, "ssf_graph_apply"); if (rc) return rc; }
     drop_shard_sizes(h);
-    h->ahead.valid = false;
+    h->drop_ahead();
     const GraphWs& g = h->graph;
     const size_t m = g.m;
     float *d_nr, *d_nt, *d_nodes;
diff --git a/supersurfel_fusion_amd/csrc/ssf_graph_solve.hip b/supersurfel_fusion_amd/csrc/ssf_graph_solve.hip
--- a/supersurfel_fusion_amd/csrc/ssf_graph_solve.hip
+++ b/supersurfel_fusion_amd/csrc/ssf_graph_solve.hip
@@ -500,7 +500,7 @@
     if (!h) return SSF_ERR_INVALID_ARG;
     { int rc = solved_usable(h, "ssf_graph_apply_solved"); if (rc) return rc; }
     drop_shard_sizes(h);
-    h->ahead.valid = false;
+    h->drop_ahead();
     const GraphWs& g = h->graph;
     float* d_nodes;
     DevTemps tmp;
diff --git a/supersurfel_fusion_amd/csrc/ssf_handle.hpp b/supersurfel_fusion_amd/csrc/ssf_handle.hpp
--- a/supersurfel_fusion_amd/csrc/ssf_handle.hpp
+++ b/supersurfel_fusion_amd/csrc/ssf_handle.hpp
@@ -17,6 +17,7 @@
 #include "../../include/ssf_motion.h"
 #include "../../include/ssf_odometry.h"
 #include "../../include/ssf_navgrid.h"
+#include "../../include/ssf_track.h"
 
 struct ncclComm; typedef struct ncclComm* ncclComm_t;
 struct Uploader;
@@ -31,28 +32,6 @@
 };
 }
 using namespace ssf;
-
-struct AheadTuner {
-    static const int START = 48, PROBE = 16, ROUNDS = 3, HOLD = 1024, SKIP = 2;
-    int forced = -1;
-    int mode = 0, frames = 0, left = START, round = 0, since_switch = 0;
-    bool probing = false;
-    double sum[2] = {0, 0}; int n[2] = {0, 0};
-    double last_done_us = -1.0; int last_mode = 0;
-    int current() const { return forced >= 0 ? (forced ? 1 : 0) : mode; }
-    void sequence_break() { last_done_us = -1.0; }
-    void frame_done(double t_us, int iters) {
-        if (forced >= 0) return;
-        if (last_done_us >= 0.0 && since_switch >= SKIP && probing && iters > 0) { sum[last_mode] += (t_us - last_done_us) / (double)(iters + 4); n[last_mode]++; }
-        last_done_us = t_us; last_mode = mode; frames++; since_switch++;
-        if (--left > 0) return;
-        if (!probing) { probing = true; round = 0; sum[0] = sum[1] = 0; n[0] = n[1] = 0; mode ^= 1; left = PROBE; since_switch = 0; return; }
-        if (++round < 2 * ROUNDS) { mode ^= 1; left = PROBE; since_switch = 0; return; }
-        probing = false;
-        if (n[0] > 0 && n[1] > 0) mode = (sum[1] / n[1] < sum[0] / n[0]) ? 1 : 0;
-        left = HOLD; since_switch = 0;
-    }
-};
 
 struct IcpLoop {
     bool active = false, valid = true, done = true;
@@ -244,10 +223,12 @@
     long long* d_icp_replicas = nullptr; unsigned int* d_tickets = nullptr; float* d_srgb_lut = nullptr;
     Mailbox* mb_host = nullptr; Mailbox* mb_dev = nullptr;
     unsigned long long icp_seq = 0, cnt_seq = 0;
-    struct { bool valid = false; unsigned long long seq = 0; ExtractCtx* ctx = nullptr; int slot = 0; int stamp = 0; Rt pose; } ahead;
+    struct { bool valid = false, from_fuse = false; unsigned long long seq = 0; ExtractCtx* ctx = nullptr; int slot = 0; int stamp = 0; Rt pose; } ahead;
+    bool fuse_ahead = false; NextIcp fuse_next{}; unsigned int* d_ahead_rows = nullptr;
+    long long n_ahead_fused = 0, n_ahead_separate = 0, n_ahead_dropped = 0;
+    void drop_ahead() { if (ahead.valid) { ahead.valid = false; n_ahead_dropped++; } }
     double wait_launched_us = 0.0; long long n_waiter_match_repairs = 0; long long dbg_stall_before_match_us = 0;
     bool icp_ahead = true; int icp_ahead_mode = 1;
-    AheadTuner ahead_tuner;
     IcpGo* go = nullptr; bool icp_chain = true; unsigned long long go_count = 0;
     bool graph_failed = false; hipStream_t capture_stream = nullptr;
     TileCopy bins;
diff --git a/supersurfel_fusion_amd/csrc/ssf_host.hip b/supersurfel_fusion_amd/csrc/ssf_host.hip
--- a/supersurfel_fusion_amd/csrc/ssf_host.hip
+++ b/supersurfel_fusion_amd/csrc/ssf_host.hip
@@ -541,9 +541,11 @@
     IcpLoop& I = h->icp;
     I.ahead_seq = 0;
     if (h->ahead.valid && !prior && h->have_frame && h->active.ctx == h->ahead.ctx && h->active.slot == h->ahead.slot &&
-        h->stamp == h->ahead.stamp && std::memcmp(&h->pose, &h->ahead.pose, sizeof(Rt)) == 0) I.ahead_seq = h->ahead.seq;
-    h->ahead.valid = false;
+        h->stamp == h->ahead.stamp && std::memcmp(&h->pose, &h->ahead.pose, sizeof(Rt)) == 0) { I.ahead_seq = h->ahead.seq; h->ahead.valid = false; }
+    h->drop_ahead();
     I.active = total_visible(h) > 0 && h->cfg.icp_iter > 0;
+    if (I.active && I.ahead_seq && h->ahead.from_fuse) h->n_ahead_fused++;
+    else if (I.active && !I.ahead_seq) h->n_ahead_separate++;
     I.valid = true; I.done = !I.active; I.iter = 0;
     icp_start_from(I, h->pose);
     for (int i = 0; i < 36; i++) I.JtJ[i] = 0.0;
@@ -725,7 +727,7 @@
     return SSF_OK;
 }
 int store_from_dense(ssf_handle* h, int n, int n_visible) {
-    h->ahead.valid = false;
+    h->drop_ahead();
     h->bins.drop();
     h->model_gen++;
     int rc = copy_soa(h, h->model[h->mcur], h->dense, (size_t)n_visible);
@@ -757,7 +759,30 @@
     return SSF_OK;
 }
 
-static int fuse_begin(ssf_handle* h, int migrate) {
+static inline bool icp_chains(const ssf_handle* h);
+static int next_icp_if_ready(ssf_handle* h, bool from_fuse, NextIcp* next, bool* have) {
+    *have = false;
+    if (!(h->icp_ahead && icp_is_one_launch(h) && h->cfg.icp_iter > 0 && !h->pending.empty())) return SSF_OK;
+    ExtractCtx& nc = h->ctx[h->pending.front().first];
+    const int nslot = h->pending.front().second;
+    const bool multi = h->ctx.size() > 1;
+    bool ready = nc.launched && (!multi || nc.waited);
+    if (nc.launched && !ready && (h->icp_ahead_mode == 2 || h->p2p.on || hipEventQuery(nc.ev_done) == hipSuccess)) {
+        HCK(hipStreamWaitEvent(h->stream, nc.ev_done, 0)); nc.waited = true; ready = true;
+    }
+    (void)hipGetLastError();
+    if (!ready) return SSF_OK;
+    const FrameMaps nm = batch_slot(nc.maps, nslot);
+    IcpLoop first;
+    icp_start_from(first, h->pose);
+    *next = NextIcp{h->cam, nm.pix2, nm.fpack, icp_transform(first), h->d_icp_replicas, h->d_tickets + 8, h->d_icp, h->mb_dev, ++h->icp_seq};
+    h->drop_ahead();
+    h->ahead.valid = true; h->ahead.from_fuse = from_fuse; h->ahead.seq = next->seq; h->ahead.ctx = &nc; h->ahead.slot = nslot;
+    h->ahead.stamp = h->stamp + 1; h->ahead.pose = h->pose;
+    *have = true;
+    return SSF_OK;
+}
+static int fuse_begin(ssf_handle* h, int migrate, bool ahead_ok = false) {
     const long long nmodel_g = total_model(h), nvis_g = total_visible(h);
     SurfelSoA& M = h->model[h->mcur];
     h->bins.drop();
@@ -780,9 +805,16 @@
             h->part_set ^= 1;
         }
         const AssocTables at{h->cc->d_best, h->cc->d_matched, h->d_cand, h->S};
+        h->fuse_ahead = false;
+        FuseIcp fi{};
+        if (ahead_ok && h->fuse_totals.from_tot && (h->icp_ahead_mode == 1 || h->icp_ahead_mode == 2) && single_shard_alone(h) && icp_chains(h)) {
+            const int ra = next_icp_if_ready(h, true, &h->fuse_next, &h->fuse_ahead);
+            if (ra) return ra;
+            if (h->fuse_ahead) fi = FuseIcp{1, h->fuse_next.pix2, h->fuse_next.fpack, h->fuse_next.T, h->fuse_next.replicas, h->fuse_next.ticket};
+        }
         launch_fuse(h->stream, M, h->cc->frame, h->pose, h->stamp, h->id_offset, h->n_visible, at, nvis_g > 0 ? 1 : 0,
                     h->cfg.nb_supersurfels_max, h->shard, h->d_cnt, h->oov[h->ocur], h->oov_tail - h->oov_head, h->classify,
-                    h->d_state, h->d_state_oov, h->d_bc_oov, ws, h->fuse_totals.from_tot);
+                    h->d_state, h->d_state_oov, h->d_bc_oov, ws, h->fuse_totals.from_tot, h->fuse_ahead ? &fi : nullptr);
         if (h->fuse_migrate)
             launch_pack_emigrants(h->stream, M, at, h->id_offset, h->n_visible, h->d_state, nvis_g > 0 ? 1 : 0, h->shard, h->d_migrants);
     }
@@ -802,31 +834,20 @@
                               h->d_state, ws);
         NextIcp next{};
         P2PView next_pv{};
-        bool have_next = false;
-        if (h->icp_ahead && (h->p2p.on || h->ahead_tuner.current() == 1) && icp_is_one_launch(h) && h->cfg.icp_iter > 0 && !h->pending.empty()) {
-            ExtractCtx& nc = h->ctx[h->pending.front().first];
-            const int nslot = h->pending.front().second;
-            const bool multi = h->ctx.size() > 1;
-            bool ready = nc.launched && (!multi || nc.waited);
-            if (nc.launched && !ready && (h->icp_ahead_mode == 2 || h->p2p.on || hipEventQuery(nc.ev_done) == hipSuccess)) {
-                HCK(hipStreamWaitEvent(h->stream, nc.ev_done, 0)); nc.waited = true; ready = true;
-            }
-            (void)hipGetLastError();
-            if (ready) {
-                const FrameMaps nm = batch_slot(nc.maps, nslot);
-                IcpLoop first;
-                icp_start_from(first, h->pose);
-                next = NextIcp{h->cam, nm.pix2, nm.fpack, icp_transform(first), h->d_icp_replicas, h->d_tickets + 8, h->d_icp, h->mb_dev, ++h->icp_seq};
-                if (h->p2p.on) next_pv = p2p_view(h, ++h->p2p.seq_icp);
-                h->ahead.valid = true; h->ahead.seq = next.seq; h->ahead.ctx = &nc; h->ahead.slot = nslot;
-                h->ahead.stamp = h->stamp + 1; h->ahead.pose = h->pose;
-                have_next = true;
-            }
-        }
+        bool have_next = h->fuse_ahead;
+        if (have_next) next = h->fuse_next;
+        else if (h->p2p.on || h->icp_ahead_mode == 3) {
+            const int ra = next_icp_if_ready(h, false, &next, &have_next);
+            if (ra) return ra;
+            if (have_next && h->p2p.on) next_pv = p2p_view(h, ++h->p2p.seq_icp);
+        }
+        const IcpResidual resid{h->cc->d_best, h->cc->d_matched, h->S, h->id_offset, h->d_ahead_rows};
         if (exchanges_natively(h)) { int rg = comm_gather_counts(h); if (rg) return rg; }
         launch_move_rows(h->stream, M, h->model[h->mcur ^ 1], h->oov[h->ocur], h->n_visible + (h->fuse_migrate ? 2 : 1) * h->S, h->oov_tail - h->oov_head,
                          h->d_state, h->d_state_oov, h->d_bc_oov, ws, h->d_cnt, h->mb_dev, seq, have_next ? &next : nullptr,
-                         have_next && h->p2p.on ? &next_pv : nullptr, h->fuse_totals.from_tot ? &h->fuse_totals : nullptr);
+                         have_next && h->p2p.on ? &next_pv : nullptr, h->fuse_totals.from_tot ? &h->fuse_totals : nullptr,
+                         h->fuse_ahead ? &resid : nullptr);
+        h->fuse_ahead = false;
         h->mcur ^= 1;
     } else {
         launch_first_frame(h->stream, M, h->cc->frame, h->pose, h->S, h->cfg.nb_supersurfels_max, h->shard, h->d_cnt);
@@ -885,7 +906,7 @@
 }
 
 static int do_fuse(ssf_handle* h, ssf_frame_result* out) {
-    int rc = fuse_begin(h, 0);
+    int rc = fuse_begin(h, 0, true);
     return rc ? rc : fuse_end(h, nullptr, out);
 }
 
@@ -910,7 +931,7 @@
     (void)hipMemsetAsync(h->d_icp_replicas, 0, 2 * SSF_ICP_REPLICAS * 32 * sizeof(long long), h->stream);
     (void)hipMemsetAsync(h->d_tickets, 0, 512 * sizeof(unsigned int), h->stream);
     (void)hipStreamSynchronize(h->stream);
-    h->icp_chain = false; h->ahead.valid = false;
+    h->icp_chain = false; h->drop_ahead();
 }
 struct TrackFrame { double t_a = 0.0, t_b = 0.0; int kf = -1; bool timing = false, first_it = true; IcpWaiter w; };
 int TileCopy::make_if_large(ssf_handle* h) {
@@ -1057,7 +1078,6 @@
     ssf_frame_result r;
     if (!rc) rc = exchange_and_fuse(h, &r);
     if (rc) return rc;
-    if (h->pending.empty()) h->ahead_tuner.sequence_break(); else h->ahead_tuner.frame_done(now_us(), r.icp_iters);
     h->host_us[1] += f.t_b - f.t_a; h->host_us[2] += now_us() - f.t_b; h->host_us[3] += 1;
     if (f.timing) { rc = stage_times(h, &r); if (rc) return rc; }
     if (out) *out = r;
@@ -1259,7 +1279,6 @@
     h->move_totals_on = SSF_ENV_INT("MOVE_TOTALS", SSF_MOVE_TOTALS_DEFAULT) != 0;
     h->icp_ahead_mode = SSF_ENV_INT("ICP_AHEAD", 1);
     h->icp_ahead = h->icp_ahead_mode != 0;
-    h->ahead_tuner.forced = SSF_ENV_INT("ICP_AHEAD", -1);
     h->icp_chain = SSF_ENV_INT("ICP_CHAIN", 1) != 0;
     if (SSF_ENV_SET("NO_GRAPH")) h->graph_failed = true;
     if (cfg->stream) h->stream = (hipStream_t)cfg->stream;
@@ -1291,7 +1310,8 @@
     h->batch = std::max(1, std::min(cfg->extract_batch, SSF_MAX_BATCH));
     h->ctx.resize(nctx);
     h->pass_team = SSF_ENV_INT("PASS_TEAM", 0) != 0;
-    bool ok = dalloc(h, &h->d_srgb_lut, 256) && dalloc(h, &h->d_tickets, 512);
+    bool ok = dalloc(h, &h->d_srgb_lut, 256) && dalloc(h, &h->d_tickets, 512) && dalloc(h, &h->d_ahead_rows, SSF_MOVE_ICP_WG);
+    if (ok) ok = hipMemset(h->d_ahead_rows, 0, SSF_MOVE_ICP_WG * sizeof(unsigned int)) == hipSuccess;
     {
         const int ne = pass_geometry_entries(W, H);
         std::vector<uint2> tab((size_t)ne);
@@ -1885,7 +1905,7 @@
 int ssf_apply_deformation(ssf_handle* h, const float* np, const float* nr, const float* nt, int m, const float* w4, const int32_t* idx4) {
     if (!h || !np || !nr || !nt || !w4 || !idx4 || m <= 0) return SSF_ERR_INVALID_ARG;
     drop_shard_sizes(h);
-    h->ahead.valid = false;
+    h->drop_ahead();
     const size_t n = h->n_model;
     if (n == 0) return SSF_OK;
     float *d_np, *d_nr, *d_nt, *d_w, *d_nodes; int32_t* d_i;
@@ -1942,8 +1962,17 @@
 long long ssf_waiter_matches(ssf_handle* h) { return h ? h->n_waiter_matches : -1; }
 int ssf_tuner_state(ssf_handle* h, double* out4) {
     if (!h || !out4) return SSF_ERR_INVALID_ARG;
-    const AheadTuner& t = h->ahead_tuner;
-    out4[0] = t.current(); out4[1] = t.frames; out4[2] = t.n[0] ? t.sum[0] / t.n[0] : 0.0; out4[3] = t.n[1] ? t.sum[1] / t.n[1] : 0.0;
+    out4[0] = h->icp_ahead ? 1.0 : 0.0; out4[1] = (double)(h->n_ahead_fused + h->n_ahead_separate); out4[2] = 0.0; out4[3] = 0.0;
+    return SSF_OK;
+}
+int ssf_ahead_stats(ssf_handle* h, long long out4[4]) {
+    if (!h || !out4) return SSF_ERR_INVALID_ARG;
+    unsigned int rows[SSF_MOVE_ICP_WG];
+    HCK(hipStreamSynchronize(h->stream));
+    HCK(hipMemcpy(rows, h->d_ahead_rows, sizeof(rows), hipMemcpyDeviceToHost));
+    long long resid = 0;
+    for (int i = 0; i < SSF_MOVE_ICP_WG; i++) resid += rows[i];
+    out4[0] = h->n_ahead_fused; out4[1] = h->n_ahead_separate; out4[2] = h->n_ahead_dropped; out4[3] = resid;
     return SSF_OK;
 }
 long long ssf_waiter_match_repairs(ssf_handle* h) { return h ? h->n_waiter_match_repairs : -1; }
diff --git a/supersurfel_fusion_amd/csrc/ssf_track_fuse.hip b/supersurfel_fusion_amd/csrc/ssf_track_fuse.hip
--- a/supersurfel_fusion_amd/csrc/ssf_track_fuse.hip
+++ b/supersurfel_fusion_amd/csrc/ssf_track_fuse.hip
@@ -700,7 +700,7 @@
 #pragma unroll
     for (int j = 0; j < OOV_PER_WG; j++) {
         cls[j] = classify_post(pre[j], z[j]);
-        if (lv[j]) {
+        if (in[j]) {
             const long long phys = head + ((long long)wg * OOV_PER_WG + j) * 256  + threadIdx.x;
             if (cls[j] == 2) O.rows.conf[phys] = -1.0f;
             state_oov[phys] = (uint8_t)cls[j];
@@ -918,18 +918,20 @@
 __device__ unsigned long long* g_fuse_trace = nullptr;
 void set_fuse_trace(unsigned long long* p) { (void)hipMemcpyToSymbol(HIP_SYMBOL(g_fuse_trace), &p, sizeof(p)); }
 #endif
-__global__ __launch_bounds__(256) void k_update_insert(SurfelSoA M, SurfelSoA F, Rt pose, int stamp, long long id_offset,
+__global__ __launch_bounds__(256) __attribute__((amdgpu_num_sgpr(112))) void k_update_insert(SurfelSoA M, SurfelSoA F, Rt pose, int stamp, long long id_offset,
                                                        int n_visible, const unsigned long long* __restrict__ best,
                                                        const uint8_t* __restrict__ matched, const int32_t* __restrict__ cand, int S,
                                                        int do_update, int capacity, int rank, int nranks, float tile, Counters* cnt,
                                                        int nupd, int nchunks, int nb_vis, int nb_oov, OovStore O, ClassifyArgs ca,
                                                        uint8_t* __restrict__ state_vis, uint8_t* __restrict__ state_oov,
-                                                       uint32_t* __restrict__ bc_oov, PartitionWs ws, int migrate, int tail_in_move) {
+                                                       uint32_t* __restrict__ bc_oov, PartitionWs ws, int migrate, int tail_in_move,
+                                                       FuseIcp fi) {
     __builtin_amdgcn_s_setprio(3);
     __shared__ int wave_tot[16];
     __shared__ int hist[4][6];
     __shared__ int s_last;
     __shared__ uint32_t tot[8];
+    __shared__ unsigned long long red[29 * ICP_SLOTS];
     const int b = blockIdx.x;
 #ifdef SSF_EXPERIMENTS
     unsigned long long* const trace = g_fuse_trace;
@@ -941,15 +943,23 @@
     else if (b >= nupd + nchunks) {
         const int vb = b - nupd - nchunks, i = vb * blockDim.x + threadIdx.x, wv = threadIdx.x >> 6;
         int cls = 7;
+        const bool ahead = fi.on != 0;
+        if (ahead) {
+            for (int q = threadIdx.x; q < 29 * ICP_SLOTS; q += 256) red[q] = 0ull;
+            __syncthreads();
+        }
         if (i < n_visible) {
             int f = cand[i];
             float conf = M.conf[i]; int seen = M.stamps[2 * (size_t)i + 1]; V3 pos = ld3(M.pos, (size_t)i);
-            asm volatile("" : "+v"(f), "+v"(conf), "+v"(seen), "+v"(pos.x));
+            V3 lab = v3(0.f, 0.f, 0.f), nrm = v3(0.f, 0.f, 0.f);
+            if (ahead) { lab = ld3(M.lab, (size_t)i); nrm = ld3(M.r2, (size_t)i); }
+            asm volatile("" : "+v"(f), "+v"(conf), "+v"(seen), "+v"(pos.x), "+v"(lab.x), "+v"(nrm.x));
             const bool rewritten = do_update && f >= 0 && (uint32_t)(best[f] & 0xFFFFFFFFull) == (uint32_t)(id_offset + i);
             if (!rewritten) {
                 cls = classify_values(ca.cam, conf, seen, pos, pose, ca.plane_depth, stamp, ca.delta_t, ca.conf_thresh, ca.zmin, ca.zmax);
                 if (cls == 2) M.conf[i] = -1.0f;
                 state_vis[i] = (uint8_t)cls;
+                if (ahead && cls == 0) icp_row(ca.cam, fi.pix2, fi.fpack, fi.T.R, fi.T.t, pos, lab, nrm, red, lane() & (ICP_SLOTS - 1), 0);
             }
         }
 #pragma unroll
@@ -960,7 +970,16 @@
             if (k) {
                 atomicAdd(&ws.sup_vis[(vb / PART_GROUP) * 6 + threadIdx.x], k);
                 atomic_add_done(&ws.tot[(vb & (PART_REPLICAS - 1)) * 8 + threadIdx.x], k);
-            }
+                if (ahead && threadIdx.x == 0) (void)__hip_atomic_fetch_add(&fi.ticket[65], k, __ATOMIC_RELAXED, __HIP_MEMORY_SCOPE_AGENT);
+            }
+        }
+        if (ahead && threadIdx.x >= 64 && threadIdx.x < 64 + 29) {
+            const int k = threadIdx.x - 64;
+            unsigned long long t29 = 0;
+#pragma unroll
+            for (int sidx = 0; sidx < ICP_SLOTS; sidx++) t29 += red[k * ICP_SLOTS + sidx];
+            if (t29 != 0) (void)__hip_atomic_fetch_add(reinterpret_cast<unsigned long long*>(fi.replicas) + (size_t)(vb % SSF_ICP_REPLICAS) * 32 + k, t29,
+                                                       __ATOMIC_RELAXED, __HIP_MEMORY_SCOPE_AGENT);
         }
     } else if (b >= nupd)
         insert_chunk(M, F, pose, stamp, matched, S, capacity, rank, nranks, tile, cnt, wave_tot, b - nupd, nchunks, ca, state_vis, ws);
@@ -1052,14 +1071,106 @@
     pos = r.pos; lab = r.lab; nrm = r.r2;
     store_row(B, j, r);
 }
-template <bool ICP, bool P2P>
+#define MOVE_ICP_LIST 2048
+__device__ __forceinline__ void icp_residual_block(const SurfelSoA& V, const OovStore& O, const uint8_t* __restrict__ state_vis,
+                                                   const uint8_t* __restrict__ state_oov, const uint32_t* __restrict__ bc_oov,
+                                                   const PartitionWs& ws, const Counters* cnt, const NextIcp& nx, const MoveTotals& mt,
+                                                   const IcpResidual& rs) {
+    __shared__ unsigned long long red[29 * ICP_SLOTS];
+    __shared__ unsigned int s_list[MOVE_ICP_LIST];
+    __shared__ unsigned int s_n, s_total;
+    __shared__ int s_last;
+    const unsigned int eb = blockIdx.x, tid = threadIdx.x, t0 = eb * 256u + tid, stride = SSF_MOVE_ICP_WG * 256u;
+    for (int q = tid; q < 29 * ICP_SLOTS; q += 256) red[q] = 0ull;
+    if (tid == 0) {
+        s_n = 0u;
+        uint32_t v = 0;
+#pragma unroll
+        for (int r = 0; r < PART_REPLICAS; r++) v += ws.tot[r * 8 + 0] + ws.tot[r * 8 + 3] + ws.tot[r * 8 + 6];
+        s_total = v;
+    }
+    __syncthreads();
+    const int slot = lane() & (ICP_SLOTS - 1);
+    auto row_terms = [&](unsigned int code) {
+        const bool oov = (code >> 31) != 0u;
+        const size_t r = (size_t)(code & 0x7FFFFFFFu);
+        const float* ppos = oov ? O.rows.pos : V.pos; const float* plab = oov ? O.rows.lab : V.lab; const float* pnrm = oov ? O.rows.r2 : V.r2;
+        V3 pos = ld3(ppos, r), lab = ld3(plab, r), nrm = ld3(pnrm, r);
+        asm volatile("" : "+v"(pos.x), "+v"(lab.x), "+v"(nrm.x));
+        icp_row(nx.cam, nx.pix2, nx.fpack, nx.T.R, nx.T.t, pos, lab, nrm, red, slot, 0);
+    };
+    auto push = [&](unsigned int code) {
+        const unsigned int k = atomicAdd(&s_n, 1u);
+        if (k < MOVE_ICP_LIST) s_list[k] = code; else row_terms(code);
+    };
+    const int nv = mt.nv, n_ins = cnt->n_inserted;
+    for (unsigned int f = t0; f < (unsigned int)rs.S; f += stride) {
+        unsigned int m8 = rs.matched[f]; unsigned long long bk = rs.best[f];
+        asm volatile("" : "+v"(m8), "+v"(bk));
+        if (!m8 || bk == SSF_NO_MATCH) continue;
+        const long long local = (long long)(uint32_t)(bk & 0xFFFFFFFFull) - rs.id_offset;
+        if (local < 0 || local >= nv) continue;
+        if (state_vis[local] == 0) push((unsigned int)local);
+    }
+    for (unsigned int i = (unsigned int)nv + t0; i < (unsigned int)(nv + n_ins); i += stride)
+        if (state_vis[i] == 0) push(i);
+    {
+        const long long head = mt.head_old, tail = mt.tail_old;
+        const long long c_lo = head >> 4, c_hi = (tail + 15) >> 4, per = (c_hi - c_lo + SSF_MOVE_ICP_WG - 1) / SSF_MOVE_ICP_WG;
+        const long long c0 = c_lo + (long long)eb * per, c1 = c0 + per < c_hi ? c0 + per : c_hi;
+        for (long long c = c0 + tid; c < c1; c += 256) {
+            const long long p0 = c << 4, pa = p0 > head ? p0 : head, pb = (p0 + 16 < tail ? p0 + 16 : tail) - 1;
+            if (pb < pa) continue;
+            const uint32_t any = (bc_oov[(pa - head) >> 8] | bc_oov[(pb - head) >> 8]) & 0xFFFFu;
+            if (!any) continue;
+            uint32_t wd[4];
+            if (p0 + 16 <= (long long)O.cap) {
+                const uint4 sv = *reinterpret_cast<const uint4*>(state_oov + p0);
+                wd[0] = sv.x; wd[1] = sv.y; wd[2] = sv.z; wd[3] = sv.w;
+            } else {
+#pragma unroll
+                for (int j = 0; j < 4; j++) wd[j] = 0x07070707u;
+                for (long long q = pa; q <= pb; q++) { const int j = (int)(q - p0); wd[j >> 2] = (wd[j >> 2] & ~(0xFFu << (8 * (j & 3)))) | ((uint32_t)state_oov[q] << (8 * (j & 3))); }
+            }
+#pragma unroll
+            for (int j = 0; j < 16; j++) {
+                const long long q = p0 + j;
+                if (q >= pa && q <= pb && ((wd[j >> 2] >> (8 * (j & 3))) & 0xFFu) == 0u) push(0x80000000u | (unsigned int)q);
+            }
+        }
+    }
+    __syncthreads();
+    const unsigned int rows = s_n, listed = rows < MOVE_ICP_LIST ? rows : MOVE_ICP_LIST;
+    for (unsigned int k = tid; k < listed; k += 256) row_terms(s_list[k]);
+    __syncthreads();
+    icp_fold(red, nx.replicas);
+    if (tid == 0) {
+        rs.rows_out[eb] = rows;
+        const unsigned int add = rows + (eb == 0u ? 1u : 0u);
+        int last = 0;
+        if (add) {
+            SSF_ARRIVE_RELEASE();
+            const unsigned int before = __hip_atomic_fetch_add(&nx.ticket[65], add, __ATOMIC_RELAXED, __HIP_MEMORY_SCOPE_AGENT);
+            last = before + add == s_total + 1u;
+            if (last) { __hip_atomic_store(&nx.ticket[65], 0u, __ATOMIC_RELAXED, __HIP_MEMORY_SCOPE_AGENT); SSF_ARRIVE_ACQUIRE(); }
+        }
+        s_last = last;
+    }
+    __syncthreads();
+    if (s_last) { const P2PView none{}; icp_publish<false>(nx.replicas, nx.sums, nx.mb, nx.seq, none, 0ull); }
+}
+template <int ICP, bool P2P>
 __global__ __launch_bounds__(256) void k_move_rows(SurfelSoA V, SurfelSoA Vn, OovStore O, const uint8_t* __restrict__ state_vis,
                                                    const uint8_t* __restrict__ state_oov,
                                                    const uint32_t* __restrict__ bc_oov, PartitionWs ws,
                                                    Counters* cnt, int nb_vis, NextIcp nx, Mailbox* mb,
-                                                   unsigned long long cnt_seq, P2PView pv, MoveTotals mt) {
+                                                   unsigned long long cnt_seq, P2PView pv, MoveTotals mt, IcpResidual rs) {
     __builtin_amdgcn_s_setprio(3);
-    if (blockIdx.x == 0 && threadIdx.x == 255) {
+    if constexpr (ICP == 2) {
+        if (blockIdx.x < SSF_MOVE_ICP_WG) { icp_residual_block(V, O, state_vis, state_oov, bc_oov, ws, cnt, nx, mt, rs); return; }
+    }
+    const unsigned int bx = blockIdx.x - (ICP == 2 ? SSF_MOVE_ICP_WG : 0);
+    if (bx == 0 && threadIdx.x == 255) {
         Counters c;
         if (mt.from_tot) {
             uint32_t tot[8];
@@ -1082,9 +1193,9 @@
         }
         mailbox_counters(c, mb, cnt_seq);
     }
-    if (mt.from_tot && blockIdx.x == 0 && threadIdx.x >= 64 && threadIdx.x < 255)
+    if (mt.from_tot && bx == 0 && threadIdx.x >= 64 && threadIdx.x < 255)
         for (int i = threadIdx.x - 64; i < ws.words; i += 191) ws.other[i] = 0u;
-    if ((int)blockIdx.x >= nb_vis && bc_oov[blockIdx.x - nb_vis] == 0u) return;
+    if ((int)bx >= nb_vis && bc_oov[bx - nb_vis] == 0u) return;
     __shared__ uint32_t s_tot[8];
     if (mt.from_tot && threadIdx.x < 8) {
         uint32_t v = 0;
@@ -1100,16 +1211,16 @@
     auto new_n_visible = [&]() -> int { return mt.from_tot ? (int)(s_tot[0] + s_tot[6] + s_tot[3]) : cnt->n_visible; };
     __shared__ int hist[4][6];
     __shared__ uint32_t base[6];
-    __shared__ unsigned long long red[ICP ? 29 * ICP_SLOTS : 1];
-    if (ICP) for (int i = threadIdx.x; i < 29 * ICP_SLOTS; i += blockDim.x) red[i] = 0ull;
+    __shared__ unsigned long long red[ICP == 1 ? 29 * ICP_SLOTS : 1];
+    if (ICP == 1) for (int i = threadIdx.x; i < 29 * ICP_SLOTS; i += blockDim.x) red[i] = 0ull;
     if (threadIdx.x < 6) base[threadIdx.x] = 0u;
     const int wv = threadIdx.x >> 6;
     int cls = 7, in_wave = 0;
     bool keep = false;
     V3 pos, lab, nrm;
-    if ((int)blockIdx.x < nb_vis) {
+    if ((int)bx < nb_vis) {
         const int nv = mv_nv, n_rows = nv + mv_nc;
-        const int i = blockIdx.x * blockDim.x + threadIdx.x;
+        const int i = bx * blockDim.x + threadIdx.x;
         RowRegs row;
         if (i < n_rows) {
             int st = (int)state_vis[i];
@@ -1117,8 +1228,8 @@
             asm volatile("" : "+v"(st), "+v"(row.pos.x));
             cls = (i < nv ? 0 : 3) + st;
         }
-        const int g0 = (int)(blockIdx.x / PART_GROUP), ng = 6 * g0;
-        const int row0 = g0 * PART_GROUP * 256, n16 = 16 * ((int)blockIdx.x - g0 * PART_GROUP);
+        const int g0 = (int)(bx / PART_GROUP), ng = 6 * g0;
+        const int row0 = g0 * PART_GROUP * 256, n16 = 16 * ((int)bx - g0 * PART_GROUP);
         __syncthreads();
         for (int w = threadIdx.x; w < ng; w += blockDim.x) {
             const uint32_t v = ws.sup_vis[w];
@@ -1166,7 +1277,7 @@
             if (cls == 0 || cls == 3) {
                 const size_t j = cls == 0 ? r : (size_t)mv_a0() + mv_b0() + r;
                 store_row(Vn, j, row);
-                if (ICP) { pos = row.pos; lab = row.lab; nrm = row.r2; keep = true; }
+                if (ICP == 1) { pos = row.pos; lab = row.lab; nrm = row.r2; keep = true; }
             } else {
                 const size_t j = (cls == 1 ? (size_t)mv_head_new() : (size_t)mv_tail_old) + r;
                 store_row(O.rows, j, row);
@@ -1174,7 +1285,7 @@
             }
         }
     } else {
-        const int ob = blockIdx.x - nb_vis;
+        const int ob = bx - nb_vis;
         const long long phys = (long long)mv_head_old + (long long)ob * blockDim.x + threadIdx.x;
         if (phys < mv_tail_old) {
             int lv = (int)O.live[phys], st = (int)state_oov[phys];
@@ -1196,21 +1307,21 @@
             int before = 0;
             for (int w = 0; w < wv; w++) before += hist[w][0];
             const size_t j = (size_t)mv_a0() + base[0] + before + in_wave;
-            if (ICP) { copy_row_keep(O.rows, (size_t)phys, Vn, j, pos, lab, nrm); keep = true; }
+            if (ICP == 1) { copy_row_keep(O.rows, (size_t)phys, Vn, j, pos, lab, nrm); keep = true; }
             else copy_row(O.rows, (size_t)phys, Vn, j);
         }
         if (cls == 0 || cls == 2) O.live[phys] = 0;
     }
-    if (ICP) {
+    if (ICP == 1) {
         if (keep) icp_row(nx.cam, nx.pix2, nx.fpack, nx.T.R, nx.T.t, pos, lab, nrm, red, lane() & (ICP_SLOTS - 1), 0);
         const int nkeep = __syncthreads_count(keep);
         if (P2P && new_n_visible() == 0) {
-            if (blockIdx.x == 0) icp_publish<true>(nx.replicas, nx.sums, nx.mb, nx.seq, pv, pv.seq);
+            if (bx == 0) icp_publish<true>(nx.replicas, nx.sums, nx.mb, nx.seq, pv, pv.seq);
             return;
         }
-        const bool vis = (int)blockIdx.x < nb_vis;
+        const bool vis = (int)bx < nb_vis;
         const int nbr = (mv_nv + mv_nc + 255) / 256;
-        if (vis ? (int)blockIdx.x >= nbr : nkeep == 0) return;
+        if (vis ? (int)bx >= nbr : nkeep == 0) return;
         __shared__ int s_last;
         icp_fold(red, nx.replicas);
         if (threadIdx.x == 0) {
@@ -1218,7 +1329,7 @@
             unsigned int rows = (unsigned int)nkeep;
             bool report = true;
             if (vis) {
-                const unsigned int g = blockIdx.x & 63u, in_group = ((unsigned int)nbr - g + 63u) / 64u;
+                const unsigned int g = bx & 63u, in_group = ((unsigned int)nbr - g + 63u) / 64u;
                 unsigned long long* gw = reinterpret_cast<unsigned long long*>(nx.ticket + 128) + g;
                 const unsigned long long before = __hip_atomic_fetch_add(gw, ((unsigned long long)rows << 32) | 1ull, __ATOMIC_RELAXED,
                                                                          __HIP_MEMORY_SCOPE_AGENT);
@@ -1738,14 +1849,15 @@
 }
 void launch_fuse(hipStream_t st, SurfelSoA model, SurfelSoA frame, Rt pose, int stamp, long long id_offset, int n_visible,
                  const AssocTables& at, int do_update, int capacity, const ShardArgs& sh, Counters* cnt, OovStore oov, int span_upper,
-                 const ClassifyArgs& ca, uint8_t* state_vis, uint8_t* state_oov, uint32_t* bc_oov, const PartitionWs& ws, int tail_in_move) {
+                 const ClassifyArgs& ca, uint8_t* state_vis, uint8_t* state_oov, uint32_t* bc_oov, const PartitionWs& ws, int tail_in_move,
+                 const FuseIcp* ahead) {
     ScopedKernel sk("update_insert", st);
     const int S = at.S, nchunks = (S + 255) / 256, nb_oov = (span_upper + 255) / 256, nb_vis = (n_visible + 255) / 256;
     const int nupd = (S + UPD_PER_WG - 1) / UPD_PER_WG;
     hipLaunchKernelGGL(k_update_insert, dim3(nupd + nchunks + nb_vis + (nb_oov + OOV_PER_WG - 1) / OOV_PER_WG), dim3(256), 0, st, model,
                        frame, pose, stamp, id_offset,
                        n_visible, at.best, at.matched, at.cand, S, do_update, capacity, sh.rank, sh.nranks, sh.tile, cnt, nupd, nchunks, nb_vis,
-                       nb_oov, oov, ca, state_vis, state_oov, bc_oov, ws, sh.migrate, tail_in_move);
+                       nb_oov, oov, ca, state_vis, state_oov, bc_oov, ws, sh.migrate, tail_in_move, (ahead && tail_in_move) ? *ahead : FuseIcp{});
 }
 void launch_pack_emigrants(hipStream_t st, SurfelSoA model, const AssocTables& at, long long id_offset, int n_visible,
                            const uint8_t* state_vis, int do_update, const ShardArgs& sh, int32_t* table) {
@@ -1765,13 +1877,14 @@
 void launch_move_rows(hipStream_t st, SurfelSoA vis_src, SurfelSoA vis_dst, OovStore oov, int nv_upper, int span_upper,
                       const uint8_t* state_vis, const uint8_t* state_oov, const uint32_t* bc_oov, const PartitionWs& ws,
                       Counters* cnt, Mailbox* mb, unsigned long long cnt_seq, const NextIcp* next, const P2PView* next_pv,
-                      const MoveTotals* totals) {
+                      const MoveTotals* totals, const IcpResidual* residual) {
     const int nb_vis = std::max(1, (nv_upper + 255) / 256), nb_oov = (span_upper + 255) / 256;
     const MoveTotals mt = totals ? *totals : MoveTotals{0, 0, 0, 0};
-    auto kernel = !next ? k_move_rows<false, false> : (next_pv ? k_move_rows<true, true> : k_move_rows<true, false>);
+    const bool resid = next && residual && !next_pv && mt.from_tot;
+    auto kernel = !next ? k_move_rows<0, false> : (next_pv ? k_move_rows<1, true> : (resid ? k_move_rows<2, false> : k_move_rows<1, false>));
     ScopedKernel sk(next ? "reorder_move_icp" : "reorder_move", st);
-    hipLaunchKernelGGL(kernel, dim3(nb_vis + nb_oov), dim3(256), 0, st, vis_src, vis_dst, oov, state_vis, state_oov, bc_oov, ws, cnt, nb_vis,
-                       next ? *next : NextIcp{}, mb, cnt_seq, next_pv ? *next_pv : P2PView{}, mt);
+    hipLaunchKernelGGL(kernel, dim3(nb_vis + nb_oov + (resid ? SSF_MOVE_ICP_WG : 0)), dim3(256), 0, st, vis_src, vis_dst, oov, state_vis, state_oov, bc_oov, ws, cnt, nb_vis,
+                       next ? *next : NextIcp{}, mb, cnt_seq, next_pv ? *next_pv : P2PView{}, mt, residual ? *residual : IcpResidual{});
 }
 void launch_oov_compact(hipStream_t st, OovStore src, OovStore dst, int span_upper, int new_head, uint32_t* bc_oov, Counters* cnt,
                         int set_span) {
```

Measured after the change: 9259 frames/s. 0.796x the previous value.
